# alinlab/ifseg

Measured on AMD Instinct MI355X. Metric: images/sec (512x512, SegOFA-Base fwd+bwd), higher is better.
Workload: dtype bf16; 1 GPU; BASELINE configs[1]: SegOFA-Base bf16, batch 8/GPU, 512x512, 15 classes (L=36), frozen ResNet-101 trunk (one pass per 2 future batches on a second stream; a ring of 4 synthetic batches, every batch through the trunk exactly once), dropout 0.10 / drop-path 0.10; step = fwd + upsample/CE loss + bwd + clip + Adam; steps enqueued from the host; global_batch=8, parallelism=dp1

## Files before the change

### ifseg_amd/csrc/attention.hip

```cpp
#include <type_traits>
#include "common.h"
#include "prof.h"
#include "../../include/ifseg_hip.h"

namespace {

struct AttnArgs {
  const bf16_t *q, *k, *v, *pq, *pk;
  bf16_t* o;
  float* lse;
  int B, H, T, S;
  long long q_bs, k_bs, v_bs, o_bs;
  int ldq, ldk, ldv, ldo, ldpq, ldpk;
  int rel_mode, P, code_bias, n2d, Lt, causal;
  const int* gcode;
  const float *rel2d, *rel1d, *relx, *dense;
  int dense_ld;
  const bf16_t* dO; long long do_bs; int lddo;
  const float* delta;
  bf16_t *dq, *dk, *dv; long long dq_bs, dk_bs, dv_bs; int lddq, lddk, lddv;
  bf16_t *dpq, *dpk;
  float *drel2d_part, *drel1d_part, *drelx_part;
  int nparts;
  const float* gain;
// ... 1148 lines not shown
                }
                bool masked = j >= a.S;
                if (a.causal) {
                  if (tile_grid) masked |= (qi >= a.P) || (j > qi);
                  else masked |= (qi >= a.P) && (j > qi);
                }
                const float p = masked ? 0.f : __builtin_amdgcn_exp2f(fmaf(sv, LOG2E, nlse_q));
                dsv[e] = p * (gain * dp[rg * 4 + e] - del_q);
                pdp = fmaf(p, dp[rg * 4 + e], pdp);
              }
            }
            ud.w[rg2 * 2] = pack2bf(dsv[0], dsv[1]); ud.w[rg2 * 2 + 1] = pack2bf(dsv[2], dsv[3]);
          }
          dsf[s2] = ud.b;
        }
#pragma unroll
        for (int s2 = 0; s2 < 2; ++s2) {
#pragma unroll
          for (int cb = 0; cb < NKS / 2; ++cb) {
            const int o0 = (bKt ^ (cb << 6)) + (kb * 32 + s2 * 16) * 256;
            U64 x, y;
            x.s = lds_read_tr(sKb(cur) + o0);
            y.s = lds_read_tr(sKb(cur) + ((o0 + 2048) ^ 32));
            U128 f; f.w[0] = x.w[0]; f.w[1] = x.w[1]; f.w[2] = y.w[0]; f.w[3] = y.w[1];
            dq[cb] = __builtin_amdgcn_mfma_f32_32x32x16_bf16(f.b, dsf[s2], dq[cb], 0, 0, 0);
          }
        }
      }
    }
    if (it + 1 < nsched) store_kv(cur ^ 1);
    __syncthreads();
  }

  if (a.dgain_rows) {
    const float tot = pdp + __shfl_xor(pdp, 32);
    if (qvalid && half == 0) a.dgain_rows[((long long)b * a.H + h) * a.T + qi] = tot;
  }
  if (qvalid) {
    bf16_t* dqp = a.dq + (long long)b * a.dq_bs + (long long)qi * a.lddq + h * 64;
#pragma unroll
    for (int db = 0; db < 2; ++db) store_tile_bf16(dqp + db * 32, dq[db], a.dq_scale, half, true);
    if constexpr (HAS_POS) {
      bf16_t* pp = a.dpq + ((long long)b * a.T + qi) * (a.H * 64) + h * 64;
#pragma unroll
      for (int db = 0; db < 2; ++db) store_tile_bf16(pp + db * 32, dq[2 + db], a.dpq_scale, half, true);
    }
  }
}

template <bool HAS_POS>
__global__ __launch_bounds__(256, 2) void attn_bwd_dq_kernel(AttnArgs a) { attn_bwd_dq_body<HAS_POS>(a, blockIdx.x); }


__global__ void attn_delta_kernel(const bf16_t* o, const bf16_t* dO, float* delta, int B, int H, int T,
                                  long long o_bs, int ldo, long long do_bs, int lddo) {
  const long long gid = (long long)blockIdx.x * blockDim.x + threadIdx.x;
  const long long grp = gid >> 3;
  const int sub = (int)(gid & 7);
  const long long total = (long long)B * T * H;
  float acc = 0.f;
  if (grp < total) {
    const int hh = (int)(grp % H);
    const long long bt = grp / H;
    const int t = (int)(bt % T), bb = (int)(bt / T);
    U128 x, y;
    x.v = *reinterpret_cast<const uint4*>(o + bb * o_bs + (long long)t * ldo + hh * 64 + sub * 8);
    y.v = *reinterpret_cast<const uint4*>(dO + bb * do_bs + (long long)t * lddo + hh * 64 + sub * 8);
#pragma unroll
    for (int e = 0; e < 4; ++e) acc += bflo(x.w[e]) * bflo(y.w[e]) + bfhi(x.w[e]) * bfhi(y.w[e]);
  }
  acc += __shfl_xor(acc, 1); acc += __shfl_xor(acc, 2); acc += __shfl_xor(acc, 4);
  if (grp < total && sub == 0) {
    const int hh = (int)(grp % H);
    const long long bt = grp / H;
    delta[((bt / T) * H + hh) * T + (bt % T)] = acc;
  }
}

}

namespace {
constexpr int SMALL_TAB_MAX = 2048;
struct ReduceArgs { ifseg_attn_reduce_args a; int nbq, nbk, nbt[3]; };
__global__ __launch_bounds__(256) void attn_bwd_reduce_kernel(ReduceArgs r) {
  const ifseg_attn_reduce_args& a = r.a;
  int blk = blockIdx.x;
  const int tid = threadIdx.x;
  if (blk < r.nbq + r.nbk) {
    const bool isq = blk < r.nbq;
    if (!isq) blk -= r.nbq;
    const long long n = (long long)(isq ? a.T : a.S) * a.C;
    const bf16_t* part = reinterpret_cast<const bf16_t*>(isq ? a.dpos_q_part : a.dpos_k_part);
    float* acc = isq ? a.dpos_q_acc : a.dpos_k_acc;
    const long long i = ((long long)blk * 256 + tid) * 8;
    if (i >= n) return;
    float s[8] = {0.f, 0.f, 0.f, 0.f, 0.f, 0.f, 0.f, 0.f};
    if (a.accumulate_pos) {
      const float4 a0 = *reinterpret_cast<const float4*>(acc + i), a1 = *reinterpret_cast<const float4*>(acc + i + 4);
      s[0] = a0.x; s[1] = a0.y; s[2] = a0.z; s[3] = a0.w; s[4] = a1.x; s[5] = a1.y; s[6] = a1.z; s[7] = a1.w;
    }
#pragma unroll 8
    for (int b = 0; b < a.B; ++b) {
      const uint4 v = *reinterpret_cast<const uint4*>(part + (long long)b * n + i);
      s[0] += bflo(v.x); s[1] += bfhi(v.x); s[2] += bflo(v.y); s[3] += bfhi(v.y);
      s[4] += bflo(v.z); s[5] += bfhi(v.z); s[6] += bflo(v.w); s[7] += bfhi(v.w);
    }
    *reinterpret_cast<float4*>(acc + i) = make_float4(s[0], s[1], s[2], s[3]);
    *reinterpret_cast<float4*>(acc + i + 4) = make_float4(s[4], s[5], s[6], s[7]);
    return;
  }
  blk -= r.nbq + r.nbk;
  if (blk < a.H) {
    if (!a.dgain) return;
    __shared__ float red[4];
    float s = 0.f;
    for (int b = 0; b < a.B; ++b) {
      const float* d = a.delta + ((long long)b * a.H + blk) * a.T;
      for (int t = tid; t < a.T; t += 256) s += d[t];
    }
    s = warp_sum(s);
    if ((tid & 63) == 0) red[tid >> 6] = s;
    __syncthreads();
    if (tid == 0) reinterpret_cast<bf16_t*>(a.dgain)[blk] = f2bf(((red[0] + red[1]) + (red[2] + red[3])) / a.gain[blk]);
    return;
  }
  blk -= a.H;
  __shared__ float tred[8][33];
  __shared__ float tsmall[SMALL_TAB_MAX];
#pragma unroll
  for (int t = 0; t < 3; ++t) {
    if (t >= a.ntab) return;
    if (blk < r.nbt[t] && a.tab_n[t] <= SMALL_TAB_MAX) {
      const int n = a.tab_n[t], h = blk;
      if (a.nparts <= 8) {
        for (int j = tid; j < n; j += 256) {
          const float* p = a.tab_part[t] + (long long)h * a.nparts * n + j;
          float sum = 0.f;
          for (int q = 0; q < a.nparts; ++q) sum += p[(long long)q * n];
          tsmall[j] = sum;
        }
        __syncthreads();
      } else
      for (int j0 = 0; j0 < n; j0 += 32) {
        const int j = j0 + (tid & 31), g = tid >> 5;
        float sum = 0.f;
        if (j < n) {
          const float* p = a.tab_part[t] + (long long)h * a.nparts * n + j;
#pragma unroll 4
          for (int q = g; q < a.nparts; q += 8) sum += p[(long long)q * n];
        }
        tred[g][tid & 31] = sum;
        __syncthreads();
        if (g == 0 && j < n) {
          float tot = 0.f;
#pragma unroll
          for (int q = 0; q < 8; ++q) tot += tred[q][tid];
          tsmall[j] = tot;
        }
        __syncthreads();
      }
      __shared__ int sidx[SMALL_TAB_MAX];
      for (int j = tid; j < n; j += 256) sidx[j] = a.tab_idx[t][j];
      __syncthreads();
      for (int rb = tid; rb < a.tab_nbucket[t]; rb += 256) {
        float tot = 0.f;
        bool any = false;
        for (int j = 0; j < n; ++j)
          if (sidx[j] == rb) { tot += tsmall[j]; any = true; }
        if (any) a.tab_acc[t][(long long)rb * a.H + h] += tot;
      }
      return;
    }
    if (blk < r.nbt[t]) {
      const int n = a.tab_n[t], nchunk = (n + 31) / 32;
      const int h = blk / nchunk, j = (blk - h * nchunk) * 32 + (tid & 31), g = tid >> 5;
      float sum = 0.f;
      if (j < n) {
        const float* p = a.tab_part[t] + (long long)h * a.nparts * n + j;
#pragma unroll 4
        for (int q = g; q < a.nparts; q += 8) sum += p[(long long)q * n];
      }
      tred[g][tid & 31] = sum;
      __syncthreads();
      if (g == 0 && j < n) {
        const int bucket = a.tab_idx[t][j];
        if (bucket >= 0) {
          float tot = 0.f;
#pragma unroll
          for (int q = 0; q < 8; ++q) tot += tred[q][tid];
          atomicAdd(&a.tab_acc[t][(long long)bucket * a.H + h], tot);
        }
      }
      return;
    }
    blk -= r.nbt[t];
  }
}
}

extern "C" int ifseg_attn_bwd_reduce(const ifseg_attn_reduce_args* x, void* stream) {
  (void)hipGetLastError();
  if (!x || x->B <= 0 || x->H <= 0 || x->T <= 0 || x->S <= 0 || (x->C & 7) || x->ntab < 0 || x->ntab > 3) return IFSEG_ERR_BAD_ARG;
  ReduceArgs r{};
  r.a = *x;
  r.nbq = x->dpos_q_part ? (int)(((long long)x->T * x->C / 8 + 255) / 256) : 0;
  r.nbk = x->dpos_k_part ? (int)(((long long)x->S * x->C / 8 + 255) / 256) : 0;
  long long total = (long long)r.nbq + r.nbk + x->H;
  for (int t = 0; t < x->ntab; ++t) {
    if (!x->tab_part[t] || !x->tab_idx[t] || !x->tab_acc[t] || x->tab_n[t] <= 0 || x->nparts <= 0) return IFSEG_ERR_BAD_ARG;
    if (x->tab_nbucket[t] <= 0) return IFSEG_ERR_BAD_ARG;
    r.nbt[t] = x->tab_n[t] <= SMALL_TAB_MAX ? x->H : x->H * ((x->tab_n[t] + 31) / 32);
    total += r.nbt[t];
  }
  if ((x->dgain && (!x->delta || !x->gain)) || total >= (1ll << 31)) return IFSEG_ERR_BAD_ARG;
  hipLaunchKernelGGL(attn_bwd_reduce_kernel, dim3((unsigned)total), dim3(256), 0, (hipStream_t)stream, r);
  IFSEG_CHECK_LAUNCH();
  return 0;
}

static int attn_check(const AttnArgs& a) {
  if (a.rel_mode || a.causal) {
    if (a.P % 64 || a.P > a.T || a.P > a.S) return IFSEG_ERR_BAD_SHAPE;
  }
  if ((a.ldq | a.ldk | a.ldv | a.ldo) & 7) return IFSEG_ERR_BAD_SHAPE;
  if (((size_t)a.q | (size_t)a.k | (size_t)a.v | (size_t)a.o | (size_t)a.dO | (size_t)a.dq | (size_t)a.dk | (size_t)a.dv) & 15)
    return IFSEG_ERR_BAD_ARG;
  if ((a.q_bs | a.k_bs | a.v_bs | a.o_bs | a.do_bs | a.dq_bs | a.dk_bs | a.dv_bs) & 7) return IFSEG_ERR_BAD_SHAPE;
  return 0;
}

extern "C" int ifseg_attn_fwd(const void* q, const void* k, const void* v, const void* pos_q, const void* pos_k,
                              void* out, float* lse, int B, int H, int T, int S, int ldq, int ldk, int ldv,
                              int ldo, int ldpq, int ldpk, long long q_bs, long long k_bs, long long v_bs,
                              long long o_bs, int rel_mode, int P, const int* gcode, int code_bias, int n2d,
                              const float* rel2d, const float* rel1d, const float* relx, int causal,
                              const float* dense_bias, const void* gain, int grid_w, int dense_ld, void* stream) {
  (void)hipGetLastError();
  AttnArgs a{};
  a.grid_w = grid_w;
  a.q = (const bf16_t*)q; a.k = (const bf16_t*)k; a.v = (const bf16_t*)v;
  a.pq = (const bf16_t*)pos_q; a.pk = (const bf16_t*)pos_k; a.o = (bf16_t*)out; a.lse = lse;
  a.B = B; a.H = H; a.T = T; a.S = S; a.ldq = ldq; a.ldk = ldk; a.ldv = ldv; a.ldo = ldo;
  a.ldpq = ldpq; a.ldpk = ldpk; a.q_bs = q_bs; a.k_bs = k_bs; a.v_bs = v_bs; a.o_bs = o_bs;
  a.rel_mode = rel_mode; a.P = P; a.gcode = gcode; a.code_bias = code_bias; a.n2d = rel_mode ? n2d : 0;
  a.Lt = T - P; a.rel2d = rel2d; a.rel1d = rel1d; a.relx = relx; a.causal = causal; a.dense = dense_bias; a.gain = (const float*)gain;
  a.dense_ld = dense_bias ? (dense_ld > 0 ? dense_ld : S) : 0;
  if (dense_bias && a.dense_ld < S) return IFSEG_ERR_BAD_ARG;
#ifdef IFSEG_EXP_NOBIAS_FWD
  pos_q = nullptr; a.pq = nullptr; a.pk = nullptr; a.rel_mode = 0; a.n2d = 0; rel_mode = 0;
#endif
  if (!rel_mode && !causal) a.P = S;
  int rc = attn_check(a);
  if (rc) return rc;
  const int nq = (T + 127) / 128;
  size_t lds = 2 * (KT_BYTES + VT_BYTES) + (rel_mode ? (((size_t)a.n2d + 3) & ~3) * 4 + (size_t)P * 4 : 0);
  if (lds > 160 * 1024) return IFSEG_ERR_BAD_SHAPE;
  dim3 grid(nq * H * B), block(256);
  hipStream_t s = (hipStream_t)stream;
  ifseg_prof_begin(IFSEG_K_ATTN_FWD, s, 4.0 * 64 * (double)T * S * B * H, 0);
  if (pos_q) {
    if (lds > 64 * 1024) (void)hipFuncSetAttribute((const void*)attn_fwd_kernel<true>, hipFuncAttributeMaxDynamicSharedMemorySize, (int)lds);
    hipLaunchKernelGGL(attn_fwd_kernel<true>, grid, block, lds, s, a);
  } else {
    if (lds > 64 * 1024) (void)hipFuncSetAttribute((const void*)attn_fwd_kernel<false>, hipFuncAttributeMaxDynamicSharedMemorySize, (int)lds);
    hipLaunchKernelGGL(attn_fwd_kernel<false>, grid, block, lds, s, a);
  }
  ifseg_prof_end(IFSEG_K_ATTN_FWD, s);
  IFSEG_CHECK_LAUNCH();
  return 0;
}

extern "C" int ifseg_attn_bwd(const ifseg_attn_bwd_args* x, void* stream) {
  (void)hipGetLastError();
  AttnArgs a{};
  a.q = (const bf16_t*)x->q; a.k = (const bf16_t*)x->k; a.v = (const bf16_t*)x->v;
  a.pq = (const bf16_t*)x->pos_q; a.pk = (const bf16_t*)x->pos_k; a.lse = (float*)x->lse;
  a.B = x->B; a.H = x->H; a.T = x->T; a.S = x->S;
  a.ldq = x->ldq; a.ldk = x->ldk; a.ldv = x->ldv; a.ldpq = x->ldpq; a.ldpk = x->ldpk;
  a.q_bs = x->q_bs; a.k_bs = x->k_bs; a.v_bs = x->v_bs;
  a.rel_mode = x->rel_mode; a.P = x->P; a.gcode = x->gcode; a.code_bias = x->code_bias;
  a.n2d = x->rel_mode ? x->n2d : 0; a.Lt = x->T - x->P;
  a.rel2d = x->rel2d; a.rel1d = x->rel1d; a.relx = x->relx; a.causal = x->causal;
  a.dO = (const bf16_t*)x->dout; a.do_bs = x->do_bs; a.lddo = x->lddo; a.delta = x->delta;
  a.dq = (bf16_t*)x->dq; a.dk = (bf16_t*)x->dk; a.dv = (bf16_t*)x->dv;
  a.dq_bs = x->dq_bs; a.dk_bs = x->dk_bs; a.dv_bs = x->dv_bs; a.lddq = x->lddq; a.lddk = x->lddk; a.lddv = x->lddv;
  a.dpq = (bf16_t*)x->dpos_q_part; a.dpk = (bf16_t*)x->dpos_k_part;
  a.drel2d_part = x->drel2d_part; a.drel1d_part = x->drel1d_part; a.drelx_part = x->drelx_part;
  a.nparts = x->nparts; a.gain = (const float*)x->gain; a.dq_scale = x->dq_scale; a.dpq_scale = x->dpq_scale;
  a.grid_w = x->grid_w;
  a.dgain_rows = x->dgain_rows;
#ifdef IFSEG_EXP_NOBIAS_BWD
  a.pq = nullptr; a.pk = nullptr; a.rel_mode = 0; a.n2d = 0;
#endif
  if (!a.rel_mode && !a.causal) a.P = a.S;
  int rc = attn_check(a);
  if (rc) return rc;
  if ((x->lddo | x->lddq | x->lddk | x->lddv | x->ldout) & 7) return IFSEG_ERR_BAD_SHAPE;
  {
    const long long ldmax = a.ldq > a.lddo ? (a.ldq > a.ldpq ? a.ldq : a.ldpq) : (a.lddo > a.ldpq ? a.lddo : a.ldpq);
    if ((long long)a.T * ldmax * 2 >= (1ll << 31)) return IFSEG_ERR_BAD_SHAPE;
// ... 71 lines not shown
```

### ifseg_amd/csrc/attention_bi.hip

```cpp
#include <type_traits>
#include "common.h"
#include "prof.h"
#include "../../include/ifseg_hip.h"

namespace {

constexpr float NEG_INF = -INFINITY;
constexpr float LOG2E = 1.4426950408889634f;

struct BiArgs {
  const bf16_t *q, *k, *v, *dO;
  const float *lse, *delta, *gain;
  const bf16_t* D;
  float* dgain_rows;
  bf16_t *dq, *dk, *dv, *dbias;
  bf16_t* out; float* lse_out; long long o_bs; int ldo;
  int B, H, T, S, Sp, Tp;
  long long q_bs, k_bs, v_bs, do_bs, dq_bs, dk_bs, dv_bs, dbias_gs;
  int ldq, ldk, ldv, lddo, lddq, lddk, lddv;
  int causal, P;
  float dq_scale;
  const int* kv_len;
  float drop_p;
  unsigned long long drop_seed; const unsigned long long* drop_seed_add;
// ... 610 lines not shown
        fo[s2][db].w[0] = x.w[0]; fo[s2][db].w[1] = x.w[1]; fo[s2][db].w[2] = y.w[0]; fo[s2][db].w[3] = y.w[1];
        x.s = lds_read_tr(sQ + oT[s2][db][0]);
        y.s = lds_read_tr(sQ + oT[s2][db][1]);
        fq[s2][db].w[0] = x.w[0]; fq[s2][db].w[1] = x.w[1]; fq[s2][db].w[2] = y.w[0]; fq[s2][db].w[3] = y.w[1];
      }
    __builtin_amdgcn_sched_barrier(0);
    if (it + 1 < sc.n) issue(it + 1, (it + 1) & 1);
    __builtin_amdgcn_sched_barrier(0);
#pragma unroll
    for (int rg = 0; rg < 4; ++rg) db_expand(wD[rg], s, rg);
    if (anypad) {
#pragma unroll
      for (int e = 0; e < 16; ++e) s[e] = kpad ? NEG_INF : s[e];
    }
#pragma unroll
    for (int ks = 0; ks < 4; ++ks) {
      s = __builtin_amdgcn_mfma_f32_32x32x16_bf16(qf[ks], kf[ks], s, 0, 0, 0);
      dp = __builtin_amdgcn_mfma_f32_32x32x16_bf16(of[ks], vfn[ks], dp, 0, 0, 0);
    }
    U128 up[2], ud[2];
#pragma unroll
    for (int s2 = 0; s2 < 2; ++s2)
#pragma unroll
      for (int e = 0; e < 8; e += 2) {
        const int r = s2 * 8 + e;
        const float p0 = __builtin_amdgcn_exp2f(fmaf(s[r], LOG2E, -ls[r]));
        const float p1 = __builtin_amdgcn_exp2f(fmaf(s[r + 1], LOG2E, -ls[r + 1]));
        if (DROP) {
          const int i = sc.block(it) * 32 + (r & 3) + 8 * (r >> 2) + 4 * half;
          const float k0_ = attn_keep(dr, attn_row_key(dr, rowbase + i), kj), k1_ = attn_keep(dr, attn_row_key(dr, rowbase + i + 1), kj);
          up[s2].w[e >> 1] = pack2bf(p0 * k0_, p1 * k1_);
          ud[s2].w[e >> 1] = pack2bf(-p0 * (de[r] - k0_ * (de[r] - dp[r])), -p1 * (de[r + 1] - k1_ * (de[r + 1] - dp[r + 1])));
        } else {
          up[s2].w[e >> 1] = pack2bf(p0, p1);
          ud[s2].w[e >> 1] = pack2bf(-p0 * dp[r], -p1 * dp[r + 1]);
        }
      }
#pragma unroll
    for (int s2 = 0; s2 < 2; ++s2) {
#pragma unroll
      for (int db = 0; db < 2; ++db) dv[db] = __builtin_amdgcn_mfma_f32_32x32x16_bf16(fo[s2][db].b, up[s2].b, dv[db], 0, 0, 0);
#pragma unroll
      for (int db = 0; db < 2; ++db) dk[db] = __builtin_amdgcn_mfma_f32_32x32x16_bf16(fq[s2][db].b, ud[s2].b, dk[db], 0, 0, 0);
    }
  };

  if (sc.n > 0) issue(0, 0);
  for (int it = 0; it < sc.n; ++it) {
    lds_dma_wait();
    __syncthreads();
    block(it);
  }
  if (bact && kvalid) {
    bf16_t* dvp = a.dv + (long long)b * a.dv_bs + (long long)kj * a.lddv + h * 64;
    bf16_t* dkp = a.dk + (long long)b * a.dk_bs + (long long)kj * a.lddk + h * 64;
#pragma unroll
    for (int db = 0; db < 2; ++db) {
      store_tile_bf16(dvp + db * 32, dv[db], gain, half, true);
      store_tile_bf16(dkp + db * 32, dk[db], 1.f, half, true);
    }
  }
}
__global__ __launch_bounds__(512, 2) void attn_bi_dkv_kernel(BiArgs a) { attn_bi_dkv_body<false>(a); }
__global__ __launch_bounds__(512, 2) void attn_bi_dkv_drop_kernel(BiArgs a) { attn_bi_dkv_body<true>(a); }

__global__ void attn_drop_mask_kernel(unsigned char* out, int B, int H, int T, int S, float p, unsigned long long seed,
                                      const unsigned long long* seed_add) {
  const long long n = (long long)B * H * T * S, id = (long long)blockIdx.x * blockDim.x + threadIdx.x;
  if (id >= n) return;
  const AttnDrop dr = attn_drop_setup(p, seed, seed_add);
  const int j = (int)(id % S);
  const unsigned row = (unsigned)(id / S);
  out[id] = attn_keep(dr, attn_row_key(dr, row), j) != 0.f;
}

struct DenseArgs {
  const bf16_t *pq, *pk;
  int ldpq, ldpk, H, T, S, Sp, Tp;
  int rel_mode, P, code_bias, n2d, Lt, causal;
  const int* gcode;
  const float *rel2d, *rel1d, *relx;
  bf16_t* D;
};

__global__ __launch_bounds__(512) void attn_dense_bias_kernel(DenseArgs a) {
  extern __shared__ __attribute__((aligned(16))) unsigned char smem[];
  float* sT = reinterpret_cast<float*>(smem);
  float* s1 = sT + ((a.n2d + 3) & ~3);
  int* sG = reinterpret_cast<int*>(s1 + ((2 * a.Lt + 2) & ~3));
  const int tid = threadIdx.x, lane = tid & 63, wave = tid >> 6, half = lane >> 5, x = lane & 31;
  const int ntq = a.Tp >> 5, ntk = a.Sp >> 5;
  const int h = blockIdx.x / ntq, ti = blockIdx.x % ntq, i0 = ti * 32;
  float rx0 = 0.f, rx1 = 0.f;
  if (a.rel_mode) {
    for (int i = tid; i < a.n2d; i += 512) sT[i] = a.rel2d[(long long)h * a.n2d + i];
    for (int i = tid; i < 2 * a.Lt - 1; i += 512) s1[i] = a.rel1d[(long long)h * (2 * a.Lt - 1) + i];
    for (int i = tid; i < a.P; i += 512) sG[i] = a.gcode[i];
    rx0 = a.relx[h * 2]; rx1 = a.relx[h * 2 + 1];
  }
  __syncthreads();
  auto entry = [&](int i, int j, float abs_ij) -> float {
    if (i >= a.T || j >= a.S) return NEG_INF;
    if (a.causal) {
      const bool masked = (j < a.P) ? ((i >= a.P) || (j > i)) : ((i >= a.P) && (j > i));
      if (masked) return NEG_INF;
    }
    float r = 0.f;
    if (a.rel_mode) {
      if (i < a.P) r = (j < a.P) ? sT[sG[i] - sG[j] + a.code_bias] : rx0;
      else r = (j < a.P) ? rx1 : s1[(i - j) + a.Lt - 1];
    }
    return abs_ij + r;
  };
  bf16x8 fq[4];
  if (a.pq) {
    const bf16_t* qp = a.pq + (long long)min(i0 + x, a.T - 1) * a.ldpq + h * 64 + half * 8;
#pragma unroll
    for (int ks = 0; ks < 4; ++ks) { U128 u; u.v = *reinterpret_cast<const uint4*>(qp + ks * 16); fq[ks] = u.b; }
  }
  for (int tj = wave; tj < ntk; tj += 8) {
    const int j0 = tj * 32;
    const bool dead = a.causal && j0 < a.P && (i0 >= a.P || j0 > i0 + 31);
    if (dead && (i0 >= a.P || j0 > i0 + 63)) continue;
    bf16x8 fk[4];
    if (a.pq && !dead) {
      const bf16_t* kp = a.pk + (long long)min(j0 + x, a.S - 1) * a.ldpk + h * 64 + half * 8;
#pragma unroll
      for (int ks = 0; ks < 4; ++ks) { U128 w; w.v = *reinterpret_cast<const uint4*>(kp + ks * 16); fk[ks] = w.b; }
    }
    f32x16 acc;
#pragma unroll
    for (int e = 0; e < 16; ++e) acc[e] = 0.f;
    if (a.pq && !dead) {
#pragma unroll
      for (int ks = 0; ks < 4; ++ks) acc = __builtin_amdgcn_mfma_f32_32x32x16_bf16(fq[ks], fk[ks], acc, 0, 0, 0);
    }
    {
      unsigned* dp = reinterpret_cast<unsigned*>(a.D + ((long long)h * a.Tp + i0 + 4 * half) * a.Sp + j0 + (x & ~1));
      const bool odd = x & 1;
#pragma unroll
      for (int rg = 0; rg < 4; ++rg) {
        float v[4];
#pragma unroll
        for (int e = 0; e < 4; ++e) v[e] = dead ? NEG_INF : entry(i0 + 8 * rg + 4 * half + e, j0 + x, acc[rg * 4 + e]);
        const float s0 = odd ? v[0] : v[2], s1 = odd ? v[1] : v[3];
        const float r0 = __int_as_float(__builtin_amdgcn_update_dpp(0, __float_as_int(s0), 0xB1, 0xf, 0xf, true));
        const float r1 = __int_as_float(__builtin_amdgcn_update_dpp(0, __float_as_int(s1), 0xB1, 0xf, 0xf, true));
        const unsigned w0 = odd ? pack2bf(r0, v[2]) : pack2bf(v[0], r0), w1 = odd ? pack2bf(r1, v[3]) : pack2bf(v[1], r1);
        const int e0 = odd ? 2 : 0;
        dp[((long long)(8 * rg + e0) * a.Sp) >> 1] = w0;
        dp[((long long)(8 * rg + e0 + 1) * a.Sp) >> 1] = w1;
      }
    }
  }
}

constexpr int DB_NSUB = 8;
constexpr int DB_NPARTS = 4;
struct DbArgs {
  const bf16_t* dbias;
  long long gs;
  int ng, H, T, S, Sp, C;
  const bf16_t *pq, *pk;
  int ldpq, ldpk;
  float *dpq, *dpk;
  int accumulate;
  int tab_accumulate;
  float dpq_scale;
  int P, gh, gw, Lt, causal;
  float *drel2d, *drel1d, *drelx;
  int nb_q, nb_k, nb_2d;
};

__device__ __forceinline__ bf16x8 tr_frag(const unsigned char* tile, int rbase, int cb, int lane) {
  const int half = lane >> 5, i16 = lane & 15, g16 = (lane >> 4) & 1;
  const int col = cb * 32 + g16 * 16 + (i16 & 3) * 4;
  const int r0 = rbase + 4 * half + (i16 >> 2);
  U64 x, y;
  x.s = lds_read_tr(tile + vx_off(r0, col * 2));
  y.s = lds_read_tr(tile + vx_off(r0 + 8, col * 2));
  U128 f; f.w[0] = x.w[0]; f.w[1] = x.w[1]; f.w[2] = y.w[0]; f.w[3] = y.w[1];
  return f.b;
}

__global__ __launch_bounds__(256) void attn_dbias_grads_kernel(DbArgs a) {
  __shared__ __attribute__((aligned(16))) unsigned char sm[32768];
  const int tid = threadIdx.x, lane = tid & 63, half = lane >> 5;
  const int wave = __builtin_amdgcn_readfirstlane(tid >> 6);
  int blk = blockIdx.x < a.nb_q ? xcd_remap(blockIdx.x, a.nb_q) : a.nb_q + xcd_remap(blockIdx.x - a.nb_q, a.nb_k);
  const int lr = lane >> 3, lc = lane & 7;
  if (blk < a.nb_q) {
    const int nit = (a.T + 31) >> 5;
    const int h = blk / nit, i0 = (blk % nit) * 32;
    const int i = i0 + (lane & 31);
    const int ir = i < a.T ? i : a.T - 1;
    unsigned char* tile = sm + wave * 8192;
    f32x16 acc[2];
#pragma unroll
    for (int e = 0; e < 16; ++e) { acc[0][e] = 0.f; acc[1][e] = 0.f; }
    uint4 t4[4], d4[4];
    auto fetch = [&](int j0) {
#pragma unroll
      for (int u = 0; u < 4; ++u) {
        t4[u] = make_uint4(0, 0, 0, 0); d4[u] = make_uint4(0, 0, 0, 0);
        if (j0 + lr + 8 * u < a.S) t4[u] = *reinterpret_cast<const uint4*>(a.pk + (long long)(j0 + lr + 8 * u) * a.ldpk + h * 64 + lc * 8);
        const int g = lc >> 2, irow = min(i0 + lr + 8 * u, a.T - 1);
        if (g < a.ng) d4[u] = *reinterpret_cast<const uint4*>(a.dbias + g * a.gs + ((long long)h * a.T + irow) * a.Sp + j0 + (lc & 3) * 8);
      }
    };
    auto live = [&](int j) { return !(a.causal && j < a.P && (i0 >= a.P || j > i0 + 31)); };
    int j0 = wave * 32;
    if (j0 < a.Sp) fetch(j0);
    for (; j0 < a.Sp; j0 += 128) {
      if (!live(j0)) { if (j0 + 128 < a.Sp) fetch(j0 + 128); continue; }
      __builtin_amdgcn_wave_barrier();
#pragma unroll
      for (int u = 0; u < 4; ++u) {
        const int o = vx_off(lr + 8 * u, lc * 16);
        *reinterpret_cast<uint4*>(tile + o) = t4[u];
        *reinterpret_cast<uint4*>(tile + 4096 + o) = d4[u];
      }
      __builtin_amdgcn_fence(__ATOMIC_RELEASE, "wavefront");
      __builtin_amdgcn_wave_barrier();
      if (j0 + 128 < a.Sp) fetch(j0 + 128);
      U128 bfr[2][2];
#pragma unroll
      for (int s2 = 0; s2 < 2; ++s2)
#pragma unroll
        for (int g = 0; g < 2; ++g) {
          const int cb = g * 64 + (16 * s2 + 4 * half) * 2;
          const uint2 lo = *reinterpret_cast<const uint2*>(tile + 4096 + vx_off(lane & 31, cb));
          const uint2 hi = *reinterpret_cast<const uint2*>(tile + 4096 + vx_off(lane & 31, cb + 16));
          bfr[s2][g].w[0] = lo.x; bfr[s2][g].w[1] = lo.y; bfr[s2][g].w[2] = hi.x; bfr[s2][g].w[3] = hi.y;
        }
#pragma unroll
      for (int s2 = 0; s2 < 2; ++s2) {
        const bf16x8 a0 = tr_frag(tile, 16 * s2, 0, lane), a1 = tr_frag(tile, 16 * s2, 1, lane);
#pragma unroll
        for (int g = 0; g < 2; ++g)
          if (g < a.ng) {
            acc[0] = __builtin_amdgcn_mfma_f32_32x32x16_bf16(a0, bfr[s2][g].b, acc[0], 0, 0, 0);
            acc[1] = __builtin_amdgcn_mfma_f32_32x32x16_bf16(a1, bfr[s2][g].b, acc[1], 0, 0, 0);
          }
      }
      __builtin_amdgcn_wave_barrier();
    }
    __syncthreads();
    float* red = reinterpret_cast<float*>(sm);
#pragma unroll
    for (int cb = 0; cb < 2; ++cb) {
      if (cb) __syncthreads();
#pragma unroll
      for (int r = 0; r < 16; ++r) red[(wave * 16 + r) * 64 + lane] = acc[cb][r];
      __syncthreads();
#pragma unroll
      for (int k = 0; k < 4; ++k) {
        const int v = tid + 256 * k, r = v >> 6, ln = v & 63;
        const float t = (red[r * 64 + ln] + red[(16 + r) * 64 + ln]) + (red[(32 + r) * 64 + ln] + red[(48 + r) * 64 + ln]);
        const int c = cb * 32 + (r & 3) + 8 * (r >> 2) + 4 * (ln >> 5), ii = i0 + (ln & 31);
        if (ii < a.T) {
          float* p = a.dpq + (long long)ii * a.C + h * 64 + c;
          *p = (a.accumulate ? *p : 0.f) + t * a.dpq_scale;
        }
      }
    }
    return;
  }
  blk -= a.nb_q;
  {
    const int njt = a.Sp >> 5;
    const int h = blk / njt, jw0 = (blk % njt) * 32;
    unsigned char* sQ = sm + wave * 8192;
    f32x16 acc[2];
#pragma unroll
    for (int e = 0; e < 16; ++e) { acc[0][e] = 0.f; acc[1][e] = 0.f; }
    uint4 t4[4], d4[4];
    auto fetch = [&](int i0) {
#pragma unroll
      for (int u = 0; u < 4; ++u) {
        const int r = lr + 8 * u;
        t4[u] = make_uint4(0, 0, 0, 0); d4[u] = make_uint4(0, 0, 0, 0);
        if (i0 + r < a.T) {
          t4[u] = *reinterpret_cast<const uint4*>(a.pq + (long long)(i0 + r) * a.ldpq + h * 64 + lc * 8);
          const int g = lc >> 2;
          if (g < a.ng) d4[u] = *reinterpret_cast<const uint4*>(a.dbias + g * a.gs + ((long long)h * a.T + i0 + r) * a.Sp + jw0 + (lc & 3) * 8);
        }
      }
    };
    auto live = [&](int i) { return !(a.causal && jw0 < a.P && (i >= a.P || jw0 > i + 31)); };
    int i0 = wave * 32;
    if (i0 < a.T) fetch(i0);
    for (; i0 < a.T; i0 += 128) {
      if (!live(i0)) { if (i0 + 128 < a.T) fetch(i0 + 128); continue; }
      __builtin_amdgcn_wave_barrier();
#pragma unroll
      for (int u = 0; u < 4; ++u) {
        const int o = vx_off(lr + 8 * u, lc * 16);
        *reinterpret_cast<uint4*>(sQ + o) = t4[u];
        *reinterpret_cast<uint4*>(sQ + 4096 + o) = d4[u];
      }
      __builtin_amdgcn_fence(__ATOMIC_RELEASE, "wavefront");
      __builtin_amdgcn_wave_barrier();
      if (i0 + 128 < a.T) fetch(i0 + 128);
#pragma unroll
      for (int s2 = 0; s2 < 2; ++s2) {
        const bf16x8 a0 = tr_frag(sQ, 16 * s2, 0, lane), a1 = tr_frag(sQ, 16 * s2, 1, lane);
#pragma unroll
        for (int g = 0; g < 2; ++g)
          if (g < a.ng) {
            const bf16x8 bfr = tr_frag(sQ + 4096, 16 * s2, g, lane);
            acc[0] = __builtin_amdgcn_mfma_f32_32x32x16_bf16(a0, bfr, acc[0], 0, 0, 0);
            acc[1] = __builtin_amdgcn_mfma_f32_32x32x16_bf16(a1, bfr, acc[1], 0, 0, 0);
          }
      }
      __builtin_amdgcn_wave_barrier();
    }
    __syncthreads();
    float* red = reinterpret_cast<float*>(sm);
#pragma unroll
    for (int cb = 0; cb < 2; ++cb) {
      if (cb) __syncthreads();
#pragma unroll
      for (int r = 0; r < 16; ++r) red[(wave * 16 + r) * 64 + lane] = acc[cb][r];
      __syncthreads();
#pragma unroll
      for (int k = 0; k < 4; ++k) {
        const int v = tid + 256 * k, r = v >> 6, ln = v & 63;
        const float t = (red[r * 64 + ln] + red[(16 + r) * 64 + ln]) + (red[(32 + r) * 64 + ln] + red[(48 + r) * 64 + ln]);
        const int c = cb * 32 + (r & 3) + 8 * (r >> 2) + 4 * (ln >> 5), j = jw0 + (ln & 31);
        if (j < a.S) {
          float* p = a.dpk + (long long)j * a.C + h * 64 + c;
          *p = (a.accumulate ? *p : 0.f) + t;
        }
      }
    }
  }
}

__global__ __launch_bounds__(256) void attn_dbias_tables_kernel(DbArgs a) {
  __shared__ __attribute__((aligned(16))) float sf[2 * 4096];
  const int tid = threadIdx.x;
  int blk = blockIdx.x < a.nb_2d ? xcd_remap(blockIdx.x, a.nb_2d) : blockIdx.x;
  auto add8 = [](float* t, const uint4& v) {
    t[0] += bflo(v.x); t[1] += bfhi(v.x); t[2] += bflo(v.y); t[3] += bfhi(v.y);
    t[4] += bflo(v.z); t[5] += bfhi(v.z); t[6] += bflo(v.w); t[7] += bfhi(v.w);
  };
  if (blk < a.nb_2d) {
    const int ndy = 2 * a.gh - 1, w = a.gw, nch = w >> 3, npair = w * nch;
    const int dy = blk % ndy - (a.gh - 1), part = (blk / ndy) % DB_NPARTS, h = blk / (DB_NPARTS * ndy);
    const int ylo = dy > 0 ? dy : 0, yhi = dy < 0 ? a.gh + dy : a.gh;
    const int y0 = ylo + ((part - ylo) % DB_NPARTS + DB_NPARTS) % DB_NPARTS;
    float* out = a.drel2d + ((long long)h * DB_NPARTS + part) * ndy * (2 * w - 1) + (long long)(dy + a.gh - 1) * (2 * w - 1);
    if (a.causal && dy < 0) {
      if (!a.tab_accumulate) for (int d = tid; d < 2 * w - 1; d += 256) out[d] = 0.f;
      return;
    }
    const int nyp = npair <= 128 ? 2 : 1;
    const int yp = tid / npair, p = tid - yp * npair;
    for (int p0 = 0; p0 < npair; p0 += 256) {
      const int pp = p0 + p;
      float t[8] = {0.f, 0.f, 0.f, 0.f, 0.f, 0.f, 0.f, 0.f};
      const bool on = yp < nyp && pp < npair;
      const int xi = on ? pp / nch : 0, xc = on ? pp - xi * nch : 0;
      if (on) {
        const bf16_t* base = a.dbias + ((long long)h * a.T + xi) * a.Sp + xc * 8 - (long long)dy * w;
        const long long ystep = (long long)w * a.Sp + w;
#pragma unroll 4
        for (int yi = y0 + yp * DB_NPARTS; yi < yhi; yi += nyp * DB_NPARTS) {
          add8(t, *reinterpret_cast<const uint4*>(base + yi * ystep));
          if (a.ng > 1) add8(t, *reinterpret_cast<const uint4*>(base + a.gs + yi * ystep));
        }
      }
      if (p0) __syncthreads();
      if (on) {
#pragma unroll
        for (int e = 0; e < 8; ++e) sf[yp * 4096 + xi * w + xc * 8 + e] = t[e];
      }
      __syncthreads();
    }
    for (int d = tid; d < 2 * w - 1; d += 256) {
      const int dx = d - (w - 1);
      float t = 0.f;
      for (int xi = (dx > 0 ? dx : 0); xi < (dx < 0 ? w + dx : w); ++xi) {
        t += sf[xi * w + (xi - dx)];
        if (nyp > 1) t += sf[4096 + xi * w + (xi - dx)];
      }
      out[d] = (a.tab_accumulate ? out[d] : 0.f) + t;
    }
    return;
  }
  blk -= a.nb_2d;
  if (blk >= a.H * DB_NPARTS) {
    blk -= a.H * DB_NPARTS;
    const int sub = blk % DB_NSUB, part = (blk / DB_NSUB) % DB_NPARTS, h = blk / (DB_NSUB * DB_NPARTS), P = a.P, Lt = a.Lt;
    const bf16_t* hb = a.dbias + (long long)h * a.T * a.Sp;
    float* o1 = a.drel1d + ((long long)h * DB_NPARTS + part) * (2 * Lt - 1);
    const int dl = tid & 63, rc = tid >> 6;
    for (int d0 = sub; d0 < 2 * Lt - 1; d0 += DB_NSUB * 64) {
      const int d = d0 + DB_NSUB * dl;
      float t = 0.f;
      if (d < 2 * Lt - 1) {
        const int off = d - (Lt - 1);
        const int lo = off > 0 ? off : 0, hi = off < 0 ? Lt + off : Lt;
        const int first = lo + ((part - lo) % DB_NPARTS + DB_NPARTS) % DB_NPARTS;
#pragma unroll 4
        for (int ti = first + rc * DB_NPARTS; ti < hi; ti += 4 * DB_NPARTS) {
          const long long o = (long long)(P + ti) * a.Sp + P + ti - off;
          t += bf2f(hb[o]);
          if (a.ng > 1) t += bf2f(hb[a.gs + o]);
        }
      }
      __syncthreads();
      sf[rc * 64 + dl] = t;
      __syncthreads();
      if (rc == 0 && d < 2 * Lt - 1) {
        const float tt = (sf[dl] + sf[64 + dl]) + (sf[128 + dl] + sf[192 + dl]);
        o1[d] = (a.tab_accumulate ? o1[d] : 0.f) + tt;
      }
    }
    return;
  }
  {
    const int h = blk / DB_NPARTS, part = blk % DB_NPARTS, P = a.P, Lt = a.Lt;
    const bf16_t* hb = a.dbias + (long long)h * a.T * a.Sp;
    auto dB = [&](int i, int j) {
      float t = bf2f(hb[(long long)i * a.Sp + j]);
      if (a.ng > 1) t += bf2f(hb[a.gs + (long long)i * a.Sp + j]);
      return t;
    };
    float t0 = 0.f, t1 = 0.f;
    {
      const int nrow = (P - part + DB_NPARTS - 1) / DB_NPARTS, nch = Lt >> 3, nit = nrow * nch;
      float t[8] = {0.f, 0.f, 0.f, 0.f, 0.f, 0.f, 0.f, 0.f};
      for (int it0 = tid; it0 < nit; it0 += 4 * 256) {
        uint4 v[4][2];
#pragma unroll
        for (int u = 0; u < 4; ++u) {
          const int it = it0 + u * 256, r = it / nch, ch = it - r * nch;
#pragma unroll
          for (int g = 0; g < 2; ++g)
            v[u][g] = (it < nit && g < a.ng) ? *reinterpret_cast<const uint4*>(hb + g * a.gs + (long long)(part + DB_NPARTS * r) * a.Sp + P + ch * 8)
                                             : make_uint4(0, 0, 0, 0);
        }
#pragma unroll
        for (int u = 0; u < 4; ++u) { add8(t, v[u][0]); add8(t, v[u][1]); }
      }
      float tail = 0.f;
      const int nt = Lt & 7;
      for (int it = tid; it < nrow * nt; it += 256) {
        const int r = it / nt, e = it - r * nt;
        tail += dB(part + DB_NPARTS * r, P + (Lt & ~7) + e);
      }
      t0 = ((t[0] + t[1]) + (t[2] + t[3])) + ((t[4] + t[5]) + (t[6] + t[7])) + tail;
    }
    const int nchunk = P >> 3, nrs = nchunk <= 128 ? 2 : 1;
    for (int cc = tid; cc < nchunk * nrs; cc += 256) {
      const int c = cc % nchunk, rs = cc / nchunk;
      float t[8] = {0.f, 0.f, 0.f, 0.f, 0.f, 0.f, 0.f, 0.f};
      int ti = part + rs * DB_NPARTS;
      const int tstep = nrs * DB_NPARTS;
      for (; ti + 3 * tstep < Lt; ti += 4 * tstep) {
        uint4 v[4][2];
#pragma unroll
        for (int u = 0; u < 4; ++u)
#pragma unroll
          for (int g = 0; g < 2; ++g)
            v[u][g] = g < a.ng ? *reinterpret_cast<const uint4*>(hb + g * a.gs + (long long)(P + ti + u * tstep) * a.Sp + c * 8) : make_uint4(0, 0, 0, 0);
#pragma unroll
        for (int u = 0; u < 4; ++u) { add8(t, v[u][0]); add8(t, v[u][1]); }
      }
      for (; ti < Lt; ti += tstep)
        for (int g = 0; g < a.ng; ++g) add8(t, *reinterpret_cast<const uint4*>(hb + g * a.gs + (long long)(P + ti) * a.Sp + c * 8));
      t1 += ((t[0] + t[1]) + (t[2] + t[3])) + ((t[4] + t[5]) + (t[6] + t[7]));
    }
    sf[tid] = t0; sf[256 + tid] = t1;
    __syncthreads();
    for (int o = 128; o > 0; o >>= 1) {
      if (tid < o) { sf[tid] += sf[tid + o]; sf[256 + tid] += sf[256 + tid + o]; }
      __syncthreads();
    }
    float* ox = a.drelx + ((long long)h * DB_NPARTS + part) * 2;
    if (tid == 0) { ox[0] = (a.tab_accumulate ? ox[0] : 0.f) + sf[0]; ox[1] = (a.tab_accumulate ? ox[1] : 0.f) + sf[256]; }
    return;
  }
}

}

extern "C" int ifseg_attn_dense_bias(const void* pos_q, const void* pos_k, int ldpq, int ldpk, int H, int T, int S,
                                     int rel_mode, int P, const int* gcode, int code_bias, int n2d, const float* rel2d,
                                     const float* rel1d, const float* relx, int causal, void* D, int Sp, int Tp,
                                     void* stream) {
  (void)hipGetLastError();
  if (!D || H <= 0 || T <= 0 || S <= 0 || (Sp & 31) || (Tp & 31) || Sp < S || Tp < T) return IFSEG_ERR_BAD_ARG;
  if ((pos_q == nullptr) != (pos_k == nullptr) || ((ldpq | ldpk) & 7)) return IFSEG_ERR_BAD_ARG;
  if (rel_mode && (!gcode || !rel2d || !rel1d || !relx)) return IFSEG_ERR_BAD_ARG;
  if ((rel_mode || causal) && (P > T || P > S || P < 0)) return IFSEG_ERR_BAD_SHAPE;
  DenseArgs a{};
  a.pq = (const bf16_t*)pos_q; a.pk = (const bf16_t*)pos_k; a.ldpq = ldpq; a.ldpk = ldpk;
  a.H = H; a.T = T; a.S = S; a.Sp = Sp; a.Tp = Tp;
  a.rel_mode = rel_mode; a.P = (rel_mode || causal) ? P : S; a.code_bias = code_bias; a.n2d = rel_mode ? n2d : 0; a.Lt = rel_mode ? T - P : 0; a.causal = causal;
  a.gcode = gcode; a.rel2d = rel2d; a.rel1d = rel1d; a.relx = relx; a.D = (bf16_t*)D;
  if ((size_t)D & 15) return IFSEG_ERR_BAD_ARG;
  const size_t lds = rel_mode ? ((((size_t)n2d + 3) & ~(size_t)3) + (((size_t)2 * a.Lt + 2) & ~(size_t)3) + (size_t)P) * 4 : 16;
  if (lds > 160 * 1024) return IFSEG_ERR_BAD_SHAPE;
  if (lds > 64 * 1024) (void)hipFuncSetAttribute((const void*)attn_dense_bias_kernel, hipFuncAttributeMaxDynamicSharedMemorySize, (int)lds);
  hipLaunchKernelGGL(attn_dense_bias_kernel, dim3((unsigned)(H * (Tp / 32))), dim3(512), lds, (hipStream_t)stream, a);
  IFSEG_CHECK_LAUNCH();
  return 0;
}

extern "C" int ifseg_attn_bwd_bi(const ifseg_attn_bi_args* x, void* stream) {
  (void)hipGetLastError();
  if (!x || x->B <= 0 || x->H <= 0 || x->T <= 0 || x->S <= 0) return IFSEG_ERR_BAD_ARG;
  if ((x->Sp & 31) || (x->Tp & 31) || x->Sp < x->S || x->Tp < x->T || !x->D) return IFSEG_ERR_BAD_ARG;
  BiArgs a{};
  a.q = (const bf16_t*)x->q; a.k = (const bf16_t*)x->k; a.v = (const bf16_t*)x->v; a.dO = (const bf16_t*)x->dout;
  a.lse = x->lse; a.delta = x->delta; a.D = (const bf16_t*)x->D; a.gain = (const float*)x->gain;
  a.dq = (bf16_t*)x->dq; a.dk = (bf16_t*)x->dk; a.dv = (bf16_t*)x->dv; a.dbias = (bf16_t*)x->dbias; a.dgain_rows = x->dgain_rows;
  a.B = x->B; a.H = x->H; a.T = x->T; a.S = x->S; a.Sp = x->Sp; a.Tp = x->Tp;
  a.q_bs = x->q_bs; a.k_bs = x->k_bs; a.v_bs = x->v_bs; a.do_bs = x->do_bs; a.dq_bs = x->dq_bs; a.dk_bs = x->dk_bs; a.dv_bs = x->dv_bs;
  a.dbias_gs = (long long)x->H * x->T * x->Sp;
  a.ldq = x->ldq; a.ldk = x->ldk; a.ldv = x->ldv; a.lddo = x->lddo; a.lddq = x->lddq; a.lddk = x->lddk; a.lddv = x->lddv;
  a.causal = x->causal; a.P = x->causal ? x->P : x->S; a.dq_scale = x->dq_scale; a.kv_len = x->kv_len;
  a.drop_p = x->drop_p; a.drop_seed = x->drop_seed; a.drop_seed_add = x->drop_seed_add;
  if (!(a.drop_p >= 0.f && a.drop_p < 1.f)) return IFSEG_ERR_BAD_ARG;
  const bool dropping = a.drop_p > 0.f;
  if ((a.ldq | a.ldk | a.ldv | a.lddo | a.lddq | a.lddk | a.lddv) & 7) return IFSEG_ERR_BAD_SHAPE;
  if (((size_t)a.q | (size_t)a.k | (size_t)a.v | (size_t)a.dO | (size_t)a.dq | (size_t)a.dk | (size_t)a.dv | (size_t)a.dbias) & 15)
    return IFSEG_ERR_BAD_ARG;
  if ((a.q_bs | a.k_bs | a.v_bs | a.do_bs | a.dq_bs | a.dk_bs | a.dv_bs) & 7) return IFSEG_ERR_BAD_SHAPE;
  if (a.causal && ((a.P & 63) || a.P > a.T || a.P > a.S)) return IFSEG_ERR_BAD_SHAPE;
  {
    long long ldmax = a.ldq;
    for (long long l : {(long long)a.lddo, (long long)a.ldk, (long long)a.ldv}) ldmax = l > ldmax ? l : ldmax;
    const long long rows = a.T > a.S ? a.T : a.S;
    if (rows * ldmax * 2 >= (1ll << 31) || (long long)a.Tp * a.Sp * 2 >= (1ll << 31))
      return IFSEG_ERR_BAD_SHAPE;
  }
  hipStream_t s = (hipStream_t)stream;
  const int nbg = (a.B + 3) / 4;
  const int ph = x->phases ? x->phases : (IFSEG_ATTN_BWD_DKV | IFSEG_ATTN_BWD_DQ);
  if (ph & IFSEG_ATTN_BWD_DKV) {
    if (!a.dk || !a.dv) return IFSEG_ERR_BAD_ARG;
    auto kern = dropping ? attn_bi_dkv_drop_kernel : attn_bi_dkv_kernel;
    (void)hipFuncSetAttribute((const void*)kern, hipFuncAttributeMaxDynamicSharedMemorySize, LDS_DKV);
    ifseg_prof_begin(IFSEG_K_ATTN_DKV, s, 6.0 * 64 * (double)a.T * a.S * a.B * a.H, 0);
    hipLaunchKernelGGL(kern, dim3(((a.S + 63) / 64) * a.H * nbg), dim3(512), LDS_DKV, s, a);
    ifseg_prof_end(IFSEG_K_ATTN_DKV, s);
  }
  if (ph & IFSEG_ATTN_BWD_DQ) {
    if (!a.dq || !a.dbias) return IFSEG_ERR_BAD_ARG;
    auto kern = dropping ? attn_bi_dq_drop_kernel : attn_bi_dq_kernel;
    (void)hipFuncSetAttribute((const void*)kern, hipFuncAttributeMaxDynamicSharedMemorySize, LDS_DQ);
    ifseg_prof_begin(IFSEG_K_ATTN_DQ, s, 2.0 * 64 * (double)a.T * a.S * a.B * a.H, 0);
    hipLaunchKernelGGL(kern, dim3(((a.T + 63) / 64) * a.H * nbg), dim3(512), LDS_DQ, s, a);
    ifseg_prof_end(IFSEG_K_ATTN_DQ, s);
  }
  IFSEG_CHECK_LAUNCH();
  return 0;
}

extern "C" int ifseg_attn_fwd_bi(const ifseg_attn_bi_args* x, void* stream) {
  (void)hipGetLastError();
  if (!x || x->B <= 0 || x->H <= 0 || x->T <= 0 || x->S <= 0 || !x->q || !x->k || !x->v || !x->out || !x->lse || !x->D) return IFSEG_ERR_BAD_ARG;
  if ((x->Sp & 31) || x->Sp < x->S || (x->Tp & 31) || x->Tp < x->T) return IFSEG_ERR_BAD_ARG;
  BiArgs a{};
  a.q = (const bf16_t*)x->q; a.k = (const bf16_t*)x->k; a.v = (const bf16_t*)x->v; a.D = (const bf16_t*)x->D; a.gain = (const float*)x->gain;
  a.out = (bf16_t*)x->out; a.lse_out = const_cast<float*>(x->lse); a.o_bs = x->out_bs; a.ldo = x->ldout;
  a.B = x->B; a.H = x->H; a.T = x->T; a.S = x->S; a.Sp = x->Sp; a.Tp = x->Tp;
  a.q_bs = x->q_bs; a.k_bs = x->k_bs; a.v_bs = x->v_bs; a.ldq = x->ldq; a.ldk = x->ldk; a.ldv = x->ldv;
  a.causal = x->causal; a.P = x->causal ? x->P : x->S; a.kv_len = x->kv_len;
  a.drop_p = x->drop_p; a.drop_seed = x->drop_seed; a.drop_seed_add = x->drop_seed_add;
  if (!(a.drop_p >= 0.f && a.drop_p < 1.f)) return IFSEG_ERR_BAD_ARG;
  if ((a.ldq | a.ldk | a.ldv | a.ldo) & 7) return IFSEG_ERR_BAD_SHAPE;
  if (((size_t)a.q | (size_t)a.k | (size_t)a.v | (size_t)a.out) & 15) return IFSEG_ERR_BAD_ARG;
  if ((a.q_bs | a.k_bs | a.v_bs | a.o_bs) & 7) return IFSEG_ERR_BAD_SHAPE;
  if (a.causal && ((a.P & 63) || a.P > a.T || a.P > a.S)) return IFSEG_ERR_BAD_SHAPE;
  {
    const long long ldmax = a.ldk > a.ldv ? a.ldk : a.ldv;
    if ((long long)a.S * ldmax * 2 >= (1ll << 31) || (long long)a.Tp * a.Sp * 2 >= (1ll << 31)) return IFSEG_ERR_BAD_SHAPE;
  }
  hipStream_t s = (hipStream_t)stream;
  const int lds = 2 * STG_DQ;
  auto kern = a.drop_p > 0.f ? attn_bi_fwd_drop_kernel : attn_bi_fwd_kernel;
  (void)hipFuncSetAttribute((const void*)kern, hipFuncAttributeMaxDynamicSharedMemorySize, lds);
  ifseg_prof_begin(IFSEG_K_ATTN_FWD, s, 4.0 * 64 * (double)a.T * a.S * a.B * a.H, 0);
  hipLaunchKernelGGL(kern, dim3(((a.T + 63) / 64) * a.H * ((a.B + 3) / 4)), dim3(512), lds, s, a);
  ifseg_prof_end(IFSEG_K_ATTN_FWD, s);
  IFSEG_CHECK_LAUNCH();
  return 0;
}

extern "C" int ifseg_attn_dbias_grads(const ifseg_attn_dbias_args* x, void* stream) {
  (void)hipGetLastError();
  if (!x || !x->dbias || x->ng <= 0 || x->H <= 0 || x->T <= 0 || x->S <= 0 || (x->Sp & 31) || x->Sp < x->S)
    return IFSEG_ERR_BAD_ARG;
  DbArgs a{};
  a.dbias = (const bf16_t*)x->dbias; a.gs = (long long)x->H * x->T * x->Sp; a.ng = x->ng;
  a.H = x->H; a.T = x->T; a.S = x->S; a.Sp = x->Sp; a.C = x->C;
  a.pq = (const bf16_t*)x->pos_q; a.pk = (const bf16_t*)x->pos_k; a.ldpq = x->ldpq; a.ldpk = x->ldpk;
  a.dpq = x->dpos_q_acc; a.dpk = x->dpos_k_acc; a.accumulate = x->accumulate_pos; a.dpq_scale = x->dpq_scale;
  a.P = x->P; a.gh = x->grid_h; a.gw = x->grid_w; a.Lt = x->T - x->P; a.causal = x->causal;
  if (a.causal && (a.P <= 0 || (a.P & 31))) return IFSEG_ERR_BAD_SHAPE;
  a.drel2d = x->drel2d; a.drel1d = x->drel1d; a.drelx = x->drelx;
  const bool pos = a.pq != nullptr;
  if (pos && (!a.pk || !a.dpq || !a.dpk || ((a.ldpq | a.ldpk) & 7) || (a.C & 3) || a.C < a.H * 64)) return IFSEG_ERR_BAD_ARG;
  const bool rel = a.drel2d != nullptr;
  if (rel) {
    if (!a.drel1d || !a.drelx || a.gh <= 0 || a.gw <= 0 || a.gw > 64 || (a.gw & 7) || a.gh * a.gw != a.P || a.P > a.T || a.P > a.S || a.T != a.S)
      return IFSEG_ERR_BAD_SHAPE;
  }
  a.nb_q = pos ? a.H * ((a.T + 31) / 32) : 0;
  a.nb_k = pos ? a.H * (a.Sp / 32) : 0;
  a.nb_2d = rel ? a.H * (2 * a.gh - 1) * DB_NPARTS : 0;
  const int ng_all = x->ng;
  for (int g0 = 0; g0 < ng_all; g0 += 2) {
    a.dbias = (const bf16_t*)x->dbias + (long long)g0 * a.gs;
    a.ng = ng_all - g0 < 2 ? ng_all - g0 : 2;
    if (g0) { a.accumulate = 1; a.tab_accumulate = 1; }
    if (pos) hipLaunchKernelGGL(attn_dbias_grads_kernel, dim3(a.nb_q + a.nb_k), dim3(256), 0, (hipStream_t)stream, a);
    if (rel) hipLaunchKernelGGL(attn_dbias_tables_kernel, dim3(a.nb_2d + a.H * DB_NPARTS * (1 + DB_NSUB)), dim3(256), 0, (hipStream_t)stream, a);
  }
  IFSEG_CHECK_LAUNCH();
  return 0;
}

extern "C" int ifseg_attn_dbias_nparts(void) { return DB_NPARTS; }

extern "C" int ifseg_attn_dropout_mask(unsigned char* keep, int B, int H, int T, int S, float p, unsigned long long seed,
                                       const unsigned long long* seed_add, void* stream) {
  (void)hipGetLastError();
  if (!keep || B <= 0 || H <= 0 || T <= 0 || S <= 0 || !(p >= 0.f && p < 1.f) || (long long)B * H * T >= (1ll << 32)) return IFSEG_ERR_BAD_ARG;
  const long long n = (long long)B * H * T * S;
  hipLaunchKernelGGL(attn_drop_mask_kernel, dim3((unsigned)((n + 255) / 256)), dim3(256), 0, (hipStream_t)stream, keep, B, H, T, S, p, seed, seed_add);
  IFSEG_CHECK_LAUNCH();
  return 0;
}
```

### ifseg_amd/hip.py

```python
import contextlib
import ctypes
import os

import torch

from . import lab

_HERE = os.path.dirname(os.path.abspath(__file__))
LIB_PATH = os.environ.get("IFSEG_LIB", os.path.join(_HERE, "lib", "libifseg_hip.so"))
_lib = None

GEMM_NT, GEMM_NN, GEMM_TN = 0, 1, 2
GEMM_RELU, GEMM_OUT_F32, GEMM_ACCUMULATE = 1, 2, 4

c_void_p, c_int, c_float, c_ll = ctypes.c_void_p, ctypes.c_int, ctypes.c_float, ctypes.c_longlong


ABI_VERSION = 21


def lib():
    global _lib
    if _lib is None:
        if not os.path.exists(LIB_PATH):
# ... 265 lines not shown
        P = rel.P
    if P is None:
        P = S
    rc = L.ifseg_attn_fwd(_ptr(q), _ptr(k), _ptr(v), _ptr(pos_q), _ptr(pos_k), _ptr(out), _ptr(lse), c_int(B),
                          c_int(H), c_int(T), c_int(S), c_int(q.stride(1)), c_int(k.stride(1)), c_int(v.stride(1)),
                          c_int(out.stride(1)), c_int(pos_q.stride(0) if pos_q is not None else 0),
                          c_int(pos_k.stride(0) if pos_k is not None else 0), c_ll(q.stride(0)), c_ll(k.stride(0)),
                          c_ll(v.stride(0)), c_ll(out.stride(0)), c_int(1 if rel is not None else 0), c_int(P),
                          _ptr(rel.gcode) if rel is not None else None, c_int(rel.code_bias if rel is not None else 0),
                          c_int(rel.rel2d.shape[1] if rel is not None else 0),
                          _ptr(rel.rel2d) if rel is not None else None, _ptr(rel.rel1d) if rel is not None else None,
                          _ptr(rel.relx) if rel is not None else None, c_int(1 if causal else 0), _ptr(dense_bias),
                          _ptr(_f32(gain)), c_int(rel.grid_w if rel is not None else 0),
                          c_int(dense_bias.stride(1) if dense_bias is not None else 0), _stream())
    _check(rc, "attn_fwd")
    return out


ATTN_BWD_DELTA, ATTN_BWD_DKV, ATTN_BWD_DQ = 1, 2, 4


def attn_bwd(q, k, v, pos_q, pos_k, out, dout, lse, delta, dq, dk, dv, dpq_part, dpk_part, B, H, T, S, rel=None,
             causal=False, P=None, gain=None, dq_scale=1.0, dpq_scale=1.0, drel2d_part=None, drel1d_part=None,
             drelx_part=None, nparts=0, phases=0, dgain_rows=None):
    a = _AttnBwdArgs()
    a.dgain_rows = _p(dgain_rows)
    assert all(t is None or t.dtype == torch.bfloat16 for t in (dpq_part, dpk_part)), "abs-pos partials are bf16"
    if rel is not None:
        P = rel.P
    if P is None:
        P = S
    for name, t in (("q", q), ("k", k), ("v", v), ("pos_q", pos_q), ("pos_k", pos_k), ("out", out), ("dout", dout),
                    ("lse", lse), ("delta", delta), ("dq", dq), ("dk", dk), ("dv", dv), ("dpos_q_part", dpq_part),
                    ("dpos_k_part", dpk_part), ("gain", _f32(gain)), ("drel2d_part", drel2d_part),
                    ("drel1d_part", drel1d_part), ("drelx_part", drelx_part)):
        setattr(a, name, _p(t))
    a.B, a.H, a.T, a.S = B, H, T, S
    a.ldq, a.ldk, a.ldv = q.stride(1), k.stride(1), v.stride(1)
    a.ldpq = pos_q.stride(0) if pos_q is not None else 0
    a.ldpk = pos_k.stride(0) if pos_k is not None else 0
    a.ldout, a.lddo, a.lddq, a.lddk, a.lddv = out.stride(1), dout.stride(1), dq.stride(1), dk.stride(1), dv.stride(1)
    a.q_bs, a.k_bs, a.v_bs, a.out_bs = q.stride(0), k.stride(0), v.stride(0), out.stride(0)
    a.do_bs, a.dq_bs, a.dk_bs, a.dv_bs = dout.stride(0), dq.stride(0), dk.stride(0), dv.stride(0)
    a.rel_mode = 1 if rel is not None else 0
    a.P, a.causal, a.nparts = P, 1 if causal else 0, nparts
    if rel is not None:
        a.code_bias, a.n2d = rel.code_bias, rel.rel2d.shape[1]
        a.gcode, a.rel2d, a.rel1d, a.relx = _p(rel.gcode), _p(rel.rel2d), _p(rel.rel1d), _p(rel.relx)
        a.grid_w = rel.grid_w
    a.dq_scale, a.dpq_scale = dq_scale, dpq_scale
    a.phases = phases
    rc = lib().ifseg_attn_bwd(ctypes.byref(a), _stream())
    _check(rc, "attn_bwd")


def _pad32(n):
    return (n + 31) // 32 * 32


class DenseBias:

    def __init__(self, H, T, S, device):
        self.H, self.T, self.S, self.Sp, self.Tp = H, T, S, _pad32(S), _pad32(T)
        self.D = torch.empty(H, self.Tp, self.Sp, dtype=torch.bfloat16, device=device)


def attn_dense_bias(dense, pos_q, pos_k, rel=None, causal=False, P=None):
    if rel is not None:
        P = rel.P
    if P is None:
        P = dense.S
    rc = lib().ifseg_attn_dense_bias(
        _ptr(pos_q), _ptr(pos_k), c_int(pos_q.stride(0) if pos_q is not None else 0),
        c_int(pos_k.stride(0) if pos_k is not None else 0), c_int(dense.H), c_int(dense.T), c_int(dense.S),
        c_int(1 if rel is not None else 0), c_int(P), _ptr(rel.gcode) if rel is not None else None,
        c_int(rel.code_bias if rel is not None else 0), c_int(rel.rel2d.shape[1] if rel is not None else 0),
        _ptr(rel.rel2d) if rel is not None else None, _ptr(rel.rel1d) if rel is not None else None,
        _ptr(rel.relx) if rel is not None else None, c_int(1 if causal else 0), _ptr(dense.D), c_int(dense.Sp),
        c_int(dense.Tp), _stream())
    _check(rc, "attn_dense_bias")
    return dense


class _AttnBiArgs(ctypes.Structure):
    _fields_ = ([(n, c_void_p) for n in ("q", "k", "v", "dout", "lse", "delta", "D", "gain", "dq", "dk", "dv", "dbias")]
                + [(n, c_int) for n in ("B", "H", "T", "S", "Sp", "Tp", "ldq", "ldk", "ldv", "lddo", "lddq", "lddk", "lddv")]
                + [(n, c_ll) for n in ("q_bs", "k_bs", "v_bs", "do_bs", "dq_bs", "dk_bs", "dv_bs")]
                + [("causal", c_int), ("P", c_int), ("dq_scale", c_float), ("phases", c_int), ("dgain_rows", c_void_p),
                   ("out", c_void_p), ("ldout", c_int), ("out_bs", c_ll), ("kv_len", c_void_p), ("drop_p", c_float),
                   ("drop_seed", ctypes.c_uint64), ("drop_seed_add", c_void_p)])


def _attn_drop(a, drop):
    if drop is not None and drop[0] > 0:
        a.drop_p, a.drop_seed, a.drop_seed_add = float(drop[0]), drop[1] & 0xFFFFFFFFFFFFFFFF, _seed_add_ptr()


def attn_dropout_mask(B, H, T, S, p, seed, device):
    out = torch.empty(B, H, T, S, dtype=torch.uint8, device=device)
    _check(lib().ifseg_attn_dropout_mask(_ptr(out), c_int(B), c_int(H), c_int(T), c_int(S), c_float(p),
                                         ctypes.c_uint64(seed & 0xFFFFFFFFFFFFFFFF), c_void_p(_seed_add_ptr()), _stream()), "attn_dropout_mask")
    return out


def _kvlen(kv_len, B):
    if kv_len is None:
        return None
    assert kv_len.dtype == torch.int32 and kv_len.is_cuda and kv_len.numel() == B and kv_len.is_contiguous()
    return kv_len


def attn_bwd_bi(q, k, v, dout, lse, delta, dense, dq, dk, dv, dbias, B, H, T, S, causal=False, P=None, gain=None,
                dq_scale=1.0, phases=0, dgain_rows=None, kv_len=None, drop=None):
    a = _AttnBiArgs()
    for name, t in (("q", q), ("k", k), ("v", v), ("dout", dout), ("lse", lse), ("delta", delta), ("D", dense.D),
                    ("gain", _f32(gain)), ("dq", dq), ("dk", dk), ("dv", dv), ("dbias", dbias)):
        setattr(a, name, _p(t))
    assert dbias.dtype == torch.bfloat16 and tuple(dbias.shape) == ((B + 3) // 4, H, T, dense.Sp) and dbias.is_contiguous()
    a.B, a.H, a.T, a.S, a.Sp, a.Tp = B, H, T, S, dense.Sp, dense.Tp
    a.ldq, a.ldk, a.ldv, a.lddo = q.stride(1), k.stride(1), v.stride(1), dout.stride(1)
    a.lddq, a.lddk, a.lddv = dq.stride(1), dk.stride(1), dv.stride(1)
    a.q_bs, a.k_bs, a.v_bs, a.do_bs = q.stride(0), k.stride(0), v.stride(0), dout.stride(0)
    a.dq_bs, a.dk_bs, a.dv_bs = dq.stride(0), dk.stride(0), dv.stride(0)
    a.causal, a.P = (1 if causal else 0), (P if P is not None else S)
    a.dq_scale, a.phases = dq_scale, phases
    a.dgain_rows = _p(dgain_rows)
    a.kv_len = _p(_kvlen(kv_len, B))
    _attn_drop(a, drop)
    _check(lib().ifseg_attn_bwd_bi(ctypes.byref(a), _stream()), "attn_bwd_bi")


def dbias_nparts():
    return lib().ifseg_attn_dbias_nparts()


def attn_fwd_bi(q, k, v, dense, out, lse, B, H, T, S, causal=False, P=None, gain=None, kv_len=None, drop=None):
    a = _AttnBiArgs()
    for name, t in (("q", q), ("k", k), ("v", v), ("lse", lse), ("D", dense.D), ("gain", _f32(gain)), ("out", out)):
        setattr(a, name, _p(t))
    a.B, a.H, a.T, a.S, a.Sp, a.Tp = B, H, T, S, dense.Sp, dense.Tp
    a.ldq, a.ldk, a.ldv, a.ldout = q.stride(1), k.stride(1), v.stride(1), out.stride(1)
    a.q_bs, a.k_bs, a.v_bs, a.out_bs = q.stride(0), k.stride(0), v.stride(0), out.stride(0)
    a.causal, a.P = (1 if causal else 0), (P if P is not None else S)
    a.kv_len = _p(_kvlen(kv_len, B))
    _attn_drop(a, drop)
    _check(lib().ifseg_attn_fwd_bi(ctypes.byref(a), _stream()), "attn_fwd_bi")
    return out


class _AttnDbiasArgs(ctypes.Structure):
    _fields_ = [("dbias", c_void_p), ("ng", c_int), ("H", c_int), ("T", c_int), ("S", c_int), ("Sp", c_int), ("C", c_int),
                ("pos_q", c_void_p), ("pos_k", c_void_p), ("ldpq", c_int), ("ldpk", c_int),
                ("dpos_q_acc", c_void_p), ("dpos_k_acc", c_void_p), ("accumulate_pos", c_int), ("dpq_scale", c_float),
                ("P", c_int), ("grid_h", c_int), ("grid_w", c_int),
                ("drel2d", c_void_p), ("drel1d", c_void_p), ("drelx", c_void_p), ("causal", c_int)]


def attn_dbias_grads(dbias, S, pos_q=None, pos_k=None, dpq_acc=None, dpk_acc=None, accumulate_pos=False, dpq_scale=1.0,
                     P=0, grid_h=0, grid_w=0, drel2d=None, drel1d=None, drelx=None, causal=False):
    if drel2d is not None:
        assert all(t.shape[1] == dbias_nparts() and t.is_contiguous() for t in (drel2d, drel1d, drelx))
    a = _AttnDbiasArgs()
    ng, H, T, Sp = dbias.shape
    a.dbias, a.ng, a.H, a.T, a.S, a.Sp = _p(dbias), ng, H, T, S, Sp
    a.C = dpq_acc.shape[1] if dpq_acc is not None else 0
    a.pos_q, a.pos_k = _p(pos_q), _p(pos_k)
    a.ldpq = pos_q.stride(0) if pos_q is not None else 0
    a.ldpk = pos_k.stride(0) if pos_k is not None else 0
    a.dpos_q_acc, a.dpos_k_acc = _p(dpq_acc), _p(dpk_acc)
    a.accumulate_pos, a.dpq_scale = (1 if accumulate_pos else 0), dpq_scale
    a.P, a.grid_h, a.grid_w = P, grid_h, grid_w
    a.drel2d, a.drel1d, a.drelx = _p(drel2d), _p(drel1d), _p(drelx)
    a.causal = 1 if causal else 0
    _check(lib().ifseg_attn_dbias_grads(ctypes.byref(a), _stream()), "attn_dbias_grads")


def attn_bias_pack(dense, bias, causal=False, P=None):
    f32, hs, rs = 0, 0, 0
    if bias is not None:
        assert bias.dtype in (torch.float32, torch.bfloat16) and tuple(bias.shape) == (dense.H, dense.T, dense.S), "bias: fp32 / bf16 [H, T, S]"
        assert bias.stride(2) == 1 or dense.S == 1, "bias: the last dimension must be contiguous"
        f32, hs, rs = int(bias.dtype == torch.float32), bias.stride(0), bias.stride(1)
    _check(lib().ifseg_attn_bias_pack(_ptr(bias), c_int(f32), c_ll(hs), c_ll(rs), c_int(dense.H), c_int(dense.T),
                                      c_int(dense.S), c_int(1 if causal else 0), c_int(P if P is not None else dense.S),
                                      _ptr(dense.D), c_int(dense.Sp), c_int(dense.Tp), _stream()), "attn_bias_pack")
    return dense


def attn_dbias_sum(dbias, S, out):
    ng, H, T, Sp = dbias.shape
    assert dbias.dtype == torch.bfloat16 and dbias.is_contiguous()
    assert out.dtype in (torch.float32, torch.bfloat16) and tuple(out.shape) == (H, T, S) and (out.stride(2) == 1 or S == 1)
    _check(lib().ifseg_attn_dbias_sum(_ptr(dbias), c_int(ng), c_int(H), c_int(T), c_int(S), c_int(Sp), _ptr(out),
                                      c_int(int(out.dtype == torch.float32)), c_ll(out.stride(0)), c_ll(out.stride(1)),
                                      _stream()), "attn_dbias_sum")
    return out


def _map(t, rpb):
    if t is None:
        return 0, 0
    if t.dim() == 3:
        return t.stride(0), t.stride(1)
    return 0, t.stride(0)


class _DropArgs(ctypes.Structure):
    _fields_ = [("p", c_float), ("seed", ctypes.c_ulonglong), ("drop_path_scale", c_void_p), ("rows_per_batch", c_int),
                ("seed_add", c_void_p)]


_seed_add = [None]


def set_seed_add(t):
    prev = _seed_add[0]
    _seed_add[0] = t
    return prev


def _seed_add_ptr():
    t = _seed_add[0]
    return t.data_ptr() if t is not None else None


def _drop_ref(drop, rows):
    if drop is None:
        return None
    p, seed, dps, rpb = drop
    return ctypes.byref(_DropArgs(p, seed & 0xFFFFFFFFFFFFFFFF, dps.data_ptr() if dps is not None else None, rpb or rows,
                                  _seed_add_ptr()))


def _ln_flags(gamma, gelu=False, other=None):
    f32 = gamma is not None and gamma.dtype == torch.float32
    if other is not None and gamma is not None:
        assert (other.dtype == torch.float32) == f32
    elif other is not None:
        f32 = other.dtype == torch.float32
    return (1 if gelu else 0) | (2 if f32 else 0)


def ln_fwd(x, gamma, beta, y, mean=None, rstd=None, resid=None, gelu=False, eps=1e-5, drop=None):
    C = x.shape[-1]
    rows = x.numel() // C
    rpb = x.shape[1] if x.dim() == 3 else 0
    xb, xl = _map(x, rpb)
    yb, yl = _map(y, rpb)
    rb, rl = _map(resid, rpb)
    rc = lib().ifseg_ln_fwd(_ptr(x), _ptr(gamma), _ptr(beta), _ptr(resid), _ptr(y), _ptr(mean), _ptr(rstd),
                            c_int(rows), c_int(C), c_float(eps), c_int(_ln_flags(gamma, gelu)), c_int(rpb), c_ll(xb),
                            c_int(xl), c_ll(yb), c_int(yl), c_ll(rb), c_int(rl), _drop_ref(drop, rpb or rows), _stream())
    _check(rc, "ln_fwd")
    return y


def ln_fwd_pair(x, gamma, beta, y, mean, rstd, gamma2, beta2, y2, mean2, rstd2, resid=None, eps=1e-5, drop=None):
# ... 199 lines not shown
def stem_weights_mfma(w):
    wt = torch.zeros(64, 7, 8, 4, dtype=torch.float32, device=w.device)
    wt[:, :, :7, :3] = w.permute(3, 0, 1, 2)
    wt = wt.reshape(64, 224)
    t0 = wt.to(torch.bfloat16)
    t1 = (wt - t0.float()).to(torch.bfloat16)
    t2 = (wt - t0.float() - t1.float()).to(torch.bfloat16)
    return torch.stack([t0, t1, t2]).contiguous()


def stem_conv(x4, w, shift, out, B, H, W):
    if w.dtype == torch.bfloat16:
        assert tuple(w.shape) == (3, 64, 224) and w.is_contiguous()
        _check(lib().ifseg_stem_conv7x7_mfma(_ptr(x4), _ptr(w), _ptr(shift), _ptr(out), c_int(B), c_int(H), c_int(W),
                                             _stream()), "stem_conv_mfma")
        return out
    _check(lib().ifseg_stem_conv7x7(_ptr(x4), _ptr(w), _ptr(shift), _ptr(out), c_int(B), c_int(H), c_int(W),
                                    _stream()), "stem_conv")
    return out


def maxpool(x, out, B, H, W, C):
    _check(lib().ifseg_maxpool3x3s2(_ptr(x), _ptr(out), c_int(B), c_int(H), c_int(W), c_int(C), _stream()), "maxpool")
    return out


def grad_sumsq(g, workspace, out):
    _check(lib().ifseg_grad_sumsq_bf16(_ptr(g), c_ll(g.numel()), _ptr(workspace), _ptr(out), _stream()), "sumsq")
    return out


def droppath_scale(out, keep, seed):
    n, B = out.shape
    _check(lib().ifseg_droppath_scale(_ptr(out), _ptr(keep), c_int(n), c_int(B), ctypes.c_ulonglong(seed & 0xFFFFFFFFFFFFFFFF),
                                      c_void_p(_seed_add_ptr()), _stream()), "droppath_scale")


def adam_step(p32, g, m, v, p16, lr, beta1, beta2, eps, wd, step, grad_scale=1.0, max_norm=0.0, sumsq=None, overflow=None,
              hyper=None):
    _check(lib().ifseg_adam_step(_ptr(p32), _ptr(g), _ptr(m), _ptr(v), _ptr(p16), c_ll(p32.numel()), c_float(lr),
                                 c_float(beta1), c_float(beta2), c_float(eps), c_float(wd), c_int(step),
                                 c_float(grad_scale), c_float(max_norm), _ptr(sumsq), _ptr(overflow), _ptr(hyper), _stream()), "adam")


def rel_gather(table, idx, out):
    n, H = idx.numel(), table.shape[1]
    _check(lib().ifseg_rel_gather(_ptr(table), _ptr(idx), _ptr(out), c_int(n), c_int(H), _stream()), "rel_gather")
    return out


def resized_rel_bias(out, table2d, rel1d, relx, h, w, oh, ow, Lt, causal=False):
    H = out.shape[0]
    assert out.stride(2) == 1 and out.stride(0) == out.shape[1] * out.stride(1)
    _check(lib().ifseg_resized_rel_bias(_ptr(out), _ptr(table2d), _ptr(rel1d), _ptr(relx), c_int(H), c_int(h), c_int(w),
                                        c_int(oh), c_int(ow), c_int(Lt), c_int(1 if causal else 0), c_int(out.stride(1)),
                                        _stream()), "resized_rel_bias")
    return out


def resize_rows_bilinear(src, dst, h, w, oh, ow, src_stride, src_off):
    C = dst.shape[1]
    _check(lib().ifseg_resize_rows_bilinear(_ptr(src), _ptr(dst), c_int(C), c_int(h), c_int(w), c_int(oh), c_int(ow),
                                            c_int(src_stride), c_int(src_off), c_int(src.stride(0)), _stream()),
           "resize_rows_bilinear")
    return dst


def rel_gather_multi(tables, idx, out):
    L, n, H = len(tables), idx.numel(), tables[0].shape[1]
    arr = (c_void_p * L)(*[t.data_ptr() for t in tables])
    _check(lib().ifseg_rel_gather_multi(arr, c_int(L), _ptr(idx), _ptr(out), c_int(n), c_int(H), _stream()), "rel_gather_multi")
    return out


class _AttnReduceArgs(ctypes.Structure):
    _fields_ = [("B", c_int), ("H", c_int), ("T", c_int), ("S", c_int), ("C", c_int), ("nparts", c_int),
                ("accumulate_pos", c_int),
                ("dpos_q_part", c_void_p), ("dpos_k_part", c_void_p), ("dpos_q_acc", c_void_p), ("dpos_k_acc", c_void_p),
                ("delta", c_void_p), ("gain", c_void_p), ("dgain", c_void_p), ("ntab", c_int),
                ("tab_part", c_void_p * 3), ("tab_idx", c_void_p * 3), ("tab_acc", c_void_p * 3), ("tab_n", c_int * 3),
                ("tab_nbucket", c_int * 3)]


def attn_bwd_reduce(B, H, T, S, C, dpq_part, dpk_part, dpq_acc, dpk_acc, accumulate_pos, delta, gain, dgain, nparts, tables):
    assert all(t is None or t.dtype == torch.bfloat16 for t in (dpq_part, dpk_part)), "abs-pos partials are bf16"
    a = _AttnReduceArgs()
    a.B, a.H, a.T, a.S, a.C, a.nparts, a.accumulate_pos = B, H, T, S, C, nparts, 1 if accumulate_pos else 0
    a.dpos_q_part, a.dpos_k_part, a.dpos_q_acc, a.dpos_k_acc = _p(dpq_part), _p(dpk_part), _p(dpq_acc), _p(dpk_acc)
    a.delta, a.gain, a.dgain = _p(delta), _p(_f32(gain)), _p(dgain)
    a.ntab = len(tables)
    for i, (part, idx, acc) in enumerate(tables):
        assert part.dtype == torch.float32 and acc.dtype == torch.float32 and idx.dtype == torch.int32 and acc.shape[1] == H
        a.tab_part[i], a.tab_idx[i], a.tab_acc[i], a.tab_n[i], a.tab_nbucket[i] = _p(part), _p(idx), _p(acc), idx.numel(), acc.shape[0]
    _check(lib().ifseg_attn_bwd_reduce(ctypes.byref(a), _stream()), "attn_bwd_reduce")


def rel_scatter_add(d, idx, acc):
    n, H = idx.numel(), acc.shape[1]
    _check(lib().ifseg_rel_scatter_add(_ptr(d), _ptr(idx), _ptr(acc), c_int(n), c_int(H), _stream()), "rel_scatter")
    return acc


PROF_KINDS = ("gemm_nt", "gemm_nn", "gemm_tn", "conv", "attn_fwd", "attn_bwd_dkv", "attn_bwd_dq", "ln_fwd", "ln_bwd")


def prof_enable(mask, stride=1):
    lib().ifseg_prof_stride(c_int(stride))
    lib().ifseg_prof_enable(ctypes.c_uint(mask))


def prof_reset():
    lib().ifseg_prof_reset()


def prof_read(kind):
    ms, fl, by, n = ctypes.c_double(), ctypes.c_double(), ctypes.c_double(), ctypes.c_int()
    _check(lib().ifseg_prof_read(c_int(kind), ctypes.byref(ms), ctypes.byref(fl), ctypes.byref(by), ctypes.byref(n)), "prof_read")
    return {"kind": PROF_KINDS[kind], "ms": ms.value, "flops": fl.value, "bytes": by.value, "launches": n.value}


def seg_loss(logits_pad, target, hp, wp, H, W, nseg, seg_id_offset, tile_partial, stats_part, stats, dlogits_pad,
             loss_out, pad_id=1, eos_id=2, bad_label=None, label_smoothing=0.0):
    B = logits_pad.shape[0]
    ldl = logits_pad.stride(1)
    _check(lib().ifseg_seg_loss_tiles(_ptr(logits_pad), c_int(ldl), c_ll(logits_pad.stride(0)), _ptr(target),
                                      c_ll(target.stride(0)), c_int(B), c_int(hp), c_int(wp), c_int(H), c_int(W),
                                      c_int(nseg), c_ll(seg_id_offset), c_ll(pad_id), c_ll(eos_id),
                                      _ptr(tile_partial), _ptr(stats_part), _ptr(bad_label), c_float(label_smoothing), _stream()), "seg_loss_tiles")
    reduce_parts(stats_part, stats, 1, B * hp * wp, 2 + 3 * nseg)
    _check(lib().ifseg_seg_loss_gather(_ptr(tile_partial), _ptr(stats), _ptr(dlogits_pad), c_int(dlogits_pad.stride(1)),
                                       c_ll(dlogits_pad.stride(0)), c_int(B), c_int(hp), c_int(wp), c_int(nseg),
                                       _ptr(loss_out), _stream()), "seg_loss_gather")
    return loss_out


def rows_to_f32(logits_pad, nseg, rows_per_batch, softmax=False, temperature=1.0):
    B = logits_pad.shape[0]
    out = torch.empty(B, rows_per_batch, nseg, dtype=torch.float32, device=logits_pad.device)
    _check(lib().ifseg_softmax_rows(_ptr(logits_pad), c_ll(logits_pad.stride(0)), c_int(rows_per_batch),
                                    c_int(logits_pad.stride(1)), _ptr(out), c_int(B * rows_per_batch), c_int(nseg),
                                    c_float(1.0 / temperature), c_int(1 if softmax else 0), _stream()), "softmax_rows")
    return out


def neighbour_smoothing(logits_pad, nseg, feat, iters, topk, temperature=1.0):
    B, P, D = feat.shape
    dev = feat.device
    fn = torch.empty(B * P, D, dtype=torch.bfloat16, device=dev)
    _check(lib().ifseg_l2norm_rows_bf16(_ptr(feat.contiguous()), _ptr(fn), c_int(B * P), c_int(D), _stream()), "l2norm_rows")
    sim = torch.empty(B, P, P, dtype=torch.float32, device=dev)
    gemm(GEMM_NT, fn, fn, sim, P, P, D, D, D, P, flags=GEMM_OUT_F32, batch=B, sA=P * D, sB=P * D, sC=P * P)
    idx = torch.empty(B * P, topk, dtype=torch.int32, device=dev)
    _check(lib().ifseg_topk_rows_f32(_ptr(sim), _ptr(idx), c_int(B * P), c_int(P), c_int(topk), _stream()), "topk_rows")
    prob = rows_to_f32(logits_pad, nseg, P, softmax=True, temperature=temperature)
    tmp = torch.empty_like(prob)
    for _ in range(iters):
        _check(lib().ifseg_gather_mean(_ptr(prob), _ptr(idx), _ptr(tmp), c_int(B), c_int(P), c_int(nseg), c_int(topk),
                                       _stream()), "gather_mean")
        prob, tmp = tmp, prob
    return prob


def seg_eval(scores, hp, wp, target, h, w, seg_id_offset):
    n = scores.shape[-1]
    dev = scores.device
    nblk = (h * w + 255) // 256
    hist = torch.zeros(3, n, dtype=torch.int64, device=dev)
    part = torch.empty(nblk, 2, dtype=torch.float32, device=dev)
    _check(lib().ifseg_seg_eval(_ptr(scores.contiguous()), c_int(hp), c_int(wp), c_int(n), _ptr(target.contiguous()), c_int(h),
                                c_int(w), c_ll(seg_id_offset), _ptr(hist), _ptr(part), c_int(nblk), _stream()), "seg_eval")
    tot = torch.empty(2, dtype=torch.float32, device=dev)
    reduce_parts(part, tot, 1, nblk, 2)
    return tot[0] / tot[1], hist


SEG_PREDICT_MAX_CLASSES = 512

# ... 474 lines not shown
```

### ifseg_amd/models/segofa/engine.py

```python
import contextlib
import math
import os
import time

import torch

from ... import hip, lab
from . import resized as R
from .config import image_rp_bucket, token_bucket_of_delta

BF = torch.bfloat16
_POISON = lab.get("POISON_WS", "") == "1"
_EXP_SKIP = set(filter(None, lab.get("EXP_SKIP", "").split(",")))


def _pad8(n):
    return (n + 7) // 8 * 8


class HipEngine:
    def __init__(self, model):
        self.model = model
        self.cfg = model.cfg
        self.packed = False
        self.device = None
        self._ws_grad, self._ws_aux = {}, {}
        self._saved_grad, self._saved_aux = {}, {}
        self.ws, self.saved = self._ws_grad, self._saved_grad
        self._gctx = None
        self._popt = None
        self.ctx_building = None
        self._views = {}
        self.geo = {}
        self.ctx = None
        self.grad_ready_hook = None
        self.drop_on = False
        self.step_seed = 0
        self.step_dev, self._step_pin, self._step_pin_i, self._step_dev_val = None, None, 0, None
        self._pending_checks, self._checked_kinds = [], set()
        self.master_owned = False
        self.overlap = lab.get("NO_OVERLAP") is None
        self.delta_fused = lab.get("NO_DELTA_FUSE") is None
        self._side = None
        self._trunk_stream, self._pf, self._pf_slot = None, None, 0
        self._pf_more = []
        self.trunk_lookahead = max(1, int(lab.get("TRUNK_LOOKAHEAD", "2")))
        self._pf_request = None
        self._pending, self._in_flush = [], False
        self._dw_tasks = []
        self._kfix_tasks = []
        self._ln_red_tasks, self._ln_red_acc = [], []
        self.dw_grouped = lab.get("NO_DW_GROUP") is None
        self.drain_timing = [] if lab.get("DRAIN_TIMING") else None
        self.marks = [] if lab.get("PHASE_TIMING") else None
        self.attn_bwd_timing = None
        self._rb_cache, self._wver = {}, 0
        self.ffn_ln_fused = lab.get("NO_FFN_LN_FUSE") is None
        self.attn_bi = lab.get("ATTN_BI", "auto")
        self.kproj_fix = lab.get("NO_KPROJ_FIX") is None
        self.bi_fwd = lab.get("ATTN_BI_FWD", "1") != "0"
        self._ffn_pg_tasks = []
        self._train_fwd = False
        self.trunk_at = lab.get("TRUNK_AT", "fwd")
        self._bt = ""

    def _arena_order(self):
        cfg = self.cfg
        names = dict(self.model.named_parameters())
        order, fused = [], {}

        def add(n):
            if n in names and n not in order:
                order.append(n)

        def mha(p, cross=False):
            add(p + ".c_attn")
            if cross:
                add(p + ".q_proj.weight"); add(p + ".q_proj.bias")
                for suf in (".weight", ".bias"):
                    for pr in ("k_proj", "v_proj"):
                        add("%s.%s%s" % (p, pr, suf))
            else:
                for suf in (".weight", ".bias"):
                    for pr in ("q_proj", "k_proj", "v_proj"):
                        add("%s.%s%s" % (p, pr, suf))
            add(p + ".out_proj.weight"); add(p + ".out_proj.bias")

        def lnp(p):
            add(p + ".weight"); add(p + ".bias")

        e = "encoder."
        for p in ("layernorm_embedding", "patch_layernorm_embedding", "pos_ln", "image_pos_ln", "layer_norm"):
            lnp(e + p)
        add(e + "type_embedding.weight"); add(e + "embed_positions.weight"); add(e + "embed_image_positions.weight")
        for suf in (".weight", ".bias"):
            add(e + "pos_q_linear" + suf); add(e + "pos_k_linear" + suf)
        for i in range(cfg.enc_layers):
            p = "%slayers.%d." % (e, i)
            mha(p + "self_attn")
            for q in ("self_attn_layer_norm", "attn_ln", "final_layer_norm", "ffn_layernorm"):
                lnp(p + q)
            for q in ("fc1", "fc2"):
                add(p + q + ".weight"); add(p + q + ".bias")
            add("%stoken_rel_pos_table_list.%d.weight" % (e, i)); add("%simage_rel_pos_table_list.%d.weight" % (e, i))
        d = "decoder."
        for p in ("layernorm_embedding", "seg_pos_ln", "layer_norm"):
            lnp(d + p)
        add(d + "embed_seg_positions.weight")
        for suf in (".weight", ".bias"):
            add(d + "self_pos_q_linear" + suf); add(d + "self_pos_k_linear" + suf)
        for n in ("cross_pos_q_linear", "cross_pos_k_linear"):
            add(d + n + ".weight"); add(d + n + ".bias")
        for i in range(cfg.dec_layers):
            p = "%slayers.%d." % (d, i)
            mha(p + "self_attn"); mha(p + "encoder_attn", cross=True)
            for q in ("self_attn_layer_norm", "self_attn_ln", "encoder_attn_layer_norm", "cross_attn_ln",
                      "final_layer_norm", "ffn_layernorm"):
                lnp(p + q)
            for q in ("fc1", "fc2"):
                add(p + q + ".weight"); add(p + q + ".bias")
            add("%sseg_rel_pos_table_list.%d.weight" % (d, i))
        rest_train = [n for n, p in names.items() if n not in order and p.requires_grad and "embed_images" not in n]
        order += rest_train
        n_train_names = len(order)
        frozen = [n for n in names if n not in order and "embed_images" not in n]
        order += frozen
        return order, n_train_names

    def pack(self, device):
        m = self.model
        names = dict(m.named_parameters())
        order, n_train_names = self._arena_order()
        unsupported = [n for n in order[n_train_names:] if names[n].requires_grad]
        unsupported += [n for n, p in names.items() if ("embed_images" in n or "image_proj" in n) and p.requires_grad]
        self.train_tok = bool(names["encoder.embed_tokens.weight"].requires_grad)
        self.train_seg = bool(names["encoder.seg_embed_tokens.weight"].requires_grad)
        if unsupported:
            raise NotImplementedError(
                "ifseg_amd HIP engine: gradients for %s are not implemented (the shipped IFSeg recipe freezes "
                "them: coco_unseen.sh:31-33,76)" % unsupported[:4])
        offs, off = {}, 0
        for n in order:
            offs[n] = off
            off += _pad8(names[n].numel())
        total = off
        n_train = offs[order[n_train_names]] if n_train_names < len(order) else total
        self._views = {}
# ... 132 lines not shown
    def mark(self, name):
        if self.marks is not None and not torch.cuda.is_current_stream_capturing():
            ev = torch.cuda.Event(enable_timing=True)
            ev.record()
            self.marks.append((name, ev, time.perf_counter()))

    def gbuf(self, name, shape, dtype=BF):
        return self.buf(name + "@" + self._bt if self.overlap else name, shape, dtype)

    def _ev(self):
        e = self._evs[self._evi]
        self._evi = (self._evi + 1) % len(self._evs)
        return e

    def _new_stream(self, which, priority=0):
        return torch.cuda.Stream(device=self.device, priority=priority)

    def _wgrad_init(self):
        if self._side is None:
            self._side = self._new_stream("SIDE")
            self._evs = [torch.cuda.Event() for _ in range(128)]
            self._evi = 0

    @contextlib.contextmanager
    def _wgrad(self):
        if not self.overlap:
            yield
            return
        self._wgrad_init()
        e = self._ev()
        e.record(torch.cuda.current_stream())
        self._side.wait_event(e)
        with torch.cuda.stream(self._side):
            prev = hip.set_stream(self._side.cuda_stream)
            try:
                yield
            finally:
                hip.set_stream(prev)

    def _side_do(self, fn):
        if not self.overlap or self._in_flush:
            fn()
        else:
            self._pending.append(fn)

    def _side_flush(self):
        if not self._pending:
            return
        todo, self._pending = self._pending, []
        with self._wgrad():
            self._in_flush = True
            try:
                for fn in todo:
                    fn()
            finally:
                self._in_flush = False

    def _dq_stream_get(self):
        if getattr(self, "_dqs", None) is None:
            self._wgrad_init()
            self._dqs = self._new_stream("DQ")
        return self._dqs

    @contextlib.contextmanager
    def _fork(self, stream):
        e = self._ev()
        e.record(torch.cuda.current_stream())
        stream.wait_event(e)
        with torch.cuda.stream(stream):
            prev = hip.set_stream(stream.cuda_stream)
            try:
                yield
            finally:
                hip.set_stream(prev)

    def _join_side(self):
        self._side_flush()
        if self.overlap and self._side is not None:
            e = self._ev()
            e.record(self._side)
            torch.cuda.current_stream().wait_event(e)

    def _dense_bias(self, tag, H, T, S, pq, pk, rel, causal, P):
        key = "dense_" + tag
        d = self.ws.get(key)
        if d is None or (d.H, d.T, d.S) != (H, T, S):
            d = hip.DenseBias(H, T, S, self.device)
            self.ws[key] = d
        hip.attn_dense_bias(d, pq, pk, rel=rel, causal=causal, P=P)
        return d

    def _dense_from(self, tag, H, T, S, bias):
        key = "dense_" + tag
        d = self.ws.get(key)
        if d is None or (d.H, d.T, d.S) != (H, T, S):
            d = hip.DenseBias(H, T, S, self.device)
            d.D.fill_(float("-inf"))
            self.ws[key] = d
        d.D[:, :T, :S].copy_(bias)
        return d

    def _dense_built(self, ctx, tag):
        if not self.overlap:
            return
        evs = self.__dict__.setdefault("_dense_evs", {})
        ev = evs.get(tag)
        if ev is None:
            ev = evs[tag] = torch.cuda.Event()
        ev.record(self._side)
        ctx.setdefault("dense_ev", {})[tag] = ev

    def _dense_wait(self, tag):
        ev = self.ctx_building.get("dense_ev", {}).pop(tag, None)
        if ev is not None:
            torch.cuda.current_stream().wait_event(ev)

    def _geometry(self, h, w, L):
        key = (h, w, L)
        g = self.geo.get(key)
        if g is not None:
            return g
        cfg, dev = self.cfg, self.device
        P = h * w
        g = {"P": P}
        ys = torch.arange(h).repeat_interleave(w)
        xs = torch.arange(w).repeat(h)
        g["gcode"] = (ys * (2 * w - 1) + xs).int().to(dev)
        g["code_bias"] = (h - 1) * (2 * w - 1) + (w - 1)
        g["n2d"] = (2 * h - 1) * (2 * w - 1)
        dy = torch.arange(-(h - 1), h).repeat_interleave(2 * w - 1)
        dx = torch.arange(-(w - 1), w).repeat(2 * h - 1)
        b = cfg.image_bucket_size
        g["enc_idx2d"] = ((dy + b - 1) * (2 * b - 1) + (dx + b - 1)).int().to(dev)
        tb = token_bucket_of_delta(cfg.token_bucket_size, cfg.max_source_positions)
        dl = torch.arange(-(L - 1), L)
        g["enc_idx1d"] = tb[dl + cfg.max_source_positions - 1].int().to(dev)
        g["enc_idxx"] = torch.tensor([-1, -1], dtype=torch.int32, device=dev)
        sb = cfg.seg_bucket_size
        nseg_rel = (2 * sb - 1) ** 2 + 3
        g["dec_idx2d"] = ((dy + sb - 1) * (2 * sb - 1) + (dx + sb - 1)).int().to(dev)
        g["dec_idx1d"] = torch.tensor([nseg_rel - 1], dtype=torch.int32, device=dev)
        g["dec_idxx"] = torch.tensor([nseg_rel - 2, nseg_rel - 3], dtype=torch.int32, device=dev)
        self.geo[key] = g
        return g

    def prefetch_trunk(self, patch_images, append=False):
        many = isinstance(patch_images, (list, tuple))
        batches = list(patch_images) if many else [patch_images]
        if not batches or not self.packed or any(self.device != t.device for t in batches):
            return
        if any(t.shape != batches[0].shape or t.dtype != batches[0].dtype for t in batches):
            batches = batches[:1]
        if self._trunk_stream is None:
            self._trunk_stream = self._new_stream("TRUNK", -1)
        cur = torch.cuda.current_stream()
        ready = torch.cuda.Event()
        ready.record(cur)
        self._trunk_stream.wait_event(ready)
        slot = self._pf_slot = self._pf_slot ^ 1
        n, B = len(batches), batches[0].shape[0]
        with torch.cuda.stream(self._trunk_stream):
            prev = hip.set_stream(self._trunk_stream.cuda_stream)
            try:
                if n == 1:
                    feat, h, w = self._resnet(batches[0], "@pf%d" % slot)
                else:
                    allimg = self.buf("rn_in@pf%dx%d" % (slot, n), (n * B,) + tuple(batches[0].shape[1:]), batches[0].dtype)
                    for i, t in enumerate(batches):
                        allimg[i * B:(i + 1) * B].copy_(t)
                    feat, h, w = self._resnet(allimg, "@pf%dx%d" % (slot, n))
            finally:
                hip.set_stream(prev)
            done = torch.cuda.Event()
            done.record(self._trunk_stream)
        ents = [{"key": self._tkey(t), "images": t, "feat": feat[i * B:(i + 1) * B], "h": h, "w": w, "done": done}
                for i, t in enumerate(batches)]
        if append and self._pf is not None:
            self._pf_more = self._pf_more + ents
        else:
            self._pf, self._pf_more = ents[0], ents[1:]

    @staticmethod
    def _tkey(t):
        return (t.data_ptr(), t._version, tuple(t.shape), t.dtype)

    def _trunk(self, patch_images):
        pf, self._pf = self._pf, None
        more, self._pf_more = self._pf_more, []
        if pf is not None and pf["key"] == self._tkey(patch_images):
            if more:
                self._pf, self._pf_more = more[0], more[1:]
            if pf.get("done") is not None and not torch.cuda.is_current_stream_capturing():
                torch.cuda.current_stream().wait_event(pf["done"])
# ... 320 lines not shown
        T, Td = P + L, P + 1
        self._drop_setup(B, need_grad)
        self._train_fwd = bool(need_grad)
        ctx = {"B": B, "L": L, "P": P, "T": T, "Td": Td, "h": h, "w": w, "full": bool(full_context_alignment),
               "src_tokens": src_tokens, "feat": feat}
        if resized:
            ctx["resized"] = True
        if pads:
            nonpad = src_tokens.ne(1)
            ctx["nonpad"] = nonpad
            ctx["klen"] = (nonpad.sum(1) + P).to(torch.int32).contiguous()
        self.ctx_building = ctx
        e = "encoder."
        if need_grad and getattr(self, "train_tok", False):
            if bag is not None:
                raise NotImplementedError("ifseg_amd HIP engine: the image-free entry with a trainable token table "
                                          "(--freeze-encoder-embedding false) is not supported")
            ctx["src_ids"] = src_tokens.reshape(-1).contiguous()
        self._params_wait(["g0"])
        img_pre = buf("img_pre", (B * P, C))
        if bag is not None:
            self._params_wait(["emb"])
            hip.embed_bag_mean(W(e + "embed_tokens.weight"), bag[0].contiguous(), bag[1].contiguous(),
                               W(e + "type_embedding.weight")[1], img_pre)
        else:
            bias_img = buf("bias_img", (C,))
            hip.add_bf16(W(e + "image_proj.bias"), W(e + "type_embedding.weight")[1], bias_img)
            hip.linear_fwd(feat.view(B * P, 1024), W(e + "image_proj.weight"), bias_img, out=img_pre)
        x = buf("e_x_in", (B, T, C))
        mu, rs = self._ln_stats("img_ln", B * P)
        hip.ln_fwd(img_pre.view(B, P, C), Wf(e + "patch_layernorm_embedding.weight"),
                   Wf(e + "patch_layernorm_embedding.bias"), x[:, :P], mu, rs, drop=self._dropargs(1))
        tok_pre = buf("tok_pre", (B * L, C))
        self._params_wait(["emb"])
        hip.embed_rows(W(e + "embed_tokens.weight"), src_tokens.reshape(-1).contiguous(),
                       W(e + "type_embedding.weight")[0], tok_pre)
        mu, rs = self._ln_stats("tok_ln", B * L)
        hip.ln_fwd(tok_pre.view(B, L, C), Wf(e + "layernorm_embedding.weight"), Wf(e + "layernorm_embedding.bias"),
                   x[:, P:], mu, rs, drop=self._dropargs(2))
        if pads:
            x[:, P:].mul_(ctx["nonpad"].unsqueeze(-1).to(x.dtype))
        bsz = cfg.image_bucket_size
        pos_all = buf("e_pos_all", (T, C))
        mu, rs = self._ln_stats("ipos_ln", P)
        if resized and P > oh * oh:
            ipos = buf("e_ipos_resized", (P, C))
            hip.resize_rows_bilinear(W(e + "embed_image_positions.weight"), ipos, h, w, oh, oh, bsz, 1)
            hip.ln_fwd(ipos, Wf(e + "image_pos_ln.weight"), Wf(e + "image_pos_ln.bias"), pos_all[:P], mu, rs)
        else:
            img_pos_view = W(e + "embed_image_positions.weight")[1:1 + bsz * h].view(h, bsz, C)[:, :w]
            hip.ln_fwd(img_pos_view, Wf(e + "image_pos_ln.weight"), Wf(e + "image_pos_ln.bias"), pos_all[:P].view(h, w, C), mu, rs)
        mu, rs = self._ln_stats("tpos_ln", L)
        hip.ln_fwd(W(e + "embed_positions.weight")[:L], Wf(e + "pos_ln.weight"), Wf(e + "pos_ln.bias"), pos_all[P:], mu, rs)
        pqk = buf("e_pqk", (T, 2 * C))
        hip.linear_fwd(pos_all, self._fused(self.p16, e + "pos_q_linear.weight", 2 * C, C),
                       self._fused(self.p16, e + "pos_q_linear.bias", 2 * C), out=pqk, alpha=scaling, alpha_ncols=C)
        ctx["e_pq"], ctx["e_pk"] = pqk[:, :C], pqk[:, C:]
        (e_r2,) = self._rel_tables_all("e_img", ["%simage_rel_pos_table_list.%d.weight" % (e, l) for l in range(cfg.enc_layers)],
                                       [(True, g["enc_idx2d"])])
        (e_r1,) = self._rel_tables_all("e_tok", ["%stoken_rel_pos_table_list.%d.weight" % (e, l) for l in range(cfg.enc_layers)],
                                       [(True, g["enc_idx1d"])])
        (e_rx,) = self._rel_tables_all("e_x", [None] * cfg.enc_layers, [(False, g["enc_idxx"])])
        self.mark("enc_layers_start")
        x_pre = None
        bi = resized or ((need_grad or pads) and w <= 64 and w % 8 == 0 and self.attn_bi in ("1", "auto"))
        bi_which = lab.get("ATTN_BI_WHICH", "e+d+c").split("+") if bi else []
        if pads and not (bi and "e" in bi_which and "c" in bi_which and self.bi_fwd):
            raise NotImplementedError("ifseg_amd HIP engine: key padding is implemented by the batch-inner attention kernels "
                                      "(grids up to 64 wide, a multiple of 8)")
        ctx["dense"] = {}
        if resized:
            bi_which = ["e", "d", "c"]
            with self._wgrad():
                bufs = dict(self.model.named_buffers())
                absb = R.abs_bias(ctx["e_pq"], ctx["e_pk"], H)
                for l in range(cfg.enc_layers):
                    relb = R.encoder_rel_bias(W("%stoken_rel_pos_table_list.%d.weight" % (e, l)).float(),
                                              W("%simage_rel_pos_table_list.%d.weight" % (e, l)).float(),
                                              bufs["encoder.token_rp_bucket"], bufs["encoder.image_rp_bucket"], (h, w), oh, bsz, L)
                    ctx["dense"]["e%d" % l] = self._dense_from(("e%d" % l), H, T, T, absb + relb)
                    self._dense_built(ctx, "e%d" % l)
        elif bi and "e" in bi_which:
            with self._wgrad():
                for l in range(cfg.enc_layers):
                    rel = hip.RelBias(P, g["gcode"], g["code_bias"], e_r2[l], e_r1[l], e_rx[l], grid_w=w)
                    ctx["dense"]["e%d" % l] = self._dense_bias("e%d" % l, H, T, T, ctx["e_pq"], ctx["e_pk"], rel, False, P)
                    self._dense_built(ctx, "e%d" % l)
        if need_grad and bi and self.overlap and not self._popt:
            self._dec_pos_dense(ctx, g, pos_all, scaling, bi, bi_which, resized)
        if need_grad and self.overlap and not torch.cuda.is_current_stream_capturing() and "g16fwd" not in _EXP_SKIP:
            with self._wgrad():
                self._params_wait(None, stream=self._side)
                self.g16.zero_()
                if getattr(self, "_g16_ev", None) is None:
                    self._g16_ev = torch.cuda.Event()
                self._g16_ev.record(self._side)
                ctx["g16_zeroed"] = self._g16_ev
        for l in range(cfg.enc_layers):
            p = "%slayers.%d." % (e, l)
            tg = "e%d" % l
            self._params_wait([tg])
            rel = None if resized else hip.RelBias(P, g["gcode"], g["code_bias"], e_r2[l], e_r1[l], e_rx[l], grid_w=w)
            x, xn = self._self_block_fwd(tg, p, "self_attn", "self_attn_layer_norm", "attn_ln", x, B, T,
                                         ctx["e_pq"], ctx["e_pk"], rel, False, scaling, site=("e", l, 0), xn_pre=x_pre,
                                         next_ln=(p + "final_layer_norm", tg + "_fln1", buf(tg + "_fxn", (B * T, C))))
            if l + 1 < cfg.enc_layers:
                nl = ("%slayers.%d.self_attn_layer_norm" % (e, l + 1), "e%d_ln1" % (l + 1), buf("e%d_xn" % (l + 1), (B * T, C)))
            else:
                nl = (e + "layer_norm", "e_final_ln", buf("enc_out", (B, T, C)).view(B * T, C))
            if l + 1 < cfg.enc_layers:
                self._params_wait(["e%d" % (l + 1)])
            x, x_pre = self._ffn_fwd(tg, p, x, B * T, site=("e", l, 1), rpb=T, xn_pre=xn, next_ln=nl)
        enc_out = buf("enc_out", (B, T, C))
        if x_pre is None:
            mu, rs = self._ln_stats("e_final_ln", B * T)
            hip.ln_fwd(x.view(B * T, C), Wf(e + "layer_norm.weight"), Wf(e + "layer_norm.bias"), enc_out.view(B * T, C), mu, rs)
        ctx["e_x_final"] = x
        ctx["enc_out"] = enc_out
        self.mark("enc_fwd_end")
        self._params_wait(None)

        d = "decoder."
        ctx["ckv_ready"] = None
        if need_grad and self.ffn_ln_fused:
            self._ffn_ln_coefs()
        if self.overlap and need_grad:
            with self._wgrad():
                ctx["ckv_ready"] = []
                for l in range(cfg.dec_layers):
                    a_ = "%slayers.%d.encoder_attn" % (d, l)
                    kv = buf("d%d_ckv" % l, (B, T, 2 * C))
                    hip.linear_fwd(enc_out.view(B * T, C), self._fused(self.p16, a_ + ".k_proj.weight", 2 * C, C),
                                   self._fused(self.p16, a_ + ".k_proj.bias", 2 * C), out=kv.view(B * T, 2 * C))
                    ev = self._ev()
                    ev.record(self._side)
                    ctx["ckv_ready"].append(ev)
        y0b = buf("d_bos", (B, 1, C))
        bos = (prev_output_tokens[:, :1] if prev_output_tokens is not None
               else torch.zeros(B, 1, dtype=torch.long, device=dev))
        hip.embed_rows(W(e + "embed_tokens.weight"), bos.reshape(-1).contiguous(), None, y0b)
        ctx["bos_ids"] = bos.reshape(-1).contiguous()
        y = buf("d_y_in", (B, Td, C))
        mu, rs = self._ln_stats("d_emb_ln_p", B * P)
        hip.ln_fwd(enc_out[:, :P], Wf(d + "layernorm_embedding.weight"), Wf(d + "layernorm_embedding.bias"), y[:, :P],
                   mu, rs, drop=self._dropargs(3))
        mu, rs = self._ln_stats("d_emb_ln_b", B)
        hip.ln_fwd(y0b, Wf(d + "layernorm_embedding.weight"), Wf(d + "layernorm_embedding.bias"), y[:, P:], mu, rs,
                   drop=self._dropargs(4))
        if "d_cpq" not in ctx:
            self._dec_pos_dense(ctx, g, pos_all, scaling, bi, bi_which, resized)
        cpq, cpk, causal = ctx["d_cpq"], ctx["d_cpk"], ctx["d_causal"]
        d_r2, d_r1, d_rx = ctx["d_rel"]
        y_pre = None
        for l in range(cfg.dec_layers):
            p = "%slayers.%d." % (d, l)
            tg = "d%d" % l
            rel = None if resized else hip.RelBias(P, g["gcode"], g["code_bias"], d_r2[l], d_r1[l], d_rx[l], grid_w=w)
            y, yn = self._self_block_fwd(tg, p, "self_attn", "self_attn_layer_norm", "self_attn_ln", y, B, Td,
                                         ctx["d_spq"], ctx["d_spk"], rel, causal and not resized, scaling, site=("d", l, 0), xn_pre=y_pre,
                                         next_ln=(p + "encoder_attn_layer_norm", tg + "_cln1", buf(tg + "_cyn", (B * Td, C))))
            y, yn = self._cross_block_fwd(tg, p, y, enc_out, B, Td, T, cpq, cpk, scaling, site=("d", l, 1), yn_pre=yn,
                                          next_ln=(p + "final_layer_norm", tg + "_fln1", buf(tg + "_fxn", (B * Td, C))))
            nl = (("%slayers.%d.self_attn_layer_norm" % (d, l + 1), "d%d_ln1" % (l + 1), buf("d%d_xn" % (l + 1), (B * Td, C)))
                  if l + 1 < cfg.dec_layers else None)
            y, y_pre = self._ffn_fwd(tg, p, y, B * Td, site=("d", l, 2), rpb=Td, xn_pre=yn, next_ln=nl)
        ctx["d_y_final"] = y
        featb = buf("d_feat", (B, Td, C))
        mu, rs = self._ln_stats("d_final_ln_p", B * P)
        hip.ln_fwd(y[:, :P], Wf(d + "layer_norm.weight"), Wf(d + "layer_norm.bias"), featb[:, 1:], mu, rs)
        mu, rs = self._ln_stats("d_final_ln_b", B)
        hip.ln_fwd(y[:, P:], Wf(d + "layer_norm.weight"), Wf(d + "layer_norm.bias"), featb[:, :1], mu, rs)
        logits = buf("logits_pad", (B, Td, self.npad))
        if self.train_seg:
            self.wseg_pad[: cfg.num_seg_tokens].copy_(W("encoder.seg_embed_tokens.weight"))
        hip.linear_fwd(featb.view(B * Td, C), self.wseg_pad, out=logits.view(B * Td, self.npad))
        self.ctx = ctx
        return logits, ctx

    def _dec_pos_dense(self, ctx, g, pos_all, scaling, bi, bi_which, resized):
        cfg = self.cfg
        B, L, P, T, Td, h, w = (ctx[k] for k in ("B", "L", "P", "T", "Td", "h", "w"))
        C, H = cfg.embed_dim, cfg.heads
        W, Wf, buf = self.W, self.Wf, self.buf
        d = "decoder."
        dev = self.device
        sb = cfg.seg_bucket_size
        segtab = W(d + "embed_seg_positions.weight")
        tp = buf("d_tp", (Td, C))
        seg_rows, seg_bos = segtab[1:1 + P], segtab[:1]
        if resized:
            tgt = buf("d_spos_resized", (Td, C))
            hip.resize_rows_bilinear(segtab, tgt[:P], h, w, sb, sb, sb, 1)
            tgt[P:].copy_(segtab[:1])
            seg_rows, seg_bos = tgt[:P], tgt[P:]
        mu, rs = self._ln_stats("d_tp_ln_p", P)
        hip.ln_fwd(seg_rows, Wf(d + "seg_pos_ln.weight"), Wf(d + "seg_pos_ln.bias"), tp[:P], mu, rs)
        mu, rs = self._ln_stats("d_tp_ln_b", 1)
        hip.ln_fwd(seg_bos, Wf(d + "seg_pos_ln.weight"), Wf(d + "seg_pos_ln.bias"), tp[P:], mu, rs)
        spqk = buf("d_spqk", (Td, 2 * C))
        hip.linear_fwd(tp, self._fused(self.p16, d + "self_pos_q_linear.weight", 2 * C, C),
                       self._fused(self.p16, d + "self_pos_q_linear.bias", 2 * C), out=spqk, alpha=scaling, alpha_ncols=C)
        cpq = buf("d_cpq", (Td, C))
        hip.linear_fwd(tp, W(d + "cross_pos_q_linear.weight"), W(d + "cross_pos_q_linear.bias"), out=cpq, alpha=scaling)
        cpk = buf("d_cpk", (T, C))
        hip.linear_fwd(pos_all, W(d + "cross_pos_k_linear.weight"), W(d + "cross_pos_k_linear.bias"), out=cpk)
        ctx.update(d_spq=spqk[:, :C], d_spk=spqk[:, C:], d_cpq=cpq, d_cpk=cpk)
        causal = not ctx["full"]
        d_r2, d_r1, d_rx = self._rel_tables_all(
            "d_seg", ["%sseg_rel_pos_table_list.%d.weight" % (d, l) for l in range(cfg.dec_layers)],
            [(True, g["dec_idx2d"]), (True, g["dec_idx1d"]), (True, g["dec_idxx"])])
        if resized:
            with self._wgrad():
                bufs = dict(self.model.named_buffers())
                absb = R.abs_bias(ctx["d_spq"], ctx["d_spk"], H)
                if causal:
                    absb = absb.masked_fill(R.causal_mask(P, dev)[None], float("-inf"))
                for l in range(cfg.dec_layers):
                    relb = R.decoder_rel_bias(W("%sseg_rel_pos_table_list.%d.weight" % (d, l)).float(), bufs["decoder.seg_rp_bucket"], (h, w), sb)
                    ctx["dense"]["d%d" % l] = self._dense_from("d%d" % l, H, Td, Td, absb + relb)
                    self._dense_built(ctx, "d%d" % l)
                    if l == 0:
                        ctx["dense"]["dc"] = self._dense_bias("dc", H, Td, T, cpq, cpk, None, False, None)
                        self._dense_built(ctx, "dc")
                if self.overlap:
                    if getattr(self, "_dense_ev", None) is None:
                        self._dense_ev = torch.cuda.Event()
                    self._dense_ev.record(self._side)
                    ctx["dense_ready"] = self._dense_ev
        elif bi:
            with self._wgrad():
                for l in range(cfg.dec_layers if "d" in bi_which else 0):
                    rel = hip.RelBias(P, g["gcode"], g["code_bias"], d_r2[l], d_r1[l], d_rx[l], grid_w=w)
                    ctx["dense"]["d%d" % l] = self._dense_bias("d%d" % l, H, Td, Td, ctx["d_spq"], ctx["d_spk"], rel, causal, P)
                    self._dense_built(ctx, "d%d" % l)
                    if l == 0 and "c" in bi_which:
                        ctx["dense"]["dc"] = self._dense_bias("dc", H, Td, T, cpq, cpk, None, False, None)
                        self._dense_built(ctx, "dc")
                if "c" in bi_which and "dc" not in ctx["dense"]:
                    ctx["dense"]["dc"] = self._dense_bias("dc", H, Td, T, cpq, cpk, None, False, None)
                    self._dense_built(ctx, "dc")
                if self.overlap:
                    if getattr(self, "_dense_ev", None) is None:
                        self._dense_ev = torch.cuda.Event()
                    self._dense_ev.record(self._side)
                    ctx["dense_ready"] = self._dense_ev
        ctx["d_causal"], ctx["d_rel"] = causal, (d_r2, d_r1, d_rx)

    def _resized_biases(self, kind, h, w, Lt, causal):
        cfg = self.cfg
        key = (kind, h, w, Lt, bool(causal), self._wver)
        cache = self._rb_cache
        if key in cache:
            cache[key] = cache.pop(key)
            return cache[key]
        H = cfg.heads
        if kind == "e":
            oh = cfg.orig_patch_image_size // 16
            g0 = self._geometry(oh, oh, Lt)
            e = "encoder."
            (r2,) = self._rel_tables_all("rs_e_img", ["%simage_rel_pos_table_list.%d.weight" % (e, l) for l in range(cfg.enc_layers)],
                                         [(True, g0["enc_idx2d"])])
            (r1,) = self._rel_tables_all("rs_e_tok", ["%stoken_rel_pos_table_list.%d.weight" % (e, l) for l in range(cfg.enc_layers)],
                                         [(True, g0["enc_idx1d"])])
            rx, nl = None, cfg.enc_layers
        else:
            oh = cfg.seg_bucket_size
            g0 = self._geometry(oh, oh, 1)
            d = "decoder."
            r2, r1, rx = self._rel_tables_all("rs_d_seg", ["%sseg_rel_pos_table_list.%d.weight" % (d, l) for l in range(cfg.dec_layers)],
                                              [(True, g0["dec_idx2d"]), (True, g0["dec_idx1d"]), (True, g0["dec_idxx"])])
            nl = cfg.dec_layers
        T = h * w + Lt
        out = torch.zeros(nl, H, T, (T + 3) // 4 * 4, dtype=torch.float32, device=self.device)[..., :T]
        for l in range(nl):
            hip.resized_rel_bias(out[l], r2[l], r1[l], rx[l] if rx is not None else None, h, w, oh, oh, Lt, causal=causal)
        while len(cache) >= 2 * 16:
            cache.pop(next(iter(cache)))
        for k in [k for k in cache if k[-1] != self._wver]:
            del cache[k]
        cache[key] = out
        return out

    def _forward_resized(self, src_tokens, feat, h, w, prev_output_tokens, full_context_alignment):
        cfg, dev = self.cfg, self.device
        W, Wf, buf = self.W, self.Wf, self.buf
        self.drop_on = False
        B, L = src_tokens.shape
        C, H = cfg.embed_dim, cfg.heads
        P, T, Td = h * w, h * w + L, h * w + 1
        scaling = float(cfg.head_dim * cfg.attn_scale_factor) ** -0.5
        oh = cfg.orig_patch_image_size // 16
        bsz, sb = cfg.image_bucket_size, cfg.seg_bucket_size
        e, d = "encoder.", "decoder."
        ids = lambda hh, ww, b: (torch.arange(ww, device=dev)[None, :] + torch.arange(hh, device=dev)[:, None] * b + 1).reshape(-1)
        ctx = {"B": B, "L": L, "P": P, "T": T, "Td": Td, "h": h, "w": w, "full": bool(full_context_alignment),
               "src_tokens": src_tokens, "feat": feat, "resized": True}
        bias_img = buf("bias_img", (C,))
        hip.add_bf16(W(e + "image_proj.bias"), W(e + "type_embedding.weight")[1], bias_img)
        img_pre = buf("img_pre", (B * P, C))
        hip.linear_fwd(feat.view(B * P, 1024), W(e + "image_proj.weight"), bias_img, out=img_pre)
        x = buf("e_x_in", (B, T, C))
        hip.ln_fwd(img_pre.view(B, P, C), Wf(e + "patch_layernorm_embedding.weight"),
                   Wf(e + "patch_layernorm_embedding.bias"), x[:, :P])
        tok_pre = buf("tok_pre", (B * L, C))
        hip.embed_rows(W(e + "embed_tokens.weight"), src_tokens.reshape(-1).contiguous(),
                       W(e + "type_embedding.weight")[0], tok_pre)
        hip.ln_fwd(tok_pre.view(B, L, C), Wf(e + "layernorm_embedding.weight"), Wf(e + "layernorm_embedding.bias"), x[:, P:])
        itab = W(e + "embed_image_positions.weight")
        if P > oh * oh:
            ipos = buf("e_ipos_resized", (P, C))
            hip.resize_rows_bilinear(itab, ipos, h, w, oh, oh, bsz, 1)
        else:
            ipos = itab[ids(h, w, bsz)].contiguous()
        pos_all = buf("e_pos_all", (T, C))
        hip.ln_fwd(ipos, Wf(e + "image_pos_ln.weight"), Wf(e + "image_pos_ln.bias"), pos_all[:P])
        hip.ln_fwd(W(e + "embed_positions.weight")[:L], Wf(e + "pos_ln.weight"), Wf(e + "pos_ln.bias"), pos_all[P:])
        pqk = buf("e_pqk", (T, 2 * C))
        hip.linear_fwd(pos_all, self._fused(self.p16, e + "pos_q_linear.weight", 2 * C, C),
                       self._fused(self.p16, e + "pos_q_linear.bias", 2 * C), out=pqk, alpha=scaling, alpha_ncols=C)
        e_dense = self._resized_biases("e", h, w, L, False)
        for l in range(cfg.enc_layers):
            p = "%slayers.%d." % (e, l)
            tg = "e%d" % l
# ... 307 lines not shown
        ones = self.ws.get("ones_h")
        if ones is None or ones.numel() != H:
            ones = self.ws["ones_h"] = torch.ones(H, dtype=torch.float32, device=self.device)
        kw = dict(rel=rel, causal=causal, gain=gain, dq_scale=scaling, dpq_scale=scaling, drel2d_part=parts[0],
                  drel1d_part=parts[1], drelx_part=parts[2], nparts=nparts, dgain_rows=dgr)
        args = (q, k, v, pq, pk, o, do, lse, delta, dq, dk, dv, dpq_part, dpk_part, B, H, T, S)
        timing = self.attn_bwd_timing
        if timing is not None:
            timing["seen"] += 1
            if (timing["seen"] - 1) % timing["stride"]:
                timing = None
            else:
                t0 = torch.cuda.Event(enable_timing=True)
                t0.record()
        if self.overlap and not lab.get("DQ_SERIAL"):
            if not have_delta:
                hip.attn_bwd(*args, phases=hip.ATTN_BWD_DELTA, **kw)
            with self._fork(self._dq_stream_get()):
                if "dq" not in _EXP_SKIP:
                    hip.attn_bwd(*args, phases=hip.ATTN_BWD_DQ, **kw)
                dq_done = self._ev()
                dq_done.record(self._dqs)
            if "dkv" not in _EXP_SKIP:
                hip.attn_bwd(*args, phases=hip.ATTN_BWD_DKV, **kw)
            torch.cuda.current_stream().wait_event(dq_done)
        else:
            hip.attn_bwd(*args, phases=(hip.ATTN_BWD_DKV | hip.ATTN_BWD_DQ) if have_delta else 0, **kw)
        if timing is not None:
            t1 = torch.cuda.Event(enable_timing=True)
            t1.record()
            timing["pairs"].append((t0, t1, 8.0 * 64 * T * S * B * H))
        def reductions():
            tables = []
            if rel is not None:
                for (tabname, idx), part in zip(rel_grads, parts):
                    if tabname is not None:
                        tables.append((part, idx, self._table_acc(tabname)))
            hip.attn_bwd_reduce(B, H, T, S, C, dpq_part, dpk_part, dpq_acc, dpk_acc, not first_pos, dgr, ones,
                                self.G(gain_name), nparts if rel is not None else 1, tables)
        if "reduce" not in _EXP_SKIP:
            self._side_do(reductions)

    def _attn_core_bwd_bi(self, q, k, v, pq, pk, o, lse, do, dq, dk, dv, B, T, S, rel, causal, gain, gain_name, scaling,
                          dpq_acc, dpk_acc, first_pos, rel_grads, delta, have_delta, dense, kv_len=None, adrop=None):
        C, H = self.cfg.embed_dim, self.cfg.heads
        gbuf = self.gbuf
        ng = (B + 3) // 4
        dbias = gbuf("g_dbias%s_%dx%d" % ("c%d" % (rel.P if rel is not None else 0) if causal else "", T, dense.Sp), (ng, H, T, dense.Sp))
        if not getattr(dbias, "_ifseg_zeroed", False):
            dbias.zero_()
            dbias._ifseg_zeroed = True
        if not have_delta:
            hip.attn_bwd(q, k, v, None, None, o, do, lse, delta, dq, dk, dv, None, None, B, H, T, S, phases=hip.ATTN_BWD_DELTA)
        timing = self.attn_bwd_timing
        if timing is not None:
            timing["seen"] += 1
            if (timing["seen"] - 1) % timing["stride"]:
                timing = None
            else:
                t0 = torch.cuda.Event(enable_timing=True)
                t0.record()
        P = rel.P if rel is not None else None
        dgr = gbuf("g_dgain_rows_%d" % T, (B, H, T), torch.float32)
        ones = self.ws.get("ones_h")
        if ones is None or ones.numel() != H:
            ones = self.ws["ones_h"] = torch.ones(H, dtype=torch.float32, device=self.device)
        ph = 0
        if "dq" in _EXP_SKIP:
            ph = hip.ATTN_BWD_DKV
        if "dkv" in _EXP_SKIP:
            ph = hip.ATTN_BWD_DQ if not ph else -1
        if ph >= 0:
            hip.attn_bwd_bi(q, k, v, do, lse, delta, dense, dq, dk, dv, dbias, B, H, T, S, causal=causal, P=P, gain=gain,
                            dq_scale=scaling, phases=ph, dgain_rows=dgr, kv_len=kv_len, drop=adrop)
        if timing is not None:
            t1 = torch.cuda.Event(enable_timing=True)
            t1.record()
            timing["pairs"].append((t0, t1, 8.0 * 64 * T * S * B * H))
        parts = [None, None, None]
        if rel is not None:
            parts = [gbuf("g_relg%d_%d" % (i, t.shape[1]), (H, hip.dbias_nparts(), t.shape[1]), torch.float32)
                     for i, t in enumerate((rel.rel2d, rel.rel1d, rel.relx))]

        def reductions():
            kw = {}
            if rel is not None:
                kw = dict(P=rel.P, grid_h=rel.P // rel.grid_w, grid_w=rel.grid_w, drel2d=parts[0], drel1d=parts[1], drelx=parts[2])
            hip.attn_dbias_grads(dbias, S, pos_q=pq, pos_k=pk, dpq_acc=dpq_acc, dpk_acc=dpk_acc, accumulate_pos=not first_pos,
                                 dpq_scale=scaling, causal=causal, **kw)
            tables = []
            if rel is not None:
                for (tabname, idx), part in zip(rel_grads, parts):
                    if tabname is not None:
                        tables.append((part, idx, self._table_acc(tabname)))
            hip.attn_bwd_reduce(B, H, T, S, C, None, None, dpq_acc, dpk_acc, True, dgr, ones, self.G(gain_name),
                                hip.dbias_nparts(), tables)
            if self.ctx.get("resized") and rel_grads is not None:
                self._resized_rel_grads(rel_grads, dbias, T)
        if "reduce" not in _EXP_SKIP:
            self._side_do(reductions)

    def _resized_rel_grads(self, rel_grads, dbias, T):
        cfg, ctx = self.cfg, self.ctx
        h, w, L = ctx["h"], ctx["w"], ctx["L"]
        names = []
        for n, _ in rel_grads:
            if n is not None and n not in names:
                names.append(n)
        dB = dbias[:, :, :, :T].float().sum(0)
        bufs = dict(self.model.named_buffers())
        if names[0].startswith("encoder."):
            img_n = [n for n in names if "image_rel" in n][0]
            tok_n = [n for n in names if "token_rel" in n][0]
            oh = cfg.orig_patch_image_size // 16
            fn = lambda tt, it: R.encoder_rel_bias(tt, it, bufs["encoder.token_rp_bucket"], bufs["encoder.image_rp_bucket"], (h, w), oh,
                                                   cfg.image_bucket_size, L)
            order = [tok_n, img_n]
        else:
            fn = lambda st: R.decoder_rel_bias(st, bufs["decoder.seg_rp_bucket"], (h, w), cfg.seg_bucket_size)
            order = names[:1]
        for n, gv in zip(order, R.table_grads(fn, [self.W(n) for n in order], dB)):
            self.G(n).copy_(gv)

    def _table_acc(self, tabname):
        key = "g_tabacc_" + tabname
        if key not in self.ws:
            names = sorted(n for n in self.shapes if "rel_pos_table_list" in n and self.offs[n] < self.n_train)
            assert tabname in names, tabname
            sizes = [(math.prod(self.shapes[n]) + 3) // 4 * 4 for n in names]
            flat = self.ws["g_tabacc_flat"] = torch.zeros(sum(sizes), dtype=torch.float32, device=self.device)
            o = 0
            for n, sz in zip(names, sizes):
                self.ws["g_tabacc_" + n] = flat[o:o + math.prod(self.shapes[n])].view(self.shapes[n])
                o += sz
        self._tab_touched.setdefault(key, tabname)
        return self.ws[key]

    def _tabacc_clear(self):
        flat = self.ws.get("g_tabacc_flat")
        if flat is not None:
            flat.zero_()

    def _self_block_bwd(self, tg, p, attn, ln1, ln2, dx1, B, T, pq, pk, scaling, dpq_acc, dpk_acc, first_pos, rel_grads,
                        da_pre=None, nxt=None):
        C = self.cfg.embed_dim
        s = self.saved[tg + "_sa"]
        W, Wf, G, buf = self.W, self.Wf, self.G, self.buf
        a_ = p + attn
        rows = B * T
        self._bt = tg + "s"
        gbuf = self.gbuf
        da = da_pre
        if da is None:
            da = gbuf("g_da_%d" % rows, (rows, C))
            drop = None
            if self.drop_on and s["site"] is not None:
                drop = self._dropargs(self._site_id(s["site"]), self._dp(*s["site"]), T)
            self._ln_bwd(dx1, s["a"], p + ln2, tg + "_ln2", da, drop=drop)
        do = buf("g_do_%d" % rows, (B, T, C))
        delta = self._out_proj_bwd(da, s["o"], a_, do, B, T)
        dqkv = gbuf("g_dqkv_%d" % rows, (B, T, 3 * C))
        qkv = s["qkv"]
        self._attn_core_bwd(tg, qkv[:, :, :C], qkv[:, :, C:2 * C], qkv[:, :, 2 * C:], pq, pk, s["o"], s["lse"], do,
                            dqkv[:, :, :C], dqkv[:, :, C:2 * C], dqkv[:, :, 2 * C:], B, T, T, s["rel"], s["causal"],
                            s["gain"], a_ + ".c_attn", scaling, dpq_acc, dpk_acc, first_pos, rel_grads, delta=delta,
                            dense=self.ctx.get("dense", {}).get(tg))
        dxn = buf("g_dxn_%d" % rows, (rows, C))
        self._linear_bwd(dqkv.view(rows, 3 * C), s["xn"], self._fused(self.p16, a_ + ".q_proj.weight", 3 * C, C),
                         self._fused(self.g16, a_ + ".q_proj.weight", 3 * C, C),
                         self._fused(self.g16, a_ + ".q_proj.bias", 3 * C), dx_out=dxn)
        if self.kproj_fix:
            self._kfix_tasks.append((G(a_ + ".k_proj.weight"), G(a_ + ".k_proj.bias"), s["xn"], tg))
        dx = gbuf("g_dx0_%d" % rows, (rows, C))
        self._ln_bwd_fused(dxn, s["x"].view(rows, C), p + ln1, tg + "_ln1", dx, dx1, nxt)
        return dx

    def _cross_block_bwd(self, tg, p, dy2, B, Td, Te, cpq, cpk, scaling, d_enc_out, first_cross, dcpq_acc, dcpk_acc,
                         da_pre=None, nxt=None):
        C = self.cfg.embed_dim
        s = self.saved[tg + "_ca"]
        W, Wf, G, buf = self.W, self.Wf, self.G, self.buf
        a_ = p + "encoder_attn"
        rows = B * Td
        self._bt = tg + "c"
        gbuf = self.gbuf
        da = da_pre
        if da is None:
            da = gbuf("g_da_%d" % rows, (rows, C))
            drop = None
            if self.drop_on and s["site"] is not None:
                drop = self._dropargs(self._site_id(s["site"]), self._dp(*s["site"]), Td)
            self._ln_bwd(dy2, s["a"], p + "cross_attn_ln", tg + "_cln2", da, drop=drop)
        do = buf("g_do_%d" % rows, (B, Td, C))
        delta = self._out_proj_bwd(da, s["o"], a_, do, B, Td)
        dq = gbuf("g_cdq", (B, Td, C))
        dkv = gbuf("g_cdkv", (B, Te, 2 * C))
        kv = s["kv"]
        self._attn_core_bwd(tg + "c", s["q"], kv[:, :, :C], kv[:, :, C:], cpq, cpk, s["o"], s["lse"], do, dq,
                            dkv[:, :, :C], dkv[:, :, C:], B, Td, Te, None, False, s["gain"], a_ + ".c_attn", scaling,
                            dcpq_acc, dcpk_acc, first_cross, None, delta=delta, dense=self.ctx.get("dense", {}).get("dc"))
        dyn = buf("g_dxn_%d" % rows, (rows, C))
        self._linear_bwd(dq.view(rows, C), s["xn"], W(a_ + ".q_proj.weight"), G(a_ + ".q_proj.weight"),
                         G(a_ + ".q_proj.bias"), dx_out=dyn)
        enc2d = self.ctx["enc_out"].view(B * Te, C)
        wkv = self._fused(self.p16, a_ + ".k_proj.weight", 2 * C, C)
        if self.overlap:
            self._side_do(lambda: self._linear_bwd(
                dkv.view(B * Te, 2 * C), enc2d, wkv, self._fused(self.g16, a_ + ".k_proj.weight", 2 * C, C),
                self._fused(self.g16, a_ + ".k_proj.bias", 2 * C), need_dx=False))
            with self._fork(self._dq_stream_get()):
                hip.linear_dx(dkv.view(B * Te, 2 * C), wkv, out=d_enc_out.view(B * Te, C), accumulate=not first_cross)
        else:
            self._linear_bwd(dkv.view(B * Te, 2 * C), enc2d, wkv, self._fused(self.g16, a_ + ".k_proj.weight", 2 * C, C),
                             self._fused(self.g16, a_ + ".k_proj.bias", 2 * C), dx_out=d_enc_out.view(B * Te, C),
                             dx_accumulate=not first_cross)
        if self.kproj_fix:
            self._kfix_tasks.append((G(a_ + ".k_proj.weight"), G(a_ + ".k_proj.bias"), enc2d, "enc_out"))
        dy1 = gbuf("g_dy1c_%d" % rows, (rows, C))
        self._ln_bwd_fused(dyn, s["x"].view(rows, C), p + "encoder_attn_layer_norm", tg + "_cln1", dy1, dy2, nxt)
        self._side_flush()
        return dy1

    def _backward(self, dlogits):
        cfg, ctx = self.cfg, self.ctx
        B, L, P, T, Td, h, w = (ctx[k] for k in ("B", "L", "P", "T", "Td", "h", "w"))
        C, H = cfg.embed_dim, cfg.heads
        scaling = float(cfg.head_dim * cfg.attn_scale_factor) ** -0.5
        W, Wf, G, buf = self.W, self.Wf, self.G, self.buf
        g = self._geometry(h, w, L)
        self.mark("bwd_start")
        if ctx.get("g16_zeroed") is not None:
            torch.cuda.current_stream().wait_event(ctx.pop("g16_zeroed"))
        else:
            self.g16.zero_()
        self._tab_touched = {}
        self._side_do(self._tabacc_clear)
        self._xsum_done = set()
        self._bt = "top"
        if ctx.get("dense_ready") is not None:
            torch.cuda.current_stream().wait_event(ctx["dense_ready"])
        e, d = "encoder.", "decoder."
        fresh = "g_dlogits" not in self.ws or self.ws["g_dlogits"].shape != (B * Td, self.npad)
        dl = buf("g_dlogits", (B * Td, self.npad))
        if fresh or _POISON:
            dl.zero_()
        dl.view(B, Td, self.npad)[:, :, : cfg.num_seg_tokens].copy_(dlogits)
        dfeat = buf("g_dfeat", (B, Td, C))
        hip.linear_dx(dl, self.wseg_pad, out=dfeat.view(B * Td, C))
        if self.train_seg:
            dwseg = buf("g_dwseg", (self.npad, C))
            hip.linear_dw(dl, self.ws["d_feat"].view(B * Td, C), dwseg)
            G("encoder.seg_embed_tokens.weight").copy_(dwseg[: cfg.num_seg_tokens])
        y = ctx["d_y_final"]
        dy = buf("g_dy_final", (B, Td, C))
        self._ln_bwd(dfeat[:, 1:], y[:, :P], d + "layer_norm", "d_final_ln_p", dy[:, :P])
        self._ln_bwd(dfeat[:, :1], y[:, P:], d + "layer_norm", "d_final_ln_b", dy[:, P:], accumulate=True)
        dy = dy.view(B * Td, C)
        d_enc_out = buf("g_d_enc_out", (B, T, C))
        dspq, dspk = buf("g_dspq", (Td, C), torch.float32), buf("g_dspk", (Td, C), torch.float32)
        dcpq, dcpk = buf("g_dcpq", (Td, C), torch.float32), buf("g_dcpk", (T, C), torch.float32)
        fuse = lab.get("NO_LN_BWD_DROP") is None
        dbr = None
        for l in reversed(range(cfg.dec_layers)):
            p = "%slayers.%d." % (d, l)
            tg = "d%d" % l
            first = l == cfg.dec_layers - 1
            nx_f = self._next_drop("d%d" % (l - 1), B * Td) if fuse and l > 0 else None
            dy = self._ffn_bwd(tg, p, dy, B * Td, dbr_pre=dbr)
            dy = self._cross_block_bwd(tg, p, dy, B, Td, T, ctx["d_cpq"], ctx["d_cpk"], scaling, d_enc_out, first, dcpq, dcpk)
            tabn = "%sseg_rel_pos_table_list.%d.weight" % (d, l)
            dy = self._self_block_bwd(tg, p, "self_attn", "self_attn_layer_norm", "self_attn_ln", dy, B, Td,
                                      ctx["d_spq"], ctx["d_spk"], scaling, dspq, dspk, first,
                                      [(tabn, g["dec_idx2d"]), (tabn, g["dec_idx1d"]), (tabn, g["dec_idxx"])], nxt=nx_f)
            dbr = nx_f["out"] if nx_f else None
            self._layer_end(p)
        self.mark("dec_bwd_end")
        self._bt = "dtop"
        if self.overlap and getattr(self, "_dqs", None) is not None:
            ev = self._ev()
            ev.record(self._dqs)
            torch.cuda.current_stream().wait_event(ev)
        dy3 = dy.view(B, Td, C)
        enc_out = ctx["enc_out"]
        dyp, dyb = dy3[:, :P], dy3[:, P:]
        self._ln_bwd(dyp, enc_out[:, :P], d + "layernorm_embedding", "d_emb_ln_p", d_enc_out[:, :P],
                     dx_add=d_enc_out[:, :P], drop=self._dropargs(3))
        scratch = buf("g_bos_scratch", (B, 1, C))
        self._ln_bwd(dyb, self.ws["d_bos"], d + "layernorm_embedding", "d_emb_ln_b", scratch, accumulate=True,
                     drop=self._dropargs(4))
        if self.train_tok:
            self._embed_grads(scratch.view(B, C), ctx["bos_ids"])
        pos_all = self.ws["e_pos_all"]
        dpos_all = buf("g_dpos_all", (T, C))
        self._side_do(lambda: self._dec_pos_bwd(B, P, T, Td, dspq, dspk, dcpq, dcpk, pos_all, dpos_all))
        self._side_flush()
        dx = buf("g_dx_enc", (B * T, C))
        self._ln_bwd(d_enc_out.view(B * T, C), ctx["e_x_final"].view(B * T, C), e + "layer_norm", "e_final_ln", dx)
        depq, depk = buf("g_depq", (T, C), torch.float32), buf("g_depk", (T, C), torch.float32)
        dbr = None
        for l in reversed(range(cfg.enc_layers)):
            p = "%slayers.%d." % (e, l)
            tg = "e%d" % l
            first = l == cfg.enc_layers - 1
            if self.trunk_at == "e%d" % l:
                self._trunk_launch_point()
            nx_f = self._next_drop("e%d" % (l - 1), B * T) if fuse and l > 0 else None
            dx = self._ffn_bwd(tg, p, dx, B * T, dbr_pre=dbr)
            dx = self._self_block_bwd(tg, p, "self_attn", "self_attn_layer_norm", "attn_ln", dx, B, T, ctx["e_pq"],
                                      ctx["e_pk"], scaling, depq, depk, first,
                                      [("%simage_rel_pos_table_list.%d.weight" % (e, l), g["enc_idx2d"]),
                                       ("%stoken_rel_pos_table_list.%d.weight" % (e, l), g["enc_idx1d"]),
                                       (None, None)], nxt=nx_f)
            dbr = nx_f["out"] if nx_f else None
            self._layer_end(p)
        self._bt = "etop"
        if "tailsplit" in _EXP_SKIP:
            self._side_do(lambda: (self._dw_flush(), self._enc_tail_pos_bwd(B, L, P, T, h, w, depq, depk, pos_all, dpos_all),
                                   self._enc_tail_emb_bwd(B, L, P, T, dx)))
        else:
            self._side_do(lambda: (self._dw_flush(wgs=0), self._enc_tail_pos_bwd(B, L, P, T, h, w, depq, depk, pos_all, dpos_all)))
            self._side_flush()
            self._enc_tail_emb_bwd(B, L, P, T, dx)
        if self.trunk_at == "end":
            self._trunk_launch_point()
        elif self.trunk_at == "fwd" and self._pf_request is not None and not torch.cuda.is_current_stream_capturing():
            req, self._pf_request = self._pf_request, None
            self._prefetch_request(req, at_end=True)
        if self.drain_timing is not None:
            t0 = torch.cuda.Event(enable_timing=True); t0.record()
        self.mark("bwd_main_end")
        self._join_side()
        self.mark("joined")
        if self.drain_timing is not None:
            t1 = torch.cuda.Event(enable_timing=True); t1.record()
            self.drain_timing.append((t0, t1))
        self._notify(e)
        return self.g16

    def _ffn_ln_coefs(self):
        cfg = self.cfg
        w2, gam, bet, b2, coef = [], [], [], [], []
        for kind, n in (("e", cfg.enc_layers), ("d", cfg.dec_layers)):
            for l in range(n):
                p = "%s.layers.%d." % ("encoder" if kind == "e" else "decoder", l)
                w2.append(self.W(p + "fc2.weight")); gam.append(self.Wf(p + "ffn_layernorm.weight"))
                bet.append(self.Wf(p + "ffn_layernorm.bias")); b2.append(self.W(p + "fc2.bias"))
                coef.append(self.buf("%s%d_fcoef" % (kind, l), (2, cfg.embed_dim), torch.float32))
        for i in range(0, len(w2), 32):
            hip.ffn_ln_coef(w2[i:i + 32], gam[i:i + 32], bet[i:i + 32], b2[i:i + 32], coef[i:i + 32])

    def _prefetch_request(self, req, at_end=False):
        if not isinstance(req, (list, tuple)):
            if not at_end:
                self.prefetch_trunk(req)
            return False
        cache = ([self._pf] if self._pf is not None else []) + (self._pf_more if self._pf is not None else [])
        covered = 0
        while covered < len(cache) and covered < len(req) and cache[covered]["key"] == self._tkey(req[covered]):
            covered += 1
        if covered < len(cache):
            covered = 0
            self._pf, self._pf_more = None, []
        if not at_end:
            if covered == 0:
                if req:
                    self.prefetch_trunk(list(req[: self.trunk_lookahead]))
                return False
            return self.trunk_lookahead > 1
        if covered <= 1 and len(req) > covered and self.trunk_lookahead > 1:
            self.prefetch_trunk(list(req[covered: covered + self.trunk_lookahead]), append=covered > 0)
        return False

    def _trunk_launch_point(self):
        if self._pf_request is not None and not torch.cuda.is_current_stream_capturing():
            req, self._pf_request = self._pf_request, None
            self._prefetch_request(req)

    def _enc_tail_pos_bwd(self, B, L, P, T, h, w, depq, depk, pos_all, dpos_all):
        cfg = self.cfg
        C = cfg.embed_dim
        W, Wf, G, buf = self.W, self.Wf, self.G, self.buf
        e = "encoder."
        depqk = buf("g_depqk", (T, 2 * C))
        tmp = buf("g_tmp_ec", (T, C))
        hip.cast_f32_bf16(depq, tmp); depqk[:, :C].copy_(tmp)
        hip.cast_f32_bf16(depk, tmp); depqk[:, C:].copy_(tmp)
        self._linear_bwd(depqk, pos_all, self._fused(self.p16, e + "pos_q_linear.weight", 2 * C, C),
                         self._fused(self.g16, e + "pos_q_linear.weight", 2 * C, C),
                         self._fused(self.g16, e + "pos_q_linear.bias", 2 * C), dx_out=dpos_all, dx_accumulate=True)
        bsz = cfg.image_bucket_size
        oh = cfg.orig_patch_image_size // 16
        if self.ctx.get("resized") and P > oh * oh:
            dipos = buf("g_dipos", (P, C))
            self._ln_bwd(dpos_all[:P], self.ws["e_ipos_resized"], e + "image_pos_ln", "ipos_ln", dipos)
            G(e + "embed_image_positions.weight")[1:1 + bsz * oh].view(oh, bsz, C)[:, :oh].copy_(
                R.rows_resize_adjoint(dipos, (oh, oh), (h, w)).view(oh, oh, C))
        else:
# ... 10 lines not shown
        C = cfg.embed_dim
        W, Wf, G, buf = self.W, self.Wf, self.G, self.buf
        e = "encoder."
        dx3 = dx.view(B, T, C)
        dxi, dxt = dx3[:, :P], dx3[:, P:]
        if self.ctx.get("nonpad") is not None:
            dxt.mul_(self.ctx["nonpad"].unsqueeze(-1).to(dxt.dtype))
        dimg = buf("g_dimg_pre", (B, P, C))
        self._ln_bwd(dxi, self.ws["img_pre"].view(B, P, C), e + "patch_layernorm_embedding", "img_ln", dimg,
                     drop=self._dropargs(1))
        dtok = buf("g_dtok_pre", (B, L, C))
        self._ln_bwd(dxt, self.ws["tok_pre"].view(B, L, C), e + "layernorm_embedding", "tok_ln", dtok,
                     drop=self._dropargs(2))
        gt = G(e + "type_embedding.weight")
        if self.train_tok:
            self._embed_grads(dtok.view(B * L, C), self.ctx["src_ids"])
        self._bias_grad(dtok.view(B * L, C), gt[0])
        self._bias_grad(dimg.view(B * P, C), gt[1])
        self._dw_flush()
        assert not self._ln_red_tasks and not self._ln_red_acc and not self._dw_tasks

    def _embed_grads(self, drows, ids):
        sid, perm = torch.sort(ids.reshape(-1), stable=True)
        hip.rows_segment_sum(drows, perm, None, sid, self.G("encoder.embed_tokens.weight"), skip_id=1)

    def _dec_pos_bwd(self, B, P, T, Td, dspq, dspk, dcpq, dcpk, pos_all, dpos_all):
        cfg = self.cfg
        C = cfg.embed_dim
        W, Wf, G, buf = self.W, self.Wf, self.G, self.buf
        d = "decoder."
        dspqk = buf("g_dspqk", (Td, 2 * C))
        hip.cast_f32_bf16(dspq, buf("g_tmp_tc", (Td, C)))
        dspqk[:, :C].copy_(self.ws["g_tmp_tc"])
        hip.cast_f32_bf16(dspk, self.ws["g_tmp_tc"])
        dspqk[:, C:].copy_(self.ws["g_tmp_tc"])
        tp = self.ws["d_tp"]
        dtp = buf("g_dtp", (Td, C))
        self._linear_bwd(dspqk, tp, self._fused(self.p16, d + "self_pos_q_linear.weight", 2 * C, C),
                         self._fused(self.g16, d + "self_pos_q_linear.weight", 2 * C, C),
                         self._fused(self.g16, d + "self_pos_q_linear.bias", 2 * C), dx_out=dtp)
        dcpq16 = buf("g_dcpq16", (Td, C))
        hip.cast_f32_bf16(dcpq, dcpq16)
        self._linear_bwd(dcpq16, tp, W(d + "cross_pos_q_linear.weight"), G(d + "cross_pos_q_linear.weight"),
                         G(d + "cross_pos_q_linear.bias"), dx_out=dtp, dx_accumulate=True)
        segG = G(d + "embed_seg_positions.weight")
        segtab = W(d + "embed_seg_positions.weight")
        if self.ctx.get("resized"):
            sb = cfg.seg_bucket_size
            tgt, dtgt = self.ws["d_spos_resized"], buf("g_dtgt", (Td, C))
            self._ln_bwd(dtp[:P], tgt[:P], d + "seg_pos_ln", "d_tp_ln_p", dtgt[:P])
            self._ln_bwd(dtp[P:], tgt[P:], d + "seg_pos_ln", "d_tp_ln_b", dtgt[P:], accumulate=True)
            segG[1:1 + sb * sb].copy_(R.rows_resize_adjoint(dtgt[:P], (sb, sb), (self.ctx["h"], self.ctx["w"])))
            segG[:1].copy_(dtgt[P:])
        else:
            self._ln_bwd(dtp[:P], segtab[1:1 + P], d + "seg_pos_ln", "d_tp_ln_p", segG[1:1 + P])
            self._ln_bwd(dtp[P:], segtab[:1], d + "seg_pos_ln", "d_tp_ln_b", segG[:1], accumulate=True)
        dcpk16 = buf("g_dcpk16", (T, C))
        hip.cast_f32_bf16(dcpk, dcpk16)
        self._linear_bwd(dcpk16, pos_all, W(d + "cross_pos_k_linear.weight"), G(d + "cross_pos_k_linear.weight"),
                         G(d + "cross_pos_k_linear.bias"), dx_out=dpos_all)
        self._dw_flush()
        self._side_do(lambda: self._notify(d))

    def _dw_flush(self, wgs=None):
        tasks, self._dw_tasks = self._dw_tasks, []
        if tasks and "dw" not in _EXP_SKIP:
            hip.linear_dw_group(tasks, wgs)
        kf, self._kfix_tasks = self._kfix_tasks, []
        for gw, gb, x, tag in kf:
            key = "g_xmean_" + tag
            if key not in self._xsum_done:
                hip.col_mean(x, self.buf(key, (hip.COLSUM_BLOCKS + 1, x.shape[-1]), torch.float32), every=8)
                self._xsum_done.add(key)
            hip.kproj_common_mode(gw, gb, self.ws[key][hip.COLSUM_BLOCKS])
        pg, self._ffn_pg_tasks = self._ffn_pg_tasks, []
        for w2, dw2, db2, gam, bet, dgam, dbet, dy_, u_, mu_, rs_ in pg:
            hip.ffn_ln_param_grads(w2, dw2, db2, gam, bet, dgam, dbet, dy=dy_, u=u_, mean=mu_, rstd=rs_)
        for attr in ("_ln_red_tasks", "_ln_red_acc"):
            red = getattr(self, attr)
            setattr(self, attr, [])
            if red:
                hip.reduce_parts_multi(red)

    def _layer_end(self, p):
        self._side_do(lambda: (self._flush_tables(), self._notify(p)))
        self._side_flush()

    def _flush_tables(self):
        self._dw_flush()
        for key, tabname in self._tab_touched.items():
            hip.cast_f32_bf16(self.ws[key].view(-1), self.G(tabname).view(-1))
        self._tab_touched = {}

    def _notify(self, prefix):
        if self.grad_ready_hook is not None:
            self.grad_ready_hook(prefix)
```

### include/ifseg_hip.h

```cpp
#ifndef IFSEG_HIP_H
#define IFSEG_HIP_H
#ifdef __cplusplus
extern "C" {
#endif

#define IFSEG_ABI_VERSION 21
#define IFSEG_ERR_BAD_SHAPE (-2)
#define IFSEG_ERR_BAD_ARG (-3)

int ifseg_abi_version(void);
int ifseg_experimental_build(void);

#define IFSEG_GEMM_NT 0
#define IFSEG_GEMM_NN 1
#define IFSEG_GEMM_TN 2
#define IFSEG_GEMM_RELU 1
#define IFSEG_GEMM_OUT_F32 2
#define IFSEG_GEMM_ACCUMULATE 4
#define IFSEG_GEMM_COLSUM 8

int ifseg_gemm_bf16(int layout, const void* A, const void* B, void* C, int M, int N, int K, int lda,
                    int ldb, int ldc, const void* bias, float alpha, int alpha_ncols,
                    const void* resid, int ldr, int flags, int batch, long long strideA,
                    long long strideB, long long strideC, long long strideR, int splitk, void* stream);
#define IFSEG_GEMM_GROUP_MAX 8
typedef struct {
  const void* A; const void* B; void* C;
  int M, N, K, lda, ldb, colsum, accumulate;
} ifseg_gemm_tn_problem;
int ifseg_gemm_tn_group(int n, const ifseg_gemm_tn_problem* probs, int max_workgroups, void* stream);
int ifseg_gemm_nn_rowdot(const void* A, const void* B, void* C, int M, int N, int K, int lda, int ldb, int ldc,
                         const void* dot, int ldd, float* dot_out, int rows_per_batch, void* stream);

int ifseg_ffn_ln_coef(const void* const* w2, int ldw, const float* const* gamma, const float* const* beta,
                      const void* const* b2 , float* const* coef ,
                      int L , int J, int N, void* stream);
int ifseg_ffn_ln_rowstats(const void* dy, int lddy, const void* t, int ldt, const float* coef, float* c ,
                          int rows, int J, int N, void* stream);
int ifseg_gemm_nn_gelu_ln_bwd(const void* A, const void* B, void* C, int M, int N, int K, int lda, int ldb, int ldc,
                              const void* u, int ldu, const float* gamma, const float* mean, const float* rstd,
                              const float* cstats, void* stream);
int ifseg_ffn_ln_param_grads(const void* w2, const void* dw2, const void* db2, const float* gamma, const float* beta,
                             void* dgamma, void* dbeta, float* workspace ,
                             int J, int N,
                             const void* dy, int lddy, const void* u, int ldu, const float* mean, const float* rstd, int M,
                             void* stream);

int ifseg_conv2d_nhwc_bf16(const void* in, const void* w, const void* shift, const void* resid,
                           void* out, int B, int H, int W, int Cin, int Cout, int KH, int KW,
                           int stride, int pad, int relu, void* stream);

int ifseg_attn_fwd(const void* q, const void* k, const void* v, const void* pos_q, const void* pos_k,
                   void* out, float* lse, int B, int H, int T, int S, int ldq, int ldk, int ldv, int ldo,
                   int ldpq, int ldpk, long long q_bs, long long k_bs, long long v_bs, long long o_bs,
                   int rel_mode, int P, const int* gcode, int code_bias, int n2d, const float* rel2d,
                   const float* rel1d, const float* relx, int causal, const float* dense_bias,
                   const void* gain ,
                   int grid_w ,
                   int dense_ld ,
                   void* stream);

typedef struct ifseg_attn_bwd_args {
  const void *q, *k, *v, *pos_q, *pos_k, *out, *dout;
  const float* lse;
  float* delta;
  void *dq, *dk, *dv;
  void *dpos_q_part, *dpos_k_part;
  int B, H, T, S;
  int ldq, ldk, ldv, ldpq, ldpk, ldout, lddo, lddq, lddk, lddv;
  long long q_bs, k_bs, v_bs, out_bs, do_bs, dq_bs, dk_bs, dv_bs;
  int rel_mode, P, code_bias, n2d, causal, nparts;
  const int* gcode;
  const float *rel2d, *rel1d, *relx;
  const void* gain;
  float *drel2d_part, *drel1d_part, *drelx_part;
  float dq_scale, dpq_scale;
  int grid_w;
  int phases;
  float* dgain_rows;
} ifseg_attn_bwd_args;
#define IFSEG_ATTN_BWD_DELTA 1
#define IFSEG_ATTN_BWD_DKV 2
#define IFSEG_ATTN_BWD_DQ 4
int ifseg_attn_bwd(const ifseg_attn_bwd_args* args, void* stream);

typedef struct ifseg_attn_reduce_args {
  int B, H, T, S, C, nparts, accumulate_pos;
  const void *dpos_q_part, *dpos_k_part;
  float *dpos_q_acc, *dpos_k_acc;
  const float* delta;
  const float* gain;
  void* dgain;
  int ntab;
  const float* tab_part[3];
  const int* tab_idx[3];
  float* tab_acc[3];
  int tab_n[3];
  int tab_nbucket[3];
} ifseg_attn_reduce_args;
int ifseg_attn_bwd_reduce(const ifseg_attn_reduce_args* args, void* stream);

int ifseg_attn_dense_bias(const void* pos_q, const void* pos_k, int ldpq, int ldpk, int H, int T, int S, int rel_mode,
                          int P, const int* gcode, int code_bias, int n2d, const float* rel2d, const float* rel1d,
                          const float* relx, int causal, void* D, int Sp, int Tp, void* stream);

typedef struct ifseg_attn_bi_args {
  const void *q, *k, *v, *dout;
  const float *lse, *delta;
  const void* D;
  const void* gain;
  void *dq, *dk, *dv, *dbias;
  int B, H, T, S, Sp, Tp;
  int ldq, ldk, ldv, lddo, lddq, lddk, lddv;
  long long q_bs, k_bs, v_bs, do_bs, dq_bs, dk_bs, dv_bs;
  int causal, P;
  float dq_scale;
  int phases;
  float* dgain_rows;
  void* out;
  int ldout; long long out_bs;
  const int* kv_len;
  float drop_p;
  unsigned long long drop_seed;
  const unsigned long long* drop_seed_add;
} ifseg_attn_bi_args;
int ifseg_attn_bwd_bi(const ifseg_attn_bi_args* args, void* stream);
int ifseg_attn_fwd_bi(const ifseg_attn_bi_args* args, void* stream);
int ifseg_attn_dropout_mask(unsigned char* keep, int B, int H, int T, int S, float p, unsigned long long seed,
                            const unsigned long long* seed_add, void* stream);

typedef struct ifseg_attn_dbias_args {
  const void* dbias;
  int ng, H, T, S, Sp, C;
  const void *pos_q, *pos_k;
  int ldpq, ldpk;
  float *dpos_q_acc, *dpos_k_acc;
  int accumulate_pos;
  float dpq_scale;
  int P, grid_h, grid_w;
  float *drel2d, *drel1d, *drelx;
  int causal;
} ifseg_attn_dbias_args;
int ifseg_attn_dbias_grads(const ifseg_attn_dbias_args* args, void* stream);
int ifseg_attn_dbias_nparts(void);

int ifseg_attn_bias_pack(const void* bias, int bias_is_f32, long long head_stride, long long row_stride, int H, int T, int S,
                         int causal, int P, void* D, int Sp, int Tp, void* stream);
int ifseg_attn_dbias_sum(const void* dbias, int ng, int H, int T, int S, int Sp, void* out, int out_is_f32,
                         long long head_stride, long long row_stride, void* stream);


typedef struct ifseg_drop_args {
  float p;
  unsigned long long seed;
  const float* drop_path_scale;
  int rows_per_batch;
  const unsigned long long* seed_add;
} ifseg_drop_args;
#define IFSEG_LN_GELU 1
#define IFSEG_LN_PARAMS_F32 2
int ifseg_ln_fwd(const void* x, const void* gamma, const void* beta, const void* resid, void* y, float* mean,
                 float* rstd, int rows, int C, float eps, int act_gelu, int rpb, long long x_bs, int ldx,
                 long long y_bs, int ldy, long long r_bs, int ldr, const ifseg_drop_args* drop, void* stream);
int ifseg_ln_fwd_pair(const void* x, const void* gamma, const void* beta, const void* resid, void* y, float* mean,
                      float* rstd, const void* gamma2, const void* beta2, void* y2, float* mean2, float* rstd2, int rows,
                      int C, float eps, int flags, int rpb, long long x_bs, int ldx, long long y_bs, int ldy, long long r_bs, int ldr,
                      long long y2_bs, int ldy2, const ifseg_drop_args* drop, void* stream);
int ifseg_ln_bwd(const void* dy, const void* x, const void* gamma, const float* mean, const float* rstd,
                 const void* dx_add, void* dx, float* dgamma_part, float* dbeta_part, int nblocks, int rows,
                 int C, int act_gelu, int rpb, long long dy_bs, int lddy, long long x_bs, int ldx,
                 long long dx_bs, int lddx, long long add_bs, int ldadd, const ifseg_drop_args* drop, void* stream);
int ifseg_ln_bwd_drop(const void* dy, const void* x, const void* gamma, const float* mean, const float* rstd,
                      const void* dx_add, void* dx, float* dgamma_part, float* dbeta_part, void* dx2, int nblocks, int rows,
                      int C, int flags, int rpb, long long dy_bs, int lddy, long long x_bs, int ldx, long long dx_bs, int lddx,
                      long long add_bs, int ldadd, long long dx2_bs, int lddx2, const ifseg_drop_args* drop2, void* stream);
int ifseg_check_inputs(const void* x, long long n, int mode, long long value, long long row_len,
                       unsigned char* verdict_host_pinned, void* stream);
int ifseg_sync_master(float* master, const void* p16, long long n, void* stream);
int ifseg_reduce_parts(const float* in, void* out, int outer, int parts, long long n, int accumulate,
                       int out_bf16, float scale, void* stream);
typedef struct ifseg_reduce_task {
  const float* in; void* out;
  int outer, parts; long long n;
  int accumulate, out_bf16; float scale;
} ifseg_reduce_task;
int ifseg_reduce_parts_multi(int ntask, const ifseg_reduce_task* tasks, void* stream);
int ifseg_colsum_bf16(const void* x, float* part, int nblk_rows, int M, int N, int rpb, long long x_bs, int ldx,
                      void* stream);
int ifseg_kproj_common_mode(void* gw, const void* db, const float* xmean, int N, int C, void* stream);
int ifseg_embed_rows(const void* table, const long long* ids, const void* add, void* out, int n, int C, int rpb,
                     long long o_bs, int ldo, void* stream);
int ifseg_rows_segment_sum(const void* src, const long long* src_row, const float* weight, const long long* sorted_ids,
                           void* table_grad, long long m, int C, long long V, long long skip_id, void* stream);
int ifseg_embed_bag_mean(const void* table, const long long* ids, const long long* ends, const void* add, void* out,
                         int B, int P, int C, int maxlen, int rpb, long long o_bs, int ldo, void* stream);
int ifseg_cast_f32_bf16(const float* in, void* out, long long n, float scale, void* stream);
int ifseg_add_bf16(const void* a, const void* b, void* out, long long n, void* stream);
int ifseg_nchw_to_nhwc_bf16(const void* in, int in_is_f32, void* out, int B, int C, int H, int W, int Cpad,
                            void* stream);

int ifseg_rel_gather(const void* table, const int* idx, float* out, int n, int H, void* stream);
int ifseg_rel_gather_multi(const void* const* tables, int L, const int* idx, float* out, int n, int H, void* stream);
int ifseg_rel_scatter_add(const float* d, const int* idx, float* acc, int n, int H, void* stream);

int ifseg_resized_rel_bias(float* out, const float* table2d, const float* rel1d, const float* relx, int H, int h, int w,
                           int oh, int ow, int Lt, int causal, int ld , void* stream);
int ifseg_resize_rows_bilinear(const void* src, void* dst, int C, int h, int w, int oh, int ow, int src_stride, int src_off,
                               int ld_src, void* stream);

int ifseg_dropout(const void* x, const void* resid, void* out, long long rows, int C, float p,
                  unsigned long long seed, const float* drop_path_scale, int rows_per_batch, int rpb, long long x_bs,
                  int ldx, long long r_bs, int ldr, long long o_bs, int ldo, const unsigned long long* seed_add, void* stream);
int ifseg_dropout_fill(const void* x, void* out, long long n, float p, unsigned long long seed,
                       const unsigned long long* seed_add, float fill, void* stream);
int ifseg_droppath_scale(float* out, const float* keep, int n, int B, unsigned long long seed,
                         const unsigned long long* seed_add, void* stream);

int ifseg_stem_conv7x7(const void* in_nhwc4, const float* w, const float* shift, void* out, int B, int H, int W,
                       void* stream);
int ifseg_stem_conv7x7_mfma(const void* in_nhwc4, const void* wt, const float* shift, void* out, int B, int H, int W,
                            void* stream);
int ifseg_maxpool3x3s2(const void* in, void* out, int B, int H, int W, int C, void* stream);

int ifseg_seg_loss_tiles(const void* logits, int ldl, long long logits_bs, const long long* target,
                         long long target_bs, int B, int hp, int wp, int H, int W, int nseg,
                         long long seg_id_offset, long long pad_id, long long eos_id, float* tile_partial,
// ... 113 lines not shown
```

Baseline: 500.4 images/sec.

## Batch per-layer attention side kernels into grouped multi-task launches

Adds grouped variants of the dense-bias build, dbias-gradient and backward-reduce kernels. Each variant takes up to eight layer tasks in one launch, using block-offset dispatch or an in-kernel loop over tasks that shares the running position-gradient accumulator. The Python side queues per-layer side tasks by kind and flushes them in groups, deferring layer-end notifications until a flush. This cuts launch count and host enqueue overhead on the side stream, at the cost of delaying gradient availability, more complex ordering, and a dbias kernel that now loops serially over tasks.

```diff
diff --git a/ifseg_amd/csrc/attention.hip b/ifseg_amd/csrc/attention.hip
--- a/ifseg_amd/csrc/attention.hip
+++ b/ifseg_amd/csrc/attention.hip
@@ -1254,9 +1254,16 @@
 namespace {
 constexpr int SMALL_TAB_MAX = 2048;
 struct ReduceArgs { ifseg_attn_reduce_args a; int nbq, nbk, nbt[3]; };
-__global__ __launch_bounds__(256) void attn_bwd_reduce_kernel(ReduceArgs r) {
+struct ReduceGroupArgs {
+  int n, start[IFSEG_ATTN_SIDE_GROUP_MAX + 1];
+  ReduceArgs t[IFSEG_ATTN_SIDE_GROUP_MAX];
+};
+__global__ __launch_bounds__(256) void attn_bwd_reduce_kernel(ReduceGroupArgs ga) {
+  int task = 0;
+  for (int i = 1; i < ga.n; ++i) task = ((int)blockIdx.x >= ga.start[i]) ? i : task;
+  const ReduceArgs& r = ga.t[task];
   const ifseg_attn_reduce_args& a = r.a;
-  int blk = blockIdx.x;
+  int blk = (int)blockIdx.x - ga.start[task];
   const int tid = threadIdx.x;
   if (blk < r.nbq + r.nbk) {
     const bool isq = blk < r.nbq;
@@ -1370,24 +1377,37 @@
 }
 }
 
-extern "C" int ifseg_attn_bwd_reduce(const ifseg_attn_reduce_args* x, void* stream) {
+extern "C" int ifseg_attn_bwd_reduce_group(int n, const ifseg_attn_reduce_args* tasks, void* stream) {
   (void)hipGetLastError();
-  if (!x || x->B <= 0 || x->H <= 0 || x->T <= 0 || x->S <= 0 || (x->C & 7) || x->ntab < 0 || x->ntab > 3) return IFSEG_ERR_BAD_ARG;
-  ReduceArgs r{};
-  r.a = *x;
-  r.nbq = x->dpos_q_part ? (int)(((long long)x->T * x->C / 8 + 255) / 256) : 0;
-  r.nbk = x->dpos_k_part ? (int)(((long long)x->S * x->C / 8 + 255) / 256) : 0;
-  long long total = (long long)r.nbq + r.nbk + x->H;
-  for (int t = 0; t < x->ntab; ++t) {
-    if (!x->tab_part[t] || !x->tab_idx[t] || !x->tab_acc[t] || x->tab_n[t] <= 0 || x->nparts <= 0) return IFSEG_ERR_BAD_ARG;
-    if (x->tab_nbucket[t] <= 0) return IFSEG_ERR_BAD_ARG;
-    r.nbt[t] = x->tab_n[t] <= SMALL_TAB_MAX ? x->H : x->H * ((x->tab_n[t] + 31) / 32);
-    total += r.nbt[t];
-  }
-  if ((x->dgain && (!x->delta || !x->gain)) || total >= (1ll << 31)) return IFSEG_ERR_BAD_ARG;
-  hipLaunchKernelGGL(attn_bwd_reduce_kernel, dim3((unsigned)total), dim3(256), 0, (hipStream_t)stream, r);
+  if (n <= 0 || n > IFSEG_ATTN_SIDE_GROUP_MAX || !tasks) return IFSEG_ERR_BAD_ARG;
+  ReduceGroupArgs ga{};
+  ga.n = n;
+  long long total = 0;
+  for (int i = 0; i < n; ++i) {
+    const ifseg_attn_reduce_args* x = &tasks[i];
+    if (x->B <= 0 || x->H <= 0 || x->T <= 0 || x->S <= 0 || (x->C & 7) || x->ntab < 0 || x->ntab > 3) return IFSEG_ERR_BAD_ARG;
+    ReduceArgs& r = ga.t[i];
+    r.a = *x;
+    r.nbq = x->dpos_q_part ? (int)(((long long)x->T * x->C / 8 + 255) / 256) : 0;
+    r.nbk = x->dpos_k_part ? (int)(((long long)x->S * x->C / 8 + 255) / 256) : 0;
+    ga.start[i] = (int)total;
+    total += (long long)r.nbq + r.nbk + x->H;
+    for (int t = 0; t < x->ntab; ++t) {
+      if (!x->tab_part[t] || !x->tab_idx[t] || !x->tab_acc[t] || x->tab_n[t] <= 0 || x->nparts <= 0) return IFSEG_ERR_BAD_ARG;
+      if (x->tab_nbucket[t] <= 0) return IFSEG_ERR_BAD_ARG;
+      r.nbt[t] = x->tab_n[t] <= SMALL_TAB_MAX ? x->H : x->H * ((x->tab_n[t] + 31) / 32);
+      total += r.nbt[t];
+    }
+    if ((x->dgain && (!x->delta || !x->gain)) || total >= (1ll << 31)) return IFSEG_ERR_BAD_ARG;
+  }
+  for (int i = n; i <= IFSEG_ATTN_SIDE_GROUP_MAX; ++i) ga.start[i] = (int)total;
+  hipLaunchKernelGGL(attn_bwd_reduce_kernel, dim3((unsigned)total), dim3(256), 0, (hipStream_t)stream, ga);
   IFSEG_CHECK_LAUNCH();
   return 0;
+}
+
+extern "C" int ifseg_attn_bwd_reduce(const ifseg_attn_reduce_args* x, void* stream) {
+  return ifseg_attn_bwd_reduce_group(1, x, stream);
 }
 
 static int attn_check(const AttnArgs& a) {
diff --git a/ifseg_amd/csrc/attention_bi.hip b/ifseg_amd/csrc/attention_bi.hip
--- a/ifseg_amd/csrc/attention_bi.hip
+++ b/ifseg_amd/csrc/attention_bi.hip
@@ -716,15 +716,28 @@
   const float *rel2d, *rel1d, *relx;
   bf16_t* D;
 };
-
-__global__ __launch_bounds__(512) void attn_dense_bias_kernel(DenseArgs a) {
+constexpr int SIDE_GROUP_MAX = IFSEG_ATTN_SIDE_GROUP_MAX;
+__device__ __forceinline__ int side_task(const int* start, int n, int bid) {
+  int task = 0;
+  for (int i = 1; i < n; ++i) task = (bid >= start[i]) ? i : task;
+  return task;
+}
+struct DenseGroupArgs {
+  int n, start[SIDE_GROUP_MAX + 1];
+  DenseArgs t[SIDE_GROUP_MAX];
+};
+
+__global__ __launch_bounds__(512) void attn_dense_bias_kernel(DenseGroupArgs ga) {
+  const int task = side_task(ga.start, ga.n, (int)blockIdx.x);
+  const DenseArgs& a = ga.t[task];
+  const int bid = (int)blockIdx.x - ga.start[task];
   extern __shared__ __attribute__((aligned(16))) unsigned char smem[];
   float* sT = reinterpret_cast<float*>(smem);
   float* s1 = sT + ((a.n2d + 3) & ~3);
   int* sG = reinterpret_cast<int*>(s1 + ((2 * a.Lt + 2) & ~3));
   const int tid = threadIdx.x, lane = tid & 63, wave = tid >> 6, half = lane >> 5, x = lane & 31;
   const int ntq = a.Tp >> 5, ntk = a.Sp >> 5;
-  const int h = blockIdx.x / ntq, ti = blockIdx.x % ntq, i0 = ti * 32;
+  const int h = bid / ntq, ti = bid % ntq, i0 = ti * 32;
   float rx0 = 0.f, rx1 = 0.f;
   if (a.rel_mode) {
     for (int i = tid; i < a.n2d; i += 512) sT[i] = a.rel2d[(long long)h * a.n2d + i];
@@ -817,87 +830,126 @@
   return f.b;
 }
 
-__global__ __launch_bounds__(256) void attn_dbias_grads_kernel(DbArgs a) {
+struct DbTask {
+  const bf16_t *dbias, *pq, *pk;
+  float dpq_scale;
+  int ng;
+};
+struct DbGradsArgs {
+  DbArgs a;
+  int n;
+  DbTask t[SIDE_GROUP_MAX];
+};
+struct DbTabArgs {
+  int n, start[SIDE_GROUP_MAX + 1];
+  DbArgs t[SIDE_GROUP_MAX];
+};
+
+__global__ __launch_bounds__(256, 3) void attn_dbias_grads_kernel(DbGradsArgs ga) {
   __shared__ __attribute__((aligned(16))) unsigned char sm[32768];
+  const DbArgs& a = ga.a;
   const int tid = threadIdx.x, lane = tid & 63, half = lane >> 5;
   const int wave = __builtin_amdgcn_readfirstlane(tid >> 6);
   int blk = blockIdx.x < a.nb_q ? xcd_remap(blockIdx.x, a.nb_q) : a.nb_q + xcd_remap(blockIdx.x - a.nb_q, a.nb_k);
   const int lr = lane >> 3, lc = lane & 7;
+  float run[2][4];
   if (blk < a.nb_q) {
     const int nit = (a.T + 31) >> 5;
     const int h = blk / nit, i0 = (blk % nit) * 32;
-    const int i = i0 + (lane & 31);
-    const int ir = i < a.T ? i : a.T - 1;
     unsigned char* tile = sm + wave * 8192;
-    f32x16 acc[2];
-#pragma unroll
-    for (int e = 0; e < 16; ++e) { acc[0][e] = 0.f; acc[1][e] = 0.f; }
+    auto outp = [&](int cb, int k) -> float* {
+      const int v = tid + 256 * k, r = v >> 6, ln = v & 63;
+      const int c = cb * 32 + (r & 3) + 8 * (r >> 2) + 4 * (ln >> 5), ii = i0 + (ln & 31);
+      return ii < a.T ? a.dpq + (long long)ii * a.C + h * 64 + c : nullptr;
+    };
+#pragma unroll
+    for (int cb = 0; cb < 2; ++cb)
+#pragma unroll
+      for (int k = 0; k < 4; ++k) {
+        const float* p = outp(cb, k);
+        run[cb][k] = (a.accumulate && p) ? *p : 0.f;
+      }
     uint4 t4[4], d4[4];
-    auto fetch = [&](int j0) {
+    auto fetch = [&](int n, int j0) {
+      const DbTask& t = ga.t[n];
 #pragma unroll
       for (int u = 0; u < 4; ++u) {
         t4[u] = make_uint4(0, 0, 0, 0); d4[u] = make_uint4(0, 0, 0, 0);
-        if (j0 + lr + 8 * u < a.S) t4[u] = *reinterpret_cast<const uint4*>(a.pk + (long long)(j0 + lr + 8 * u) * a.ldpk + h * 64 + lc * 8);
+        if (j0 + lr + 8 * u < a.S) t4[u] = *reinterpret_cast<const uint4*>(t.pk + (long long)(j0 + lr + 8 * u) * a.ldpk + h * 64 + lc * 8);
         const int g = lc >> 2, irow = min(i0 + lr + 8 * u, a.T - 1);
-        if (g < a.ng) d4[u] = *reinterpret_cast<const uint4*>(a.dbias + g * a.gs + ((long long)h * a.T + irow) * a.Sp + j0 + (lc & 3) * 8);
+        if (g < t.ng) d4[u] = *reinterpret_cast<const uint4*>(t.dbias + g * a.gs + ((long long)h * a.T + irow) * a.Sp + j0 + (lc & 3) * 8);
       }
     };
     auto live = [&](int j) { return !(a.causal && j < a.P && (i0 >= a.P || j > i0 + 31)); };
-    int j0 = wave * 32;
-    if (j0 < a.Sp) fetch(j0);
-    for (; j0 < a.Sp; j0 += 128) {
-      if (!live(j0)) { if (j0 + 128 < a.Sp) fetch(j0 + 128); continue; }
-      __builtin_amdgcn_wave_barrier();
-#pragma unroll
-      for (int u = 0; u < 4; ++u) {
-        const int o = vx_off(lr + 8 * u, lc * 16);
-        *reinterpret_cast<uint4*>(tile + o) = t4[u];
-        *reinterpret_cast<uint4*>(tile + 4096 + o) = d4[u];
-      }
-      __builtin_amdgcn_fence(__ATOMIC_RELEASE, "wavefront");
-      __builtin_amdgcn_wave_barrier();
-      if (j0 + 128 < a.Sp) fetch(j0 + 128);
-      U128 bfr[2][2];
-#pragma unroll
-      for (int s2 = 0; s2 < 2; ++s2)
-#pragma unroll
-        for (int g = 0; g < 2; ++g) {
-          const int cb = g * 64 + (16 * s2 + 4 * half) * 2;
-          const uint2 lo = *reinterpret_cast<const uint2*>(tile + 4096 + vx_off(lane & 31, cb));
-          const uint2 hi = *reinterpret_cast<const uint2*>(tile + 4096 + vx_off(lane & 31, cb + 16));
-          bfr[s2][g].w[0] = lo.x; bfr[s2][g].w[1] = lo.y; bfr[s2][g].w[2] = hi.x; bfr[s2][g].w[3] = hi.y;
+    if (wave * 32 < a.Sp) fetch(0, wave * 32);
+    for (int n = 0; n < ga.n; ++n) {
+      const int ng = ga.t[n].ng;
+      f32x16 acc[2];
+#pragma unroll
+      for (int e = 0; e < 16; ++e) { acc[0][e] = 0.f; acc[1][e] = 0.f; }
+      for (int j0 = wave * 32; j0 < a.Sp; j0 += 128) {
+        auto next = [&]() {
+          if (j0 + 128 < a.Sp) fetch(n, j0 + 128);
+          else if (n + 1 < ga.n) fetch(n + 1, wave * 32);
+        };
+        if (!live(j0)) { next(); continue; }
+        __builtin_amdgcn_wave_barrier();
+#pragma unroll
+        for (int u = 0; u < 4; ++u) {
+          const int o = vx_off(lr + 8 * u, lc * 16);
+          *reinterpret_cast<uint4*>(tile + o) = t4[u];
+          *reinterpret_cast<uint4*>(tile + 4096 + o) = d4[u];
         }
-#pragma unroll
-      for (int s2 = 0; s2 < 2; ++s2) {
-        const bf16x8 a0 = tr_frag(tile, 16 * s2, 0, lane), a1 = tr_frag(tile, 16 * s2, 1, lane);
-#pragma unroll
-        for (int g = 0; g < 2; ++g)
-          if (g < a.ng) {
-            acc[0] = __builtin_amdgcn_mfma_f32_32x32x16_bf16(a0, bfr[s2][g].b, acc[0], 0, 0, 0);
-            acc[1] = __builtin_amdgcn_mfma_f32_32x32x16_bf16(a1, bfr[s2][g].b, acc[1], 0, 0, 0);
+        __builtin_amdgcn_fence(__ATOMIC_RELEASE, "wavefront");
+        __builtin_amdgcn_wave_barrier();
+        next();
+        U128 bfr[2][2];
+#pragma unroll
+        for (int s2 = 0; s2 < 2; ++s2)
+#pragma unroll
+          for (int g = 0; g < 2; ++g) {
+            const int cb = g * 64 + (16 * s2 + 4 * half) * 2;
+            const uint2 lo = *reinterpret_cast<const uint2*>(tile + 4096 + vx_off(lane & 31, cb));
+            const uint2 hi = *reinterpret_cast<const uint2*>(tile + 4096 + vx_off(lane & 31, cb + 16));
+            bfr[s2][g].w[0] = lo.x; bfr[s2][g].w[1] = lo.y; bfr[s2][g].w[2] = hi.x; bfr[s2][g].w[3] = hi.y;
           }
-      }
-      __builtin_amdgcn_wave_barrier();
-    }
-    __syncthreads();
-    float* red = reinterpret_cast<float*>(sm);
-#pragma unroll
-    for (int cb = 0; cb < 2; ++cb) {
-      if (cb) __syncthreads();
-#pragma unroll
-      for (int r = 0; r < 16; ++r) red[(wave * 16 + r) * 64 + lane] = acc[cb][r];
+#pragma unroll
+        for (int s2 = 0; s2 < 2; ++s2) {
+          const bf16x8 a0 = tr_frag(tile, 16 * s2, 0, lane), a1 = tr_frag(tile, 16 * s2, 1, lane);
+#pragma unroll
+          for (int g = 0; g < 2; ++g)
+            if (g < ng) {
+              acc[0] = __builtin_amdgcn_mfma_f32_32x32x16_bf16(a0, bfr[s2][g].b, acc[0], 0, 0, 0);
+              acc[1] = __builtin_amdgcn_mfma_f32_32x32x16_bf16(a1, bfr[s2][g].b, acc[1], 0, 0, 0);
+            }
+        }
+        __builtin_amdgcn_wave_barrier();
+      }
       __syncthreads();
+      float* red = reinterpret_cast<float*>(sm);
+      const float scale = ga.t[n].dpq_scale;
+#pragma unroll
+      for (int cb = 0; cb < 2; ++cb) {
+        if (cb) __syncthreads();
+#pragma unroll
+        for (int r = 0; r < 16; ++r) red[(wave * 16 + r) * 64 + lane] = acc[cb][r];
+        __syncthreads();
+#pragma unroll
+        for (int k = 0; k < 4; ++k) {
+          const int v = tid + 256 * k, r = v >> 6, ln = v & 63;
+          const float t = (red[r * 64 + ln] + red[(16 + r) * 64 + ln]) + (red[(32 + r) * 64 + ln] + red[(48 + r) * 64 + ln]);
+          run[cb][k] = run[cb][k] + t * scale;
+        }
+      }
+      if (n + 1 < ga.n) __syncthreads();
+    }
+#pragma unroll
+    for (int cb = 0; cb < 2; ++cb)
 #pragma unroll
       for (int k = 0; k < 4; ++k) {
-        const int v = tid + 256 * k, r = v >> 6, ln = v & 63;
-        const float t = (red[r * 64 + ln] + red[(16 + r) * 64 + ln]) + (red[(32 + r) * 64 + ln] + red[(48 + r) * 64 + ln]);
-        const int c = cb * 32 + (r & 3) + 8 * (r >> 2) + 4 * (ln >> 5), ii = i0 + (ln & 31);
-        if (ii < a.T) {
-          float* p = a.dpq + (long long)ii * a.C + h * 64 + c;
-          *p = (a.accumulate ? *p : 0.f) + t * a.dpq_scale;
-        }
-      }
-    }
+        float* p = outp(cb, k);
+        if (p) *p = run[cb][k];
+      }
     return;
   }
   blk -= a.nb_q;
@@ -905,76 +957,102 @@
     const int njt = a.Sp >> 5;
     const int h = blk / njt, jw0 = (blk % njt) * 32;
     unsigned char* sQ = sm + wave * 8192;
-    f32x16 acc[2];
-#pragma unroll
-    for (int e = 0; e < 16; ++e) { acc[0][e] = 0.f; acc[1][e] = 0.f; }
+    auto outp = [&](int cb, int k) -> float* {
+      const int v = tid + 256 * k, r = v >> 6, ln = v & 63;
+      const int c = cb * 32 + (r & 3) + 8 * (r >> 2) + 4 * (ln >> 5), j = jw0 + (ln & 31);
+      return j < a.S ? a.dpk + (long long)j * a.C + h * 64 + c : nullptr;
+    };
+#pragma unroll
+    for (int cb = 0; cb < 2; ++cb)
+#pragma unroll
+      for (int k = 0; k < 4; ++k) {
+        const float* p = outp(cb, k);
+        run[cb][k] = (a.accumulate && p) ? *p : 0.f;
+      }
     uint4 t4[4], d4[4];
-    auto fetch = [&](int i0) {
+    auto fetch = [&](int n, int i0) {
+      const DbTask& t = ga.t[n];
 #pragma unroll
       for (int u = 0; u < 4; ++u) {
         const int r = lr + 8 * u;
         t4[u] = make_uint4(0, 0, 0, 0); d4[u] = make_uint4(0, 0, 0, 0);
         if (i0 + r < a.T) {
-          t4[u] = *reinterpret_cast<const uint4*>(a.pq + (long long)(i0 + r) * a.ldpq + h * 64 + lc * 8);
+          t4[u] = *reinterpret_cast<const uint4*>(t.pq + (long long)(i0 + r) * a.ldpq + h * 64 + lc * 8);
           const int g = lc >> 2;
-          if (g < a.ng) d4[u] = *reinterpret_cast<const uint4*>(a.dbias + g * a.gs + ((long long)h * a.T + i0 + r) * a.Sp + jw0 + (lc & 3) * 8);
+          if (g < t.ng) d4[u] = *reinterpret_cast<const uint4*>(t.dbias + g * a.gs + ((long long)h * a.T + i0 + r) * a.Sp + jw0 + (lc & 3) * 8);
         }
       }
     };
     auto live = [&](int i) { return !(a.causal && jw0 < a.P && (i >= a.P || jw0 > i + 31)); };
-    int i0 = wave * 32;
-    if (i0 < a.T) fetch(i0);
-    for (; i0 < a.T; i0 += 128) {
-      if (!live(i0)) { if (i0 + 128 < a.T) fetch(i0 + 128); continue; }
-      __builtin_amdgcn_wave_barrier();
-#pragma unroll
-      for (int u = 0; u < 4; ++u) {
-        const int o = vx_off(lr + 8 * u, lc * 16);
-        *reinterpret_cast<uint4*>(sQ + o) = t4[u];
-        *reinterpret_cast<uint4*>(sQ + 4096 + o) = d4[u];
-      }
-      __builtin_amdgcn_fence(__ATOMIC_RELEASE, "wavefront");
-      __builtin_amdgcn_wave_barrier();
-      if (i0 + 128 < a.T) fetch(i0 + 128);
-#pragma unroll
-      for (int s2 = 0; s2 < 2; ++s2) {
-        const bf16x8 a0 = tr_frag(sQ, 16 * s2, 0, lane), a1 = tr_frag(sQ, 16 * s2, 1, lane);
-#pragma unroll
-        for (int g = 0; g < 2; ++g)
-          if (g < a.ng) {
-            const bf16x8 bfr = tr_frag(sQ + 4096, 16 * s2, g, lane);
-            acc[0] = __builtin_amdgcn_mfma_f32_32x32x16_bf16(a0, bfr, acc[0], 0, 0, 0);
-            acc[1] = __builtin_amdgcn_mfma_f32_32x32x16_bf16(a1, bfr, acc[1], 0, 0, 0);
-          }
-      }
-      __builtin_amdgcn_wave_barrier();
-    }
-    __syncthreads();
-    float* red = reinterpret_cast<float*>(sm);
-#pragma unroll
-    for (int cb = 0; cb < 2; ++cb) {
-      if (cb) __syncthreads();
-#pragma unroll
-      for (int r = 0; r < 16; ++r) red[(wave * 16 + r) * 64 + lane] = acc[cb][r];
+    if (wave * 32 < a.T) fetch(0, wave * 32);
+    for (int n = 0; n < ga.n; ++n) {
+      const int ng = ga.t[n].ng;
+      f32x16 acc[2];
+#pragma unroll
+      for (int e = 0; e < 16; ++e) { acc[0][e] = 0.f; acc[1][e] = 0.f; }
+      for (int i0 = wave * 32; i0 < a.T; i0 += 128) {
+        auto next = [&]() {
+          if (i0 + 128 < a.T) fetch(n, i0 + 128);
+          else if (n + 1 < ga.n) fetch(n + 1, wave * 32);
+        };
+        if (!live(i0)) { next(); continue; }
+        __builtin_amdgcn_wave_barrier();
+#pragma unroll
+        for (int u = 0; u < 4; ++u) {
+          const int o = vx_off(lr + 8 * u, lc * 16);
+          *reinterpret_cast<uint4*>(sQ + o) = t4[u];
+          *reinterpret_cast<uint4*>(sQ + 4096 + o) = d4[u];
+        }
+        __builtin_amdgcn_fence(__ATOMIC_RELEASE, "wavefront");
+        __builtin_amdgcn_wave_barrier();
+        next();
+#pragma unroll
+        for (int s2 = 0; s2 < 2; ++s2) {
+          const bf16x8 a0 = tr_frag(sQ, 16 * s2, 0, lane), a1 = tr_frag(sQ, 16 * s2, 1, lane);
+#pragma unroll
+          for (int g = 0; g < 2; ++g)
+            if (g < ng) {
+              const bf16x8 bfr = tr_frag(sQ + 4096, 16 * s2, g, lane);
+              acc[0] = __builtin_amdgcn_mfma_f32_32x32x16_bf16(a0, bfr, acc[0], 0, 0, 0);
+              acc[1] = __builtin_amdgcn_mfma_f32_32x32x16_bf16(a1, bfr, acc[1], 0, 0, 0);
+            }
+        }
+        __builtin_amdgcn_wave_barrier();
+      }
       __syncthreads();
+      float* red = reinterpret_cast<float*>(sm);
+#pragma unroll
+      for (int cb = 0; cb < 2; ++cb) {
+        if (cb) __syncthreads();
+#pragma unroll
+        for (int r = 0; r < 16; ++r) red[(wave * 16 + r) * 64 + lane] = acc[cb][r];
+        __syncthreads();
+#pragma unroll
+        for (int k = 0; k < 4; ++k) {
+          const int v = tid + 256 * k, r = v >> 6, ln = v & 63;
+          const float t = (red[r * 64 + ln] + red[(16 + r) * 64 + ln]) + (red[(32 + r) * 64 + ln] + red[(48 + r) * 64 + ln]);
+          run[cb][k] = run[cb][k] + t;
+        }
+      }
+      if (n + 1 < ga.n) __syncthreads();
+    }
+#pragma unroll
+    for (int cb = 0; cb < 2; ++cb)
 #pragma unroll
       for (int k = 0; k < 4; ++k) {
-        const int v = tid + 256 * k, r = v >> 6, ln = v & 63;
-        const float t = (red[r * 64 + ln] + red[(16 + r) * 64 + ln]) + (red[(32 + r) * 64 + ln] + red[(48 + r) * 64 + ln]);
-        const int c = cb * 32 + (r & 3) + 8 * (r >> 2) + 4 * (ln >> 5), j = jw0 + (ln & 31);
-        if (j < a.S) {
-          float* p = a.dpk + (long long)j * a.C + h * 64 + c;
-          *p = (a.accumulate ? *p : 0.f) + t;
-        }
-      }
-    }
-  }
-}
-
-__global__ __launch_bounds__(256) void attn_dbias_tables_kernel(DbArgs a) {
+        float* p = outp(cb, k);
+        if (p) *p = run[cb][k];
+      }
+  }
+}
+
+__global__ __launch_bounds__(256) void attn_dbias_tables_kernel(DbTabArgs ga) {
   __shared__ __attribute__((aligned(16))) float sf[2 * 4096];
   const int tid = threadIdx.x;
-  int blk = blockIdx.x < a.nb_2d ? xcd_remap(blockIdx.x, a.nb_2d) : blockIdx.x;
+  const int task = side_task(ga.start, ga.n, (int)blockIdx.x);
+  const DbArgs& a = ga.t[task];
+  const int bid = (int)blockIdx.x - ga.start[task];
+  int blk = bid < a.nb_2d ? xcd_remap(bid, a.nb_2d) : bid;
   auto add8 = [](float* t, const uint4& v) {
     t[0] += bflo(v.x); t[1] += bfhi(v.x); t[2] += bflo(v.y); t[3] += bfhi(v.y);
     t[4] += bflo(v.z); t[5] += bfhi(v.z); t[6] += bflo(v.w); t[7] += bfhi(v.w);
@@ -1121,27 +1199,56 @@
 
 }
 
+static int dense_task_args(const ifseg_attn_dense_task& x, DenseArgs* out, size_t* lds_out) {
+  if (!x.D || x.H <= 0 || x.T <= 0 || x.S <= 0 || (x.Sp & 31) || (x.Tp & 31) || x.Sp < x.S || x.Tp < x.T) return IFSEG_ERR_BAD_ARG;
+  if ((x.pos_q == nullptr) != (x.pos_k == nullptr) || ((x.ldpq | x.ldpk) & 7)) return IFSEG_ERR_BAD_ARG;
+  if (x.rel_mode && (!x.gcode || !x.rel2d || !x.rel1d || !x.relx)) return IFSEG_ERR_BAD_ARG;
+  if ((x.rel_mode || x.causal) && (x.P > x.T || x.P > x.S || x.P < 0)) return IFSEG_ERR_BAD_SHAPE;
+  DenseArgs a{};
+  a.pq = (const bf16_t*)x.pos_q; a.pk = (const bf16_t*)x.pos_k; a.ldpq = x.ldpq; a.ldpk = x.ldpk;
+  a.H = x.H; a.T = x.T; a.S = x.S; a.Sp = x.Sp; a.Tp = x.Tp;
+  a.rel_mode = x.rel_mode; a.P = (x.rel_mode || x.causal) ? x.P : x.S; a.code_bias = x.code_bias; a.n2d = x.rel_mode ? x.n2d : 0;
+  a.Lt = x.rel_mode ? x.T - x.P : 0; a.causal = x.causal;
+  a.gcode = x.gcode; a.rel2d = x.rel2d; a.rel1d = x.rel1d; a.relx = x.relx; a.D = (bf16_t*)x.D;
+  if ((size_t)x.D & 15) return IFSEG_ERR_BAD_ARG;
+  const size_t lds = x.rel_mode ? ((((size_t)x.n2d + 3) & ~(size_t)3) + (((size_t)2 * a.Lt + 2) & ~(size_t)3) + (size_t)x.P) * 4 : 16;
+  if (lds > 160 * 1024) return IFSEG_ERR_BAD_SHAPE;
+  *out = a; *lds_out = lds;
+  return 0;
+}
+
+extern "C" int ifseg_attn_dense_bias_group(int n, const ifseg_attn_dense_task* tasks, void* stream) {
+  (void)hipGetLastError();
+  if (n <= 0 || n > SIDE_GROUP_MAX || !tasks) return IFSEG_ERR_BAD_ARG;
+  DenseGroupArgs ga{};
+  ga.n = n;
+  size_t lds = 16;
+  long long total = 0;
+  for (int i = 0; i < n; ++i) {
+    size_t l = 0;
+    const int rc = dense_task_args(tasks[i], &ga.t[i], &l);
+    if (rc) return rc;
+    lds = l > lds ? l : lds;
+    ga.start[i] = (int)total;
+    total += (long long)ga.t[i].H * (ga.t[i].Tp / 32);
+    if (total >= (1ll << 31)) return IFSEG_ERR_BAD_SHAPE;
+  }
+  for (int i = n; i <= SIDE_GROUP_MAX; ++i) ga.start[i] = (int)total;
+  if (lds > 64 * 1024) (void)hipFuncSetAttribute((const void*)attn_dense_bias_kernel, hipFuncAttributeMaxDynamicSharedMemorySize, (int)lds);
+  hipLaunchKernelGGL(attn_dense_bias_kernel, dim3((unsigned)total), dim3(512), lds, (hipStream_t)stream, ga);
+  IFSEG_CHECK_LAUNCH();
+  return 0;
+}
+
 extern "C" int ifseg_attn_dense_bias(const void* pos_q, const void* pos_k, int ldpq, int ldpk, int H, int T, int S,
                                      int rel_mode, int P, const int* gcode, int code_bias, int n2d, const float* rel2d,
                                      const float* rel1d, const float* relx, int causal, void* D, int Sp, int Tp,
                                      void* stream) {
-  (void)hipGetLastError();
-  if (!D || H <= 0 || T <= 0 || S <= 0 || (Sp & 31) || (Tp & 31) || Sp < S || Tp < T) return IFSEG_ERR_BAD_ARG;
-  if ((pos_q == nullptr) != (pos_k == nullptr) || ((ldpq | ldpk) & 7)) return IFSEG_ERR_BAD_ARG;
-  if (rel_mode && (!gcode || !rel2d || !rel1d || !relx)) return IFSEG_ERR_BAD_ARG;
-  if ((rel_mode || causal) && (P > T || P > S || P < 0)) return IFSEG_ERR_BAD_SHAPE;
-  DenseArgs a{};
-  a.pq = (const bf16_t*)pos_q; a.pk = (const bf16_t*)pos_k; a.ldpq = ldpq; a.ldpk = ldpk;
-  a.H = H; a.T = T; a.S = S; a.Sp = Sp; a.Tp = Tp;
-  a.rel_mode = rel_mode; a.P = (rel_mode || causal) ? P : S; a.code_bias = code_bias; a.n2d = rel_mode ? n2d : 0; a.Lt = rel_mode ? T - P : 0; a.causal = causal;
-  a.gcode = gcode; a.rel2d = rel2d; a.rel1d = rel1d; a.relx = relx; a.D = (bf16_t*)D;
-  if ((size_t)D & 15) return IFSEG_ERR_BAD_ARG;
-  const size_t lds = rel_mode ? ((((size_t)n2d + 3) & ~(size_t)3) + (((size_t)2 * a.Lt + 2) & ~(size_t)3) + (size_t)P) * 4 : 16;
-  if (lds > 160 * 1024) return IFSEG_ERR_BAD_SHAPE;
-  if (lds > 64 * 1024) (void)hipFuncSetAttribute((const void*)attn_dense_bias_kernel, hipFuncAttributeMaxDynamicSharedMemorySize, (int)lds);
-  hipLaunchKernelGGL(attn_dense_bias_kernel, dim3((unsigned)(H * (Tp / 32))), dim3(512), lds, (hipStream_t)stream, a);
-  IFSEG_CHECK_LAUNCH();
-  return 0;
+  ifseg_attn_dense_task t{};
+  t.pos_q = pos_q; t.pos_k = pos_k; t.ldpq = ldpq; t.ldpk = ldpk; t.H = H; t.T = T; t.S = S; t.rel_mode = rel_mode; t.P = P;
+  t.gcode = gcode; t.code_bias = code_bias; t.n2d = n2d; t.rel2d = rel2d; t.rel1d = rel1d; t.relx = relx; t.causal = causal;
+  t.D = D; t.Sp = Sp; t.Tp = Tp;
+  return ifseg_attn_dense_bias_group(1, &t, stream);
 }
 
 extern "C" int ifseg_attn_bwd_bi(const ifseg_attn_bi_args* x, void* stream) {
@@ -1226,8 +1333,7 @@
   return 0;
 }
 
-extern "C" int ifseg_attn_dbias_grads(const ifseg_attn_dbias_args* x, void* stream) {
-  (void)hipGetLastError();
+static int dbias_task_args(const ifseg_attn_dbias_args* x, DbArgs* out) {
   if (!x || !x->dbias || x->ng <= 0 || x->H <= 0 || x->T <= 0 || x->S <= 0 || (x->Sp & 31) || x->Sp < x->S)
     return IFSEG_ERR_BAD_ARG;
   DbArgs a{};
@@ -1248,16 +1354,68 @@
   a.nb_q = pos ? a.H * ((a.T + 31) / 32) : 0;
   a.nb_k = pos ? a.H * (a.Sp / 32) : 0;
   a.nb_2d = rel ? a.H * (2 * a.gh - 1) * DB_NPARTS : 0;
-  const int ng_all = x->ng;
-  for (int g0 = 0; g0 < ng_all; g0 += 2) {
-    a.dbias = (const bf16_t*)x->dbias + (long long)g0 * a.gs;
-    a.ng = ng_all - g0 < 2 ? ng_all - g0 : 2;
-    if (g0) { a.accumulate = 1; a.tab_accumulate = 1; }
-    if (pos) hipLaunchKernelGGL(attn_dbias_grads_kernel, dim3(a.nb_q + a.nb_k), dim3(256), 0, (hipStream_t)stream, a);
-    if (rel) hipLaunchKernelGGL(attn_dbias_tables_kernel, dim3(a.nb_2d + a.H * DB_NPARTS * (1 + DB_NSUB)), dim3(256), 0, (hipStream_t)stream, a);
+  *out = a;
+  return 0;
+}
+
+extern "C" int ifseg_attn_dbias_grads_group(int n, const ifseg_attn_dbias_args* tasks, void* stream) {
+  (void)hipGetLastError();
+  if (n <= 0 || n > SIDE_GROUP_MAX || !tasks) return IFSEG_ERR_BAD_ARG;
+  DbArgs t[SIDE_GROUP_MAX];
+  int npos = 0, max_ng = 0;
+  for (int i = 0; i < n; ++i) {
+    const int rc = dbias_task_args(&tasks[i], &t[i]);
+    if (rc) return rc;
+    npos += t[i].pq != nullptr;
+    max_ng = t[i].ng > max_ng ? t[i].ng : max_ng;
+  }
+  if (npos) {
+    if (npos != n) return IFSEG_ERR_BAD_ARG;
+    const DbArgs& f = t[0];
+    for (int i = 1; i < n; ++i)
+      if (t[i].H != f.H || t[i].T != f.T || t[i].S != f.S || t[i].Sp != f.Sp || t[i].C != f.C || t[i].ldpq != f.ldpq || t[i].ldpk != f.ldpk ||
+          t[i].P != f.P || t[i].causal != f.causal || t[i].dpq != f.dpq || t[i].dpk != f.dpk)
+        return IFSEG_ERR_BAD_ARG;
+    DbGradsArgs ga{};
+    ga.a = f;
+    bool launched = false;
+    for (int i = 0; i < n; ++i)
+      for (int g0 = 0; g0 < t[i].ng; g0 += 2) {
+        DbTask& u = ga.t[ga.n++];
+        u.dbias = t[i].dbias + (long long)g0 * f.gs; u.pq = t[i].pq; u.pk = t[i].pk; u.dpq_scale = t[i].dpq_scale;
+        u.ng = t[i].ng - g0 < 2 ? t[i].ng - g0 : 2;
+        if (ga.n == SIDE_GROUP_MAX || (i == n - 1 && g0 + 2 >= t[i].ng)) {
+          if (launched) ga.a.accumulate = 1;
+          hipLaunchKernelGGL(attn_dbias_grads_kernel, dim3(f.nb_q + f.nb_k), dim3(256), 0, (hipStream_t)stream, ga);
+          launched = true;
+          ga.n = 0;
+        }
+      }
+  }
+  for (int g0 = 0; g0 < max_ng; g0 += 2) {
+    DbTabArgs ta{};
+    long long total = 0;
+    for (int i = 0; i < n; ++i) {
+      if (!t[i].drel2d || g0 >= t[i].ng) continue;
+      DbArgs& u = ta.t[ta.n];
+      u = t[i];
+      u.dbias = t[i].dbias + (long long)g0 * u.gs;
+      u.ng = t[i].ng - g0 < 2 ? t[i].ng - g0 : 2;
+      u.tab_accumulate = g0 ? 1 : 0;
+      ta.start[ta.n++] = (int)total;
+      total += (long long)u.nb_2d + (long long)u.H * DB_NPARTS * (1 + DB_NSUB);
+      if (total >= (1ll << 31)) return IFSEG_ERR_BAD_SHAPE;
+    }
+    if (!ta.n) continue;
+    for (int i = ta.n; i <= SIDE_GROUP_MAX; ++i) ta.start[i] = (int)total;
+    hipLaunchKernelGGL(attn_dbias_tables_kernel, dim3((unsigned)total), dim3(256), 0, (hipStream_t)stream, ta);
   }
   IFSEG_CHECK_LAUNCH();
   return 0;
+}
+
+extern "C" int ifseg_attn_dbias_grads(const ifseg_attn_dbias_args* x, void* stream) {
+  return ifseg_attn_dbias_grads_group(1, x, stream);
 }
 
 extern "C" int ifseg_attn_dbias_nparts(void) { return DB_NPARTS; }
diff --git a/ifseg_amd/hip.py b/ifseg_amd/hip.py
--- a/ifseg_amd/hip.py
+++ b/ifseg_amd/hip.py
@@ -371,6 +371,41 @@
     return dense
 
 
+SIDE_GROUP_MAX = 8
+
+
+def _chunks(tasks, arg_type):
+    for i in range(0, len(tasks), SIDE_GROUP_MAX):
+        part = tasks[i:i + SIDE_GROUP_MAX]
+        arr = (arg_type * len(part))()
+        yield part, arr
+
+
+class _AttnDenseTask(ctypes.Structure):
+    _fields_ = [("pos_q", c_void_p), ("pos_k", c_void_p), ("ldpq", c_int), ("ldpk", c_int), ("H", c_int), ("T", c_int), ("S", c_int),
+                ("rel_mode", c_int), ("P", c_int), ("gcode", c_void_p), ("code_bias", c_int), ("n2d", c_int),
+                ("rel2d", c_void_p), ("rel1d", c_void_p), ("relx", c_void_p), ("causal", c_int), ("D", c_void_p),
+                ("Sp", c_int), ("Tp", c_int)]
+
+
+def attn_dense_bias_group(tasks):
+    for part, arr in _chunks(tasks, _AttnDenseTask):
+        for a, (dense, pos_q, pos_k, rel, causal, P) in zip(arr, part):
+            if rel is not None:
+                P = rel.P
+            if P is None:
+                P = dense.S
+            a.pos_q, a.pos_k = _p(pos_q), _p(pos_k)
+            a.ldpq = pos_q.stride(0) if pos_q is not None else 0
+            a.ldpk = pos_k.stride(0) if pos_k is not None else 0
+            a.H, a.T, a.S, a.Sp, a.Tp, a.D = dense.H, dense.T, dense.S, dense.Sp, dense.Tp, _p(dense.D)
+            a.rel_mode, a.P, a.causal = (1 if rel is not None else 0), P, (1 if causal else 0)
+            if rel is not None:
+                a.gcode, a.code_bias, a.n2d = _p(rel.gcode), rel.code_bias, rel.rel2d.shape[1]
+                a.rel2d, a.rel1d, a.relx = _p(rel.rel2d), _p(rel.rel1d), _p(rel.relx)
+        _check(lib().ifseg_attn_dense_bias_group(c_int(len(part)), arr, _stream()), "attn_dense_bias_group")
+
+
 class _AttnBiArgs(ctypes.Structure):
     _fields_ = ([(n, c_void_p) for n in ("q", "k", "v", "dout", "lse", "delta", "D", "gain", "dq", "dk", "dv", "dbias")]
                 + [(n, c_int) for n in ("B", "H", "T", "S", "Sp", "Tp", "ldq", "ldk", "ldv", "lddo", "lddq", "lddk", "lddv")]
@@ -445,11 +480,10 @@
                 ("drel2d", c_void_p), ("drel1d", c_void_p), ("drelx", c_void_p), ("causal", c_int)]
 
 
-def attn_dbias_grads(dbias, S, pos_q=None, pos_k=None, dpq_acc=None, dpk_acc=None, accumulate_pos=False, dpq_scale=1.0,
-                     P=0, grid_h=0, grid_w=0, drel2d=None, drel1d=None, drelx=None, causal=False):
+def _dbias_args(a, dbias, S, pos_q=None, pos_k=None, dpq_acc=None, dpk_acc=None, accumulate_pos=False, dpq_scale=1.0,
+                P=0, grid_h=0, grid_w=0, drel2d=None, drel1d=None, drelx=None, causal=False):
     if drel2d is not None:
         assert all(t.shape[1] == dbias_nparts() and t.is_contiguous() for t in (drel2d, drel1d, drelx))
-    a = _AttnDbiasArgs()
     ng, H, T, Sp = dbias.shape
     a.dbias, a.ng, a.H, a.T, a.S, a.Sp = _p(dbias), ng, H, T, S, Sp
     a.C = dpq_acc.shape[1] if dpq_acc is not None else 0
@@ -461,7 +495,23 @@
     a.P, a.grid_h, a.grid_w = P, grid_h, grid_w
     a.drel2d, a.drel1d, a.drelx = _p(drel2d), _p(drel1d), _p(drelx)
     a.causal = 1 if causal else 0
+
+
+def attn_dbias_grads(dbias, S, **kw):
+    a = _AttnDbiasArgs()
+    _dbias_args(a, dbias, S, **kw)
     _check(lib().ifseg_attn_dbias_grads(ctypes.byref(a), _stream()), "attn_dbias_grads")
+
+
+def attn_dbias_grads_group(tasks):
+    first = True
+    for part, arr in _chunks(tasks, _AttnDbiasArgs):
+        for a, kw in zip(arr, part):
+            _dbias_args(a, **kw)
+        if not first:
+            arr[0].accumulate_pos = 1
+        first = False
+        _check(lib().ifseg_attn_dbias_grads_group(c_int(len(part)), arr, _stream()), "attn_dbias_grads_group")
 
 
 def attn_bias_pack(dense, bias, causal=False, P=None):
@@ -827,9 +877,8 @@
                 ("tab_nbucket", c_int * 3)]
 
 
-def attn_bwd_reduce(B, H, T, S, C, dpq_part, dpk_part, dpq_acc, dpk_acc, accumulate_pos, delta, gain, dgain, nparts, tables):
+def _reduce_args(a, B, H, T, S, C, dpq_part, dpk_part, dpq_acc, dpk_acc, accumulate_pos, delta, gain, dgain, nparts, tables):
     assert all(t is None or t.dtype == torch.bfloat16 for t in (dpq_part, dpk_part)), "abs-pos partials are bf16"
-    a = _AttnReduceArgs()
     a.B, a.H, a.T, a.S, a.C, a.nparts, a.accumulate_pos = B, H, T, S, C, nparts, 1 if accumulate_pos else 0
     a.dpos_q_part, a.dpos_k_part, a.dpos_q_acc, a.dpos_k_acc = _p(dpq_part), _p(dpk_part), _p(dpq_acc), _p(dpk_acc)
     a.delta, a.gain, a.dgain = _p(delta), _p(_f32(gain)), _p(dgain)
@@ -837,7 +886,20 @@
     for i, (part, idx, acc) in enumerate(tables):
         assert part.dtype == torch.float32 and acc.dtype == torch.float32 and idx.dtype == torch.int32 and acc.shape[1] == H
         a.tab_part[i], a.tab_idx[i], a.tab_acc[i], a.tab_n[i], a.tab_nbucket[i] = _p(part), _p(idx), _p(acc), idx.numel(), acc.shape[0]
+
+
+def attn_bwd_reduce(*args):
+    a = _AttnReduceArgs()
+    _reduce_args(a, *args)
     _check(lib().ifseg_attn_bwd_reduce(ctypes.byref(a), _stream()), "attn_bwd_reduce")
+
+
+def attn_bwd_reduce_group(tasks):
+    for part, arr in _chunks(tasks, _AttnReduceArgs):
+        for a, args in zip(arr, part):
+            assert args[11] is None or args[11].dtype == torch.float32, "grouped reductions take fp32 gains"
+            _reduce_args(a, *args)
+        _check(lib().ifseg_attn_bwd_reduce_group(c_int(len(part)), arr, _stream()), "attn_bwd_reduce_group")
 
 
 def rel_scatter_add(d, idx, acc):
diff --git a/ifseg_amd/models/segofa/engine.py b/ifseg_amd/models/segofa/engine.py
--- a/ifseg_amd/models/segofa/engine.py
+++ b/ifseg_amd/models/segofa/engine.py
@@ -1,6 +1,7 @@
 import contextlib
 import math
 import os
+import re
 import time
 
 import torch
@@ -63,6 +64,8 @@
         self._train_fwd = False
         self.trunk_at = lab.get("TRUNK_AT", "fwd")
         self._bt = ""
+        self.side_group, self.side_group_enc, self.dense_group = 1, None, 1
+        self._sg, self._sg_held = {}, []
 
     def _arena_order(self):
         cfg = self.cfg
@@ -361,13 +364,28 @@
             torch.cuda.current_stream().wait_event(e)
 
     def _dense_bias(self, tag, H, T, S, pq, pk, rel, causal, P):
+        d = self._dense_buf(tag, H, T, S)
+        hip.attn_dense_bias(d, pq, pk, rel=rel, causal=causal, P=P)
+        return d
+
+    def _dense_buf(self, tag, H, T, S):
         key = "dense_" + tag
         d = self.ws.get(key)
         if d is None or (d.H, d.T, d.S) != (H, T, S):
             d = hip.DenseBias(H, T, S, self.device)
             self.ws[key] = d
-        hip.attn_dense_bias(d, pq, pk, rel=rel, causal=causal, P=P)
         return d
+
+    def _dense_group(self, ctx, tasks):
+        per = 1 if self.dense_group == 1 else hip.SIDE_GROUP_MAX
+        for i in range(0, len(tasks), per):
+            part = tasks[i:i + per]
+            launch = []
+            for tag, H, T, S, pq, pk, rel, causal, P in part:
+                d = ctx["dense"][tag] = self._dense_buf(tag, H, T, S)
+                launch.append((d, pq, pk, rel, causal, P))
+            hip.attn_dense_bias_group(launch)
+            self._dense_built(ctx, [t[0] for t in part])
 
     def _dense_from(self, tag, H, T, S, bias):
         key = "dense_" + tag
@@ -379,15 +397,17 @@
         d.D[:, :T, :S].copy_(bias)
         return d
 
-    def _dense_built(self, ctx, tag):
+    def _dense_built(self, ctx, tags):
         if not self.overlap:
             return
+        tags = [tags] if isinstance(tags, str) else tags
         evs = self.__dict__.setdefault("_dense_evs", {})
-        ev = evs.get(tag)
+        ev = evs.get(tags[0])
         if ev is None:
-            ev = evs[tag] = torch.cuda.Event()
+            ev = evs[tags[0]] = torch.cuda.Event()
         ev.record(self._side)
-        ctx.setdefault("dense_ev", {})[tag] = ev
+        for tag in tags:
+            ctx.setdefault("dense_ev", {})[tag] = ev
 
     def _dense_wait(self, tag):
         ev = self.ctx_building.get("dense_ev", {}).pop(tag, None)
@@ -874,10 +894,9 @@
                     self._dense_built(ctx, "e%d" % l)
         elif bi and "e" in bi_which:
             with self._wgrad():
-                for l in range(cfg.enc_layers):
-                    rel = hip.RelBias(P, g["gcode"], g["code_bias"], e_r2[l], e_r1[l], e_rx[l], grid_w=w)
-                    ctx["dense"]["e%d" % l] = self._dense_bias("e%d" % l, H, T, T, ctx["e_pq"], ctx["e_pk"], rel, False, P)
-                    self._dense_built(ctx, "e%d" % l)
+                self._dense_group(ctx, [("e%d" % l, H, T, T, ctx["e_pq"], ctx["e_pk"],
+                                         hip.RelBias(P, g["gcode"], g["code_bias"], e_r2[l], e_r1[l], e_rx[l], grid_w=w), False, P)
+                                        for l in range(cfg.enc_layers)])
         if need_grad and bi and self.overlap and not self._popt:
             self._dec_pos_dense(ctx, g, pos_all, scaling, bi, bi_which, resized)
         if need_grad and self.overlap and not torch.cuda.is_current_stream_capturing() and "g16fwd" not in _EXP_SKIP:
@@ -1021,16 +1040,16 @@
                     ctx["dense_ready"] = self._dense_ev
         elif bi:
             with self._wgrad():
+                tasks = []
                 for l in range(cfg.dec_layers if "d" in bi_which else 0):
                     rel = hip.RelBias(P, g["gcode"], g["code_bias"], d_r2[l], d_r1[l], d_rx[l], grid_w=w)
-                    ctx["dense"]["d%d" % l] = self._dense_bias("d%d" % l, H, Td, Td, ctx["d_spq"], ctx["d_spk"], rel, causal, P)
-                    self._dense_built(ctx, "d%d" % l)
+                    tasks.append(("d%d" % l, H, Td, Td, ctx["d_spq"], ctx["d_spk"], rel, causal, P))
                     if l == 0 and "c" in bi_which:
-                        ctx["dense"]["dc"] = self._dense_bias("dc", H, Td, T, cpq, cpk, None, False, None)
-                        self._dense_built(ctx, "dc")
-                if "c" in bi_which and "dc" not in ctx["dense"]:
-                    ctx["dense"]["dc"] = self._dense_bias("dc", H, Td, T, cpq, cpk, None, False, None)
-                    self._dense_built(ctx, "dc")
+                        tasks.append(("dc", H, Td, T, cpq, cpk, None, False, None))
+                if "c" in bi_which and not any(t[0] == "dc" for t in tasks):
+                    tasks.append(("dc", H, Td, T, cpq, cpk, None, False, None))
+                if tasks:
+                    self._dense_group(ctx, tasks)
                 if self.overlap:
                     if getattr(self, "_dense_ev", None) is None:
                         self._dense_ev = torch.cuda.Event()
@@ -1504,23 +1523,45 @@
             parts = [gbuf("g_relg%d_%d" % (i, t.shape[1]), (H, hip.dbias_nparts(), t.shape[1]), torch.float32)
                      for i, t in enumerate((rel.rel2d, rel.rel1d, rel.relx))]
 
-        def reductions():
-            kw = {}
-            if rel is not None:
-                kw = dict(P=rel.P, grid_h=rel.P // rel.grid_w, grid_w=rel.grid_w, drel2d=parts[0], drel1d=parts[1], drelx=parts[2])
-            hip.attn_dbias_grads(dbias, S, pos_q=pq, pos_k=pk, dpq_acc=dpq_acc, dpk_acc=dpk_acc, accumulate_pos=not first_pos,
-                                 dpq_scale=scaling, causal=causal, **kw)
+        kw = {}
+        if rel is not None:
+            kw = dict(P=rel.P, grid_h=rel.P // rel.grid_w, grid_w=rel.grid_w, drel2d=parts[0], drel1d=parts[1], drelx=parts[2])
+        grads = dict(dbias=dbias, S=S, pos_q=pq, pos_k=pk, dpq_acc=dpq_acc, dpk_acc=dpk_acc, accumulate_pos=not first_pos,
+                     dpq_scale=scaling, causal=causal, **kw)
+
+        def reduce_args():
             tables = []
             if rel is not None:
                 for (tabname, idx), part in zip(rel_grads, parts):
                     if tabname is not None:
                         tables.append((part, idx, self._table_acc(tabname)))
-            hip.attn_bwd_reduce(B, H, T, S, C, None, None, dpq_acc, dpk_acc, True, dgr, ones, self.G(gain_name),
-                                hip.dbias_nparts(), tables)
-            if self.ctx.get("resized") and rel_grads is not None:
-                self._resized_rel_grads(rel_grads, dbias, T)
-        if "reduce" not in _EXP_SKIP:
+            return (B, H, T, S, C, None, None, dpq_acc, dpk_acc, True, dgr, ones, self.G(gain_name), hip.dbias_nparts(), tables)
+        if "reduce" in _EXP_SKIP:
+            return
+        task = (grads, reduce_args)
+        kind = re.sub(r"layers\.\d+\.", "", gain_name)
+        per = self.side_group_enc if (kind.startswith("encoder.") and self.side_group_enc is not None) else self.side_group
+        if per == 1 or not self.overlap or self.ctx.get("resized"):
+            def reductions():
+                self._side_tasks([task])
+                if self.ctx.get("resized") and rel_grads is not None:
+                    self._resized_rel_grads(rel_grads, dbias, T)
             self._side_do(reductions)
+            return
+        todo = self._sg.setdefault(kind, [])
+        todo.append(task)
+        if len(todo) >= (per if per > 0 else hip.SIDE_GROUP_MAX):
+            self._sg_flush(kind)
+
+    def _side_tasks(self, tasks):
+        hip.attn_dbias_grads_group([grads for grads, _ in tasks])
+        hip.attn_bwd_reduce_group([reduce_args() for _, reduce_args in tasks])
+
+    def _sg_flush(self, kind=None):
+        for k in ([kind] if kind is not None else list(self._sg)):
+            tasks = self._sg.pop(k, None)
+            if tasks:
+                self._side_do(lambda tasks=tasks: self._side_tasks(tasks))
 
     def _resized_rel_grads(self, rel_grads, dbias, T):
         cfg, ctx = self.cfg, self.ctx
@@ -1656,6 +1697,7 @@
         else:
             self.g16.zero_()
         self._tab_touched = {}
+        self._sg, self._sg_held = {}, []
         self._side_do(self._tabacc_clear)
         self._xsum_done = set()
         self._bt = "top"
@@ -1695,7 +1737,7 @@
                                       ctx["d_spq"], ctx["d_spk"], scaling, dspq, dspk, first,
                                       [(tabn, g["dec_idx2d"]), (tabn, g["dec_idx1d"]), (tabn, g["dec_idxx"])], nxt=nx_f)
             dbr = nx_f["out"] if nx_f else None
-            self._layer_end(p)
+            self._layer_end(p, last=l == 0)
         self.mark("dec_bwd_end")
         self._bt = "dtop"
         if self.overlap and getattr(self, "_dqs", None) is not None:
@@ -1734,7 +1776,7 @@
                                        ("%stoken_rel_pos_table_list.%d.weight" % (e, l), g["enc_idx1d"]),
                                        (None, None)], nxt=nx_f)
             dbr = nx_f["out"] if nx_f else None
-            self._layer_end(p)
+            self._layer_end(p, last=l == 0)
         self._bt = "etop"
         if "tailsplit" in _EXP_SKIP:
             self._side_do(lambda: (self._dw_flush(), self._enc_tail_pos_bwd(B, L, P, T, h, w, depq, depk, pos_all, dpos_all),
@@ -1911,8 +1953,15 @@
             if red:
                 hip.reduce_parts_multi(red)
 
-    def _layer_end(self, p):
-        self._side_do(lambda: (self._flush_tables(), self._notify(p)))
+    def _layer_end(self, p, last=False):
+        if last:
+            self._sg_flush()
+        self._sg_held.append(p)
+        if any(self._sg.values()):
+            self._side_do(self._dw_flush)
+        else:
+            held, self._sg_held = self._sg_held, []
+            self._side_do(lambda: (self._flush_tables(), [self._notify(q) for q in held]))
         self._side_flush()
 
     def _flush_tables(self):
diff --git a/include/ifseg_hip.h b/include/ifseg_hip.h
--- a/include/ifseg_hip.h
+++ b/include/ifseg_hip.h
@@ -99,10 +99,23 @@
   int tab_nbucket[3];
 } ifseg_attn_reduce_args;
 int ifseg_attn_bwd_reduce(const ifseg_attn_reduce_args* args, void* stream);
+#define IFSEG_ATTN_SIDE_GROUP_MAX 8
+int ifseg_attn_bwd_reduce_group(int n, const ifseg_attn_reduce_args* tasks, void* stream);
 
 int ifseg_attn_dense_bias(const void* pos_q, const void* pos_k, int ldpq, int ldpk, int H, int T, int S, int rel_mode,
                           int P, const int* gcode, int code_bias, int n2d, const float* rel2d, const float* rel1d,
                           const float* relx, int causal, void* D, int Sp, int Tp, void* stream);
+typedef struct ifseg_attn_dense_task {
+  const void *pos_q, *pos_k;
+  int ldpq, ldpk, H, T, S, rel_mode, P;
+  const int* gcode;
+  int code_bias, n2d;
+  const float *rel2d, *rel1d, *relx;
+  int causal;
+  void* D;
+  int Sp, Tp;
+} ifseg_attn_dense_task;
+int ifseg_attn_dense_bias_group(int n, const ifseg_attn_dense_task* tasks, void* stream);
 
 typedef struct ifseg_attn_bi_args {
   const void *q, *k, *v, *dout;
@@ -142,6 +155,7 @@
   int causal;
 } ifseg_attn_dbias_args;
 int ifseg_attn_dbias_grads(const ifseg_attn_dbias_args* args, void* stream);
+int ifseg_attn_dbias_grads_group(int n, const ifseg_attn_dbias_args* tasks, void* stream);
 int ifseg_attn_dbias_nparts(void);
 
 int ifseg_attn_bias_pack(const void* bias, int bias_is_f32, long long head_stride, long long row_stride, int H, int T, int S,
```

Measured after the change: 500.9 images/sec (median of 5 runs). Within noise of the previous version (+0.1%).
